# thallolang/thallo

Measured on AMD Instinct MI355X. Metric: pcg_iters_per_sec, higher is better.
Workload: dtype f32

## Files before the change

### include/thallo_hip.h

```cpp
#ifndef THALLO_HIP_H
#define THALLO_HIP_H

#ifdef __cplusplus
extern "C" {
#endif

typedef void* thallo_stream_t;

#define THALLO_HIP_MAX_PARTIALS 1024

typedef struct thallo_sum_t {
    const float* partials;
    int          count;
} thallo_sum_t;

typedef struct thallo_segs_t {
    long off[8];
    long len[8];
    int  n;
} thallo_segs_t;

#define THALLO_DIST_MAX_WORLD 8
#define THALLO_DIST_CTL_WORDS 16
typedef struct thallo_dist_t {
// ... 27 lines not shown

int thallo_hip_pcg_step2(float* r, const float* Ap, const float* pre, float* z, long n,
                         thallo_sum_t alphaN, thallo_sum_t alphaD, float* betaN_out, thallo_stream_t stream);

int thallo_hip_pcg_step2_ranges(float* r, const float* Ap, const float* pre, float* z,
                                long off0, long len0, long off1, long len1,
                                thallo_sum_t alphaN, thallo_sum_t alphaD, float* betaN_out, thallo_stream_t stream);

int thallo_hip_pcg_step2_full(float* delta, const float* p, float* r, const float* Ap, const float* pre,
                              float* z, const float* b, long n, thallo_sum_t alphaN, thallo_sum_t alphaD,
                              float* betaN_out, float* q_out, int lm, thallo_stream_t stream);

int thallo_hip_pcg_step3(float* p, const float* z, long n, thallo_sum_t betaN, thallo_sum_t alphaN,
                         int lm, thallo_stream_t stream);

int thallo_hip_pcg_pupdate(const float* z, const float* p_in, float* p_out, float* delta, long n, int first,
                           thallo_sum_t alphaN_prev, thallo_sum_t alphaD_prev, thallo_sum_t betaN_prev, thallo_stream_t stream);
int thallo_hip_pcg_pupdate_ranges(const float* z, const float* p_in, float* p_out, float* delta,
                                  long off0, long len0, long off1, long len1, int first,
                                  thallo_sum_t alphaN_prev, thallo_sum_t alphaD_prev, thallo_sum_t betaN_prev, thallo_stream_t stream);

int thallo_hip_lm_finalize_diagonal(const float* diag, float* SSq, float* CtC, float* pre, const float* r, float* b, float* z, long n,
                                    float radius, float min_lm_diagonal, float max_lm_diagonal, int save_ssq, int use_preconditioner,
                                    float* alphaN_out, thallo_stream_t stream);
int thallo_hip_lm_step1_finish(float* Ap, const float* CtC, const float* p, long n, float* alphaD_out, thallo_stream_t stream);
int thallo_hip_lm_step2_first_half(float* delta, const float* p, long n, thallo_sum_t alphaN, thallo_sum_t alphaD, thallo_stream_t stream);
int thallo_hip_lm_step2_second_half(float* r, const float* b, const float* Adelta, const float* pre, float* z, const float* delta, long n,
                                    float* betaN_out, float* q_out, thallo_stream_t stream);
int thallo_hip_pcg_init_finish(const float* r, const float* diag, float* pre, float* z, long n, int use_preconditioner,
                               float* alphaN_out, thallo_stream_t stream);
void thallo_hip_lm_set_gate(const unsigned* gate);
int thallo_hip_lm_state_reset(float* state, thallo_stream_t stream);
int thallo_hip_lm_zeta(thallo_sum_t q, int k, float q_tolerance, float* state, thallo_stream_t stream);
int thallo_hip_pcg_step2_full_zeta(float* delta, const float* p, float* r, const float* Ap, const float* pre,
                                   float* z, const float* b, long n, thallo_sum_t alphaN, thallo_sum_t alphaD,
                                   float* betaN_out, float* q_out, unsigned* tickets, int k, float q_tolerance, float* lm_state, thallo_stream_t stream);
int thallo_hip_dot(const float* a, const float* b, long n, float* out, thallo_stream_t stream);

int thallo_hip_linear_update(float* X, const float* delta, const float* p, long len,
                             thallo_sum_t alphaN, thallo_sum_t alphaD, thallo_stream_t stream);

int thallo_hip_slab_pack_iter(const float* vec, thallo_segs_t segs, const float* alphaD_partials, const double* s3_partials, int count, float* out, thallo_stream_t stream);
int thallo_hip_slab_unpack_iter(float* vec, thallo_segs_t top, const float* src_top, thallo_segs_t bot, const float* src_bot,
                                const float* gathered, long stride, int world, thallo_sum_t alphaN, float* alphaD_word, float* betaN_word, thallo_stream_t stream);
int thallo_hip_block_sums(const float* p, const float* Ap, const float* r, const float* pre, long n, float* alphaD_out, double* s3_out, thallo_stream_t stream);
int thallo_hip_shard_scalars(const float* gathered, long stride, int world, const float* alphaD_partials, const double* s3_partials, int count, thallo_sum_t alphaN,
                             float* alphaD_word, float* betaN_word, thallo_stream_t stream);
int thallo_hip_range_unpack(float* vec, thallo_segs_t first_rank_pieces, const float* gathered, long stride, long skip, int world, thallo_stream_t stream);
int thallo_hip_linear_update2(float* X, const float* delta, const float* p_older, thallo_sum_t alphaN_older, thallo_sum_t alphaD_older,
                              const float* p, thallo_sum_t alphaN, thallo_sum_t alphaD, long len, thallo_stream_t stream);
#define THALLO_HIP_MAX_UPDATE_TERMS 32
typedef struct { const float* p[THALLO_HIP_MAX_UPDATE_TERMS]; thallo_sum_t alphaN[THALLO_HIP_MAX_UPDATE_TERMS], alphaD[THALLO_HIP_MAX_UPDATE_TERMS]; int count; } thallo_update_terms_t;
int thallo_hip_linear_update_n(float* X, float* delta, thallo_update_terms_t terms, long len, int max_workgroups , thallo_stream_t stream);
int thallo_hip_wave64_selftest(unsigned long long* out_ballot, unsigned* out_peers, float* sums4);
int thallo_hip_finish_sum(thallo_sum_t s, float* out, thallo_stream_t stream);
int thallo_hip_finish_sum_gated(thallo_sum_t s, float* out, const unsigned* gate, thallo_stream_t stream);

int thallo_hip_slab_pack(const float* vec, thallo_segs_t segs, thallo_sum_t sum, float* out, thallo_stream_t stream);
int thallo_hip_slab_unpack(float* vec, thallo_segs_t top, const float* src_top, thallo_segs_t bot, const float* src_bot,
                           const float* gathered, long stride, int world, float* sum_out, thallo_stream_t stream);

int thallo_hip_alpha_beta(thallo_sum_t alphaN, thallo_sum_t alphaD, thallo_sum_t betaN, float* out2,
                          thallo_stream_t stream);

int thallo_hip_lapimg_cost(int W, int H, const float* X, const float* A, float w_fit, int xguard,
                           float* cost_out, thallo_stream_t stream);
int thallo_hip_lapimg_pcg_init(int W, int H, const float* X, const float* A, float w_fit, int xguard,
                               float* r, float* z, float* p_prev, float* delta,
                               float* diag_out, float* alphaN_out, thallo_stream_t stream);
int thallo_hip_lapimg_apply_jtj(int W, int H, float w_fit, int xguard, const float* p, float* Ap, float* alphaD_out, thallo_stream_t stream);
int thallo_hip_lapimg_pcg_step1(int W, int H, float w_fit, int xguard,
                                const float* z, const float* p_in, float* p_out, float* delta, float* Ap,
                                int first, thallo_sum_t alphaN_prev, thallo_sum_t alphaD_prev, thallo_sum_t betaN_prev,
                                float* alphaD_out, thallo_stream_t stream);

int thallo_hip_iw_cost(int W, int H, int row0, int row1, const float* offset, const float* angle, const float* urshape,
                       const float* constraints, const float* mask, float w_fit, float w_reg,
                       float* cost_out, thallo_stream_t stream);
int thallo_hip_iw_pcg_init(int W, int H, int row0, int row1, const float* offset, const float* angle, const float* urshape,
                           const float* constraints, const float* mask, float w_fit, float w_reg,
                           float* r, float* pre, float* z, float* p_prev, float* delta,
                           float* cs, unsigned char* flags, float* diag_out, int* irregular_out, float* alphaN_out, thallo_stream_t stream);
int thallo_hip_iw_pcg_step1(int W, int H, int row0, int row1, const float* cs, const float* urshape, const unsigned char* flags,
                            float w_fit, float w_reg,
                            const float* z, const float* p_in, float* p_out, float* delta, float* Ap,
                            int mode, thallo_sum_t alphaN_prev, thallo_sum_t alphaD_prev, thallo_sum_t betaN_prev,
                            thallo_sum_t alphaN_prev2, thallo_sum_t alphaD_prev2,
                            const int* irregular, const float* r, float* alphaD_out, thallo_stream_t stream);
#define THALLO_IW_STEP1_MODE(k, batched) ((k) == 0 ? 1 : !(batched) ? 0 : ((k) & 1) ? 2 : 4)
int thallo_hip_iw_pcg_iter(int W, int H, int row0, int row1, const float* cs, const float* urshape, const unsigned char* flags, const float* pre,
                           float w_fit, float w_reg, const float* r_in, float* r_out, const float* Ap_in, float* Ap_out,
                           const float* p_in, float* p_out, float* delta, int mode,
                           thallo_sum_t alphaN_prev, thallo_sum_t alphaD_prev, thallo_sum_t betaN_prev,
                           thallo_sum_t alphaN_prev2, thallo_sum_t alphaD_prev2,
                           const int* irregular, float* alphaD_out, double* s12_out,
                           unsigned* fin_tickets, float* alphaD_word, float* betaN_word, thallo_stream_t stream);
#define THALLO_HIP_FIN_TICKET_WORDS 528
int thallo_hip_iw_pcg_iter_dist(int W, int H, int row0, int row1, const float* cs, const float* urshape, const unsigned char* flags, const float* pre,
                                float w_fit, float w_reg, const float* r_in, float* r_out, const float* Ap_in, float* Ap_out,
                                const float* p_in, float* p_out, float* delta, int mode,
                                thallo_sum_t alphaN_prev, thallo_sum_t alphaD_prev, thallo_sum_t betaN_prev,
                                thallo_sum_t alphaN_prev2, thallo_sum_t alphaD_prev2,
                                const int* irregular, thallo_dist_t d, float* alphaD_out, double* s12_out,
                                unsigned* fin_tickets, int slot0, float* alphaD_word, float* betaN_word, thallo_stream_t stream);
int thallo_hip_iw_pcg_iter_march(int W, int H, int row0, int row1, const float* cs, const unsigned char* flags,
                                 float w_fit, float w_reg, const float* r_in, float* r_out, const float* Ap_in, float* Ap_out,
// ... 307 lines not shown
```

### thallo_amd/api.py

```python
import ctypes as C
import os

import numpy as np

_HERE = os.path.dirname(os.path.abspath(__file__))
LIB_PATH = os.path.join(_HERE, "libThallo.so")
ENERGY_DIR = os.path.join(_HERE, "energies")


class InitializationParameters(C.Structure):
    _fields_ = [(n, C.c_int) for n in ("doublePrecision", "verbosityLevel", "timingLevel",
                                       "threadsPerBlock", "useAutoscheduler", "cpuOnly")]


class PerformanceEntry(C.Structure):
    _fields_ = [("count", C.c_uint), ("minMS", C.c_double), ("maxMS", C.c_double),
                ("meanMS", C.c_double), ("stddevMS", C.c_double)]


class PerformanceSummary(C.Structure):
    _fields_ = [(n, PerformanceEntry) for n in ("total", "nonlinearIteration", "nonlinearSetup",
                                                "linearSolve", "nonlinearResolve")]


class SumT(C.Structure):
    _fields_ = [("partials", C.c_void_p), ("count", C.c_int)]


class DistT(C.Structure):
    _fields_ = [("mail", C.c_void_p), ("peer_mail", C.c_void_p * 8), ("peer_r", C.c_void_p * 2), ("peer_off_o", C.c_long * 2),
                ("peer_off_a", C.c_long * 2), ("ctl", C.c_void_p), ("world", C.c_int), ("rank", C.c_int)]


class SegsT(C.Structure):
    _fields_ = [("off", C.c_long * 8), ("len", C.c_long * 8), ("n", C.c_int)]


INT_PARAMS = ("nIterations", "lIterations", "residual_reset_period", "nIter")

_lib = None


AllGatherFn = C.CFUNCTYPE(C.c_int, C.c_void_p, C.c_void_p, C.c_void_p, C.c_long, C.c_void_p)
AllReduceFn = C.CFUNCTYPE(C.c_int, C.c_void_p, C.c_void_p, C.c_long, C.c_void_p)


class DistributedT(C.Structure):
    _fields_ = [("rank", C.c_int), ("world", C.c_int), ("row0", C.c_uint), ("row1", C.c_uint),
                ("allgather", AllGatherFn), ("user", C.c_void_p), ("device_exchange", C.c_int),
                ("global_row0", C.c_uint), ("global_rows", C.c_uint), ("allreduce", AllReduceFn)]


def lib():
    global _lib
    if _lib is not None:
        return _lib
    path = os.environ.get("THALLO_LIB") or LIB_PATH
    if not os.path.exists(path):
        raise RuntimeError(f"{path} not found: build it with `python -c 'import __graft_entry__ as g; g.build()'` "
                           "(make -C thallo_amd/csrc). There is no CPU fallback.")
    L = C.CDLL(path)
    vp, vpp = C.c_void_p, C.POINTER(C.c_void_p)
    L.Thallo_NewState.argtypes = [InitializationParameters]; L.Thallo_NewState.restype = vp
    L.Thallo_ProblemDefine.argtypes = [vp, C.c_char_p, C.c_char_p]; L.Thallo_ProblemDefine.restype = vp
    L.Thallo_ProblemDelete.argtypes = [vp, vp]
    L.Thallo_ProblemPlan.argtypes = [vp, vp, C.POINTER(C.c_uint)]; L.Thallo_ProblemPlan.restype = vp
    L.Thallo_PlanFree.argtypes = [vp, vp]
    L.Thallo_SetSolverParameter.argtypes = [vp, vp, C.c_char_p, vp]
    L.Thallo_GetSolverParameter.argtypes = [vp, vp, C.c_char_p, vp]
    L.Thallo_ProblemSolve.argtypes = [vp, vp, vpp]
    L.Thallo_ProblemInit.argtypes = [vp, vp, vpp]
    L.Thallo_ProblemStep.argtypes = [vp, vp, vpp]; L.Thallo_ProblemStep.restype = C.c_int
    L.Thallo_ProblemCurrentCost.argtypes = [vp, vp]; L.Thallo_ProblemCurrentCost.restype = C.c_double
    L.Thallo_GetPerformanceSummary.argtypes = [vp, vp, C.POINTER(PerformanceSummary)]
    L.ThalloX_SetStream.argtypes = [vp, vp]
    L.ThalloX_SetKernelSampling.argtypes = [vp, C.c_int]
    L.ThalloX_GetKernelStat.argtypes = [vp, C.c_int, C.POINTER(C.c_char_p), C.POINTER(C.c_long), C.POINTER(C.c_long), C.POINTER(C.c_double)]
    L.ThalloX_GetKernelStat.restype = C.c_int
    L.ThalloX_GetKernelStatOwn.argtypes = [vp, C.c_int, C.POINTER(C.c_long), C.POINTER(C.c_double)]
    L.ThalloX_GetKernelStatOwn.restype = C.c_int
    L.ThalloX_ResetKernelStats.argtypes = [vp]
    L.ThalloX_GetAlphaBetaTrace.argtypes = [vp, vp, C.c_int]; L.ThalloX_GetAlphaBetaTrace.restype = C.c_int
    L.ThalloX_EnableLM.argtypes = [vp, C.c_int]
    L.ThalloX_PlanEnergyName.argtypes = [vp]; L.ThalloX_PlanEnergyName.restype = C.c_char_p
    L.ThalloX_LastError.restype = C.c_char_p
    L.ThalloX_PlanReady.argtypes = [vp]; L.ThalloX_PlanReady.restype = C.c_int
    L.ThalloX_PlanScheduleName.argtypes = [vp]; L.ThalloX_PlanScheduleName.restype = C.c_char_p
    L.ThalloX_PlanSetDistributed.argtypes = [vp, C.POINTER(DistributedT)]; L.ThalloX_PlanSetDistributed.restype = C.c_int
    L.ThalloX_PlanDistributedInfo.argtypes = [vp]; L.ThalloX_PlanDistributedInfo.restype = C.c_char_p
    L.ThalloX_DistributedControl.argtypes = [vp, C.c_int, C.c_int]; L.ThalloX_DistributedControl.restype = C.c_int
    L.ThalloX_UnknownsChanged.argtypes = [vp, vp]
    L.ThalloX_RcclUniqueId.argtypes = [vp]; L.ThalloX_RcclUniqueId.restype = C.c_int
    L.ThalloX_PlanUseRccl.argtypes = [vp, vp, C.c_int, C.c_int]; L.ThalloX_PlanUseRccl.restype = C.c_int
    L.ThalloX_RcclSelfTest.argtypes = []; L.ThalloX_RcclSelfTest.restype = C.c_int
    L.ThalloX_RcclAvailable.argtypes = []; L.ThalloX_RcclAvailable.restype = C.c_int
    L.ThalloX_DistributedKernelOnly.argtypes = [vp, C.c_int]; L.ThalloX_DistributedKernelOnly.restype = C.c_int
    L.ThalloX_ProblemFileHash.argtypes = [C.c_char_p, C.c_char_p, C.c_int]; L.ThalloX_ProblemFileHash.restype = C.c_ulonglong
    L.ThalloX_ProblemFileSchedule.argtypes = [C.c_char_p]; L.ThalloX_ProblemFileSchedule.restype = C.c_int
    fl, ci, cl = C.c_float, C.c_int, C.c_long
    L.thallo_hip_vector_elems.argtypes = [cl]; L.thallo_hip_vector_elems.restype = cl
    L.thallo_hip_finish_sum.argtypes = [SumT, vp, vp]
    L.thallo_hip_iw_cost.argtypes = [ci, ci, ci, ci, vp, vp, vp, vp, vp, fl, fl, vp, vp]
    L.thallo_hip_iw_pcg_init.argtypes = [ci, ci, ci, ci, vp, vp, vp, vp, vp, fl, fl, vp, vp, vp, vp, vp, vp, vp, vp, vp, vp, vp]
    L.thallo_hip_iw_pcg_step1.argtypes = [ci, ci, ci, ci, vp, vp, vp, fl, fl, vp, vp, vp, vp, vp, ci, SumT, SumT, SumT, SumT, SumT, vp, vp, vp, vp]
    L.thallo_hip_linear_update2.argtypes = [vp, vp, vp, SumT, SumT, vp, SumT, SumT, cl, vp]
    L.thallo_hip_ipc_alloc.argtypes = [C.c_long, C.POINTER(vp), vp]
    L.thallo_hip_ipc_alloc2.argtypes = [C.c_long, C.POINTER(vp), vp, C.POINTER(ci)]
    L.thallo_hip_ipc_open.argtypes = [vp, C.POINTER(vp)]
    L.thallo_hip_ipc_close.argtypes = [vp]; L.thallo_hip_ipc_free.argtypes = [vp]
    L.thallo_hip_dist_begin_step.argtypes = [DistT, vp]
    L.thallo_hip_dist_collect.argtypes = [DistT, ci, ci, vp, vp]
    L.thallo_hip_dist_error.argtypes = [DistT, ci, vp]
    L.thallo_hip_slab_pack_iter.argtypes = [vp, SegsT, vp, vp, ci, vp, vp]
    L.thallo_hip_slab_unpack_iter.argtypes = [vp, SegsT, vp, SegsT, vp, vp, cl, ci, SumT, vp, vp, vp]
    L.thallo_hip_dist_exchange.argtypes = [DistT, ci, SumT, vp, vp]
    L.thallo_hip_dist_exchange_iter.argtypes = [DistT, ci, vp, vp, ci, SumT, vp, vp, vp]
    _iter = [ci, ci, ci, ci, vp, vp, vp, vp, fl, fl, vp, vp, vp, vp, vp, vp, vp, ci, SumT, SumT, SumT, SumT, SumT, vp]
    L.thallo_hip_iw_pcg_iter.argtypes = _iter + [vp, vp, vp, vp, vp, vp]
    L.thallo_hip_iw_pcg_iter_dist.argtypes = _iter + [DistT, vp, vp, vp, ci, vp, vp, vp]
    _march = [ci, ci, ci, ci, vp, vp, fl, fl, vp, vp, vp, vp, vp, vp, vp, ci, SumT, SumT, SumT, SumT, SumT, vp]
    L.thallo_hip_iw_pcg_iter_march.argtypes = _march + [vp, vp, vp, vp, vp, vp]
    L.thallo_hip_iw_pcg_iter_march_dist.argtypes = _march + [DistT, vp, vp, vp, ci, vp, vp, vp]
    L.thallo_hip_iw_urshape_irregular.argtypes = [ci, ci, vp, vp, vp]
    L.thallo_hip_march_debug_set.argtypes = [ci, ci]
    L.thallo_hip_iw_pcg_iter_finish.argtypes = [vp, vp, ci, SumT, vp, vp, vp]
    L.thallo_hip_iw_pcg_step2_dist.argtypes = [ci, ci, ci, ci, vp, fl, fl, vp, vp, SumT, SumT, DistT, vp, vp]
    L.thallo_hip_iw_pcg_step2.argtypes = [ci, ci, ci, ci, vp, fl, fl, vp, vp, vp, vp, SumT, SumT, vp, vp, vp]
    L.thallo_hip_iw_apply_jtj.argtypes = [ci, ci, ci, ci, vp, vp, vp, fl, fl, vp, vp, vp, vp, vp]
    L.thallo_hip_pcg_step2.argtypes = [vp, vp, vp, vp, cl, SumT, SumT, vp, vp]
    L.thallo_hip_pcg_step2_ranges.argtypes = [vp, vp, vp, vp, cl, cl, cl, cl, SumT, SumT, vp, vp]
    L.thallo_hip_linear_update.argtypes = [vp, vp, vp, cl, SumT, SumT, vp]
    L.thallo_hip_slab_pack.argtypes = [vp, SegsT, SumT, vp, vp]
    L.thallo_hip_slab_unpack.argtypes = [vp, SegsT, vp, SegsT, vp, vp, cl, ci, vp, vp]
    _lib = L
    return L


def energy_file(name):
    p = os.path.join(ENERGY_DIR, name if name.endswith(".t") else name + ".t")
    if not os.path.exists(p):
        raise FileNotFoundError(p)
    return p


def last_error():
    return lib().ThalloX_LastError().decode()


def slab_ghost_rows(path, dims):
    L = lib()
    L.ThalloX_FrontendSlabGhostRows.argtypes = [C.c_char_p, C.c_void_p]
    L.ThalloX_FrontendSlabGhostRows.restype = C.c_int
    d = (C.c_uint * len(dims))(*[int(x) for x in dims])
    g = L.ThalloX_FrontendSlabGhostRows(os.fsencode(path), d)
    if g < 0:
        raise ValueError(last_error())
    return g


def rccl_unique_id():
    buf = (C.c_ubyte * 128)()
    if lib().ThalloX_RcclUniqueId(C.addressof(buf)) != 0:
        raise RuntimeError("ThalloX_RcclUniqueId failed: " + last_error())
    return bytes(buf)


def _ptr_of(x):
    if hasattr(x, "data_ptr"):
        return x.data_ptr()
    if isinstance(x, (C.c_float, C.c_int, C.c_double, C.c_uint)):
        return C.addressof(x)
    if isinstance(x, int):
        return x
    raise TypeError(f"cannot turn {type(x)} into a problem parameter")

# ... 145 lines not shown
        import json
        t = self._L.ThalloX_PlanDistributedInfo(self.plan).decode()
        return json.loads(t) if t else {}

    def distributed_error(self, clear=True):
        return self._L.ThalloX_DistributedControl(self.plan, 0, 1 if clear else 0)

    def distributed_use_allgather(self):
        return self._L.ThalloX_DistributedControl(self.plan, 1, 0)

    def distributed_kernel_only(self, reps):
        return self._L.ThalloX_DistributedKernelOnly(self.plan, reps)

    def unknowns_changed(self):
        self._L.ThalloX_UnknownsChanged(self.state, self.plan)

    def enable_lm(self, on=True):
        self._L.ThalloX_EnableLM(self.plan, 1 if on else 0)

    def set_kernel_sampling(self, period):
        self._L.ThalloX_SetKernelSampling(self.plan, period)

    def reset_kernel_stats(self):
        self._L.ThalloX_ResetKernelStats(self.plan)

    def kernel_stats(self):
        out = {}
        i = 0
        while True:
            name = C.c_char_p(); launches = C.c_long(); samples = C.c_long(); total = C.c_double()
            if self._L.ThalloX_GetKernelStat(self.plan, i, C.byref(name), C.byref(launches), C.byref(samples), C.byref(total)):
                break
            ks = C.c_long(); kt = C.c_double()
            self._L.ThalloX_GetKernelStatOwn(self.plan, i, C.byref(ks), C.byref(kt))
            out[name.value.decode()] = {"launches": launches.value, "samples": samples.value, "total_ms": total.value,
                                        "mean_ms": total.value / samples.value if samples.value else None,
                                        "own_samples": ks.value, "own_mean_ms": kt.value / ks.value if ks.value else None}
            i += 1
        return out

    def alpha_beta_trace(self, cap=4096):
        buf = (C.c_float * (2 * cap))()
        n = self._L.ThalloX_GetAlphaBetaTrace(self.plan, C.addressof(buf), cap)
        n = min(n, cap)
        return [(buf[2 * i], buf[2 * i + 1]) for i in range(n)]


def iw_fused_bytes_per_iter(L, every_iteration_delta=False, ring=False):
    if os.environ.get("THALLO_MARCH", "1")[:1] in ("0", "3", "4"):
        return 99.0
    if L < 1:
        return 0.0
    if ring:
        return (69.0 + 57.0 * (L - 1)) / L
    if every_iteration_delta:
        return (69.0 + 81.0 * (L - 1)) / L
    odd, even = L // 2, (L - 1) // 2
    return (69.0 + 57.0 * odd + 93.0 * even) / L
```

### thallo_amd/csrc/energy_image_warping.hip

```cpp
#include "iw_device.hpp"

using namespace thallo;

namespace {

constexpr int TW = 64, TH = 16, BLOCK = 256;
constexpr int LW = TW + 2, LH = TH + 2, LN = LW * LH;
constexpr int PER = TH / (BLOCK / TW);
constexpr int HALO = 2 * LW + 2 * TH;

inline Geo make_geo(int W, int H, int row0, int row1)
{
    Geo g; g.W = W; g.H = H; g.row0 = row0; g.row1 = row1;
    g.tx = (W + TW - 1) / TW; g.ty = (row1 - row0 + TH - 1) / TH; g.ntiles = g.tx * g.ty;
    return g;
}
inline bool rows_ok(int H, int row0, int row1) { return row0 >= 0 && row1 <= H && row0 < row1; }
inline int grid_for(const Geo& g, int per_cu)
{
    int cap = thallo_hip_device_cu_count() * per_cu;
    if (cap > THALLO_MAX_PARTIALS) cap = THALLO_MAX_PARTIALS;
    cap -= cap % 8;
    return g.ntiles < cap ? g.ntiles : cap;
}
// ... 213 lines not shown

template <bool DIST>
__global__ __launch_bounds__(BLOCK) void k_step2_iw(float4* __restrict__ r, const float4* __restrict__ Ap, const float4* __restrict__ pre,
                                                     float4* __restrict__ z, const unsigned char* __restrict__ flags, long N, float wf2, float wr2,
                                                     long off0, long len0, long off1, long len1,
                                                     thallo_sum_t aN, thallo_sum_t aD, const int* __restrict__ irregular, float* __restrict__ bN_out,
                                                     thallo_dist_t dd, long row_o4, long row_a4)
{
    __shared__ float red[16];
    const bool grid = DIST || (irregular != nullptr && __builtin_amdgcn_readfirstlane(irregular[0]) == 0);
    const float alpha = safe_div<false>(sum_partials(aN.partials, aN.count), sum_partials(aD.partials, aD.count));
    float acc = 0.0f;
    const long n4 = len0 + len1;
    for (long j = (long)blockIdx.x * BLOCK + threadIdx.x; j < n4; j += (long)gridDim.x * BLOCK) {
        const bool in_off = j < len0;
        const long i = in_off ? off0 + j : off1 + (j - len0);
        float4 rv = ldf4(r + i, true);
        const float4 av = Ap[i];
        rv.x -= alpha * av.x; rv.y -= alpha * av.y; rv.z -= alpha * av.z; rv.w -= alpha * av.w;
        float4 m;
        if (grid) {
            if (in_off) {
                const unsigned f2 = reinterpret_cast<const unsigned short*>(flags)[i];
                float m0, m1, dummy;
                pre_from_flags((unsigned char)(f2 & 255), wf2, wr2, m0, dummy); pre_from_flags((unsigned char)(f2 >> 8), wf2, wr2, m1, dummy);
                m = make_float4(m0, m0, m1, m1);
            } else {
                const unsigned f4 = reinterpret_cast<const unsigned*>(flags)[i - N / 2];
                float d, a0, a1, a2, a3;
                pre_from_flags((unsigned char)(f4 & 255), wf2, wr2, d, a0); pre_from_flags((unsigned char)((f4 >> 8) & 255), wf2, wr2, d, a1);
                pre_from_flags((unsigned char)((f4 >> 16) & 255), wf2, wr2, d, a2); pre_from_flags((unsigned char)(f4 >> 24), wf2, wr2, d, a3);
                m = make_float4(a0, a1, a2, a3);
            }
        } else m = pre[i];
        const float4 zv = make_float4(m.x * rv.x, m.y * rv.y, m.z * rv.z, m.w * rv.w);
        stf4(r + i, rv, true);
        if (!grid) z[i] = zv;
        if (DIST) {
            const long jj = in_off ? j : j - len0, rowlen = in_off ? row_o4 : row_a4, total = in_off ? len0 : len1;
            if (jj < rowlen && dd.peer_r[0]) {
                float* dst = dd.peer_r[0] + (in_off ? dd.peer_off_o[0] : dd.peer_off_a[0]) + 4 * jj;
                st_sys(dst, rv.x); st_sys(dst + 1, rv.y); st_sys(dst + 2, rv.z); st_sys(dst + 3, rv.w);
            }
            if (jj >= total - rowlen && dd.peer_r[1]) {
                float* dst = dd.peer_r[1] + (in_off ? dd.peer_off_o[1] : dd.peer_off_a[1]) + 4 * (jj - (total - rowlen));
                st_sys(dst, rv.x); st_sys(dst + 1, rv.y); st_sys(dst + 2, rv.z); st_sys(dst + 3, rv.w);
            }
        }
        acc += zv.x * rv.x + zv.y * rv.y + zv.z * rv.z + zv.w * rv.w;
    }
    block_store_partial(acc, bN_out, red);
}

__global__ __launch_bounds__(BLOCK) void k_init(Geo g, const float2* __restrict__ off, const float* __restrict__ ang,
                                                const float2* __restrict__ ur, const float2* __restrict__ cons,
                                                const float* __restrict__ mask, float wf, float wr,
                                                float* __restrict__ r, float* __restrict__ pre, float* __restrict__ z,
                                                float* __restrict__ p_prev, float* __restrict__ delta,
                                                float2* __restrict__ cs, unsigned char* __restrict__ flags,
                                                float* __restrict__ diag_out, int* __restrict__ irregular, float* __restrict__ aN_out)
{
    __shared__ Tile T;
    __shared__ float red[16];
    const long N = (long)g.W * g.H;
    const float wr2 = wr * wr, wf2 = wf * wf;
    float acc = 0.0f;
    int bad = 0;
    for (TileSweep t(g.ntiles); t.valid(); t.next()) {
        const int x0 = (t.cur % g.tx) * TW, y0 = g.row0 + (t.cur / g.tx) * TH;
        for (int idx = threadIdx.x; idx < LN; idx += BLOCK) {
            const int ly = idx / LW, lx = idx - ly * LW;
            const int gx = x0 + lx - 1, gy = y0 + ly - 1;
            float ox = 0.f, oy = 0.f, cc = 1.f, ss = 0.f, uxx = 0.f, uyy = 0.f; unsigned char ff = 0;
            if (gx >= 0 && gx < g.W && gy >= 0 && gy < g.H) {
                const long pix = (long)gy * g.W + gx;
                const float2 o = off[pix]; const float2 u = ur[pix];
                ox = o.x; oy = o.y; uxx = u.x; uyy = u.y;
                sincosf(ang[pix], &ss, &cc);
                ff = mask[pix] == 0.0f ? 1 : 0;
                if ((gy < g.row0 || gy >= g.row1) && lx >= 1 && lx <= TW) {
                    cs[pix] = make_float2(cc, ss); flags[pix] = ff;
                    reinterpret_cast<float2*>(p_prev)[pix] = make_float2(0.f, 0.f); p_prev[2 * N + pix] = 0.f;
                }
            }
            T.px[idx] = ox; T.py[idx] = oy; T.c[idx] = cc; T.s[idx] = ss; T.ux[idx] = uxx; T.uy[idx] = uyy; T.f[idx] = ff;
        }
        __syncthreads();
        const int lx = (threadIdx.x % TW) + 1;
        const int gx = x0 + lx - 1;
        for (int k = 0; k < PER; ++k) {
            const int ly = (threadIdx.x / TW) * PER + k + 1;
            const int gy = y0 + ly - 1;
            const int i = ly * LW + lx;
            if (gx < g.W && gy < g.row1) {
                const long pix = (long)gy * g.W + gx;
                const unsigned char act = T.f[i] & 1;
                if (gx + 1 < g.W && (T.ux[i + 1] - T.ux[i] != 1.0f || T.uy[i + 1] - T.uy[i] != 0.0f)) bad = 1;
                if (gy + 1 < g.H && (T.ux[i + LW] - T.ux[i] != 0.0f || T.uy[i + LW] - T.uy[i] != 1.0f)) bad = 1;
                float rx = 0.f, ry = 0.f, ra = 0.f, mx = 0.f, my = 0.f, ma = 0.f, dgo_raw = 0.f, dga_raw = 0.f;
                unsigned char fl = act;
                if (act) {
                    const float oxi = T.px[i], oyi = T.py[i], ci = T.c[i], si = T.s[i], uxi = T.ux[i], uyi = T.uy[i];
                    float jx = 0.f, jy = 0.f, ja = 0.f, dgo = 0.f, dga = 0.f;
                    int cnt = 0; bool unit = true;
                    const int nb[4] = { i + 1, i - 1, i + LW, i - LW };
#pragma unroll
                    for (int d = 0; d < 4; ++d) {
                        const int j = nb[d];
                        if (T.f[j] & 1) {
                            const float dux = uxi - T.ux[j], duy = uyi - T.uy[j];
                            unit = unit && dux == (d == 0 ? -1.0f : d == 1 ? 1.0f : 0.0f) && duy == (d == 2 ? -1.0f : d == 3 ? 1.0f : 0.0f);
                            ++cnt;
                            const float dox = oxi - T.px[j], doy = oyi - T.py[j];
                            const float eix = dox - (ci * dux - si * duy), eiy = doy - (si * dux + ci * duy);
                            const float cj = T.c[j], sj = T.s[j];
                            const float ejx = -dox + (cj * dux - sj * duy), ejy = -doy + (sj * dux + cj * duy);
                            const float gix = -si * dux - ci * duy, giy = ci * dux - si * duy;
                            jx += eix - ejx; jy += eiy - ejy;
                            ja -= gix * eix + giy * eiy;
                            dgo += 2.0f; dga += gix * gix + giy * giy;
                        }
                    }
                    jx *= wr2; jy *= wr2; ja *= wr2; dgo *= wr2; dga *= wr2;
                    if (unit) dga = (float)cnt * wr2;
                    fl |= (unsigned char)(cnt << 2);
                    const float2 cv = cons[pix];
                    if (cv.x >= 0.0f && cv.y >= 0.0f) {
                        fl |= 2;
                        jx += wf2 * (oxi - cv.x); jy += wf2 * (oyi - cv.y); dgo += wf2;
                    }
                    rx = -jx; ry = -jy; ra = -ja;
                    mx = guarded_invert(dgo); my = mx; ma = guarded_invert(dga);
                    dgo_raw = dgo; dga_raw = dga;
                }
                if (diag_out) {
                    reinterpret_cast<float2*>(diag_out)[pix] = make_float2(dgo_raw, dgo_raw); diag_out[2 * N + pix] = dga_raw;
                }
                reinterpret_cast<float2*>(r)[pix] = make_float2(rx, ry);  r[2 * N + pix] = ra;
                reinterpret_cast<float2*>(pre)[pix] = make_float2(mx, my); pre[2 * N + pix] = ma;
                const float zx = mx * rx, zy = my * ry, zaa = ma * ra;
                reinterpret_cast<float2*>(z)[pix] = make_float2(zx, zy);  z[2 * N + pix] = zaa;
                reinterpret_cast<float2*>(p_prev)[pix] = make_float2(0.f, 0.f); p_prev[2 * N + pix] = 0.f;
                reinterpret_cast<float2*>(delta)[pix] = make_float2(0.f, 0.f);  delta[2 * N + pix] = 0.f;
                cs[pix] = make_float2(T.c[i], T.s[i]);
                flags[pix] = fl;
                acc += rx * zx + ry * zy + ra * zaa;
            }
        }
        __syncthreads();
    }
    if (irregular && __any(bad) && (threadIdx.x & 63) == 0) atomicAdd(irregular, 1);
    block_store_partial(acc, aN_out, red);
}

constexpr int CW = 64, CH = 4;
__global__ __launch_bounds__(BLOCK) void k_cost(int W, int H, int row0, int row1, int ctx, int ntiles,
                                                const float2* __restrict__ off, const float* __restrict__ ang,
                                                const float2* __restrict__ ur, const float2* __restrict__ cons,
                                                const float* __restrict__ mask, float wf, float wr, float* __restrict__ out)
{
    __shared__ float red[16];
    float acc = 0.0f;
    for (TileSweep t(ntiles); t.valid(); t.next()) {
        const int x = (t.cur % ctx) * CW + (threadIdx.x % CW), y = row0 + (t.cur / ctx) * CH + (threadIdx.x / CW);
        if (x < W && y < row1) {
            const long i = (long)y * W + x;
            if (mask[i] == 0.0f) {
                const float2 o = off[i]; const float2 u = ur[i];
                float si, ci; sincosf(ang[i], &si, &ci);
                float s2 = 0.f;
                const int dx[4] = { 1, -1, 0, 0 }, dy[4] = { 0, 0, 1, -1 };
#pragma unroll
                for (int d = 0; d < 4; ++d) {
                    const int xn = x + dx[d], yn = y + dy[d];
                    if (xn >= 0 && xn < W && yn >= 0 && yn < H) {
                        const long j = (long)yn * W + xn;
                        if (mask[j] == 0.0f) {
                            const float2 oj = off[j]; const float2 uj = ur[j];
                            const float dux = u.x - uj.x, duy = u.y - uj.y;
                            const float ex = wr * ((o.x - oj.x) - (ci * dux - si * duy));
                            const float ey = wr * ((o.y - oj.y) - (si * dux + ci * duy));
                            s2 += ex * ex + ey * ey;
                        }
                    }
                }
                const float2 cv = cons[i];
                if (cv.x >= 0.0f && cv.y >= 0.0f) {
                    const float fx = wf * (o.x - cv.x), fy = wf * (o.y - cv.y);
                    s2 += fx * fx + fy * fy;
                }
                acc += 0.5f * s2;
            }
        }
    }
    block_store_partial(acc, out, red);
}
// ... 245 lines not shown
                                                       PrevSums prev)
{
    __shared__ TileI T;
    __shared__ float red[16];
    __shared__ double redd[48];
    const bool grid = irregular != nullptr && __builtin_amdgcn_readfirstlane(irregular[0]) == 0;
    if (grid) iter_body<true, NT, DIST>(T, red, redd, g, cs, ur, flags, pre, wf2, wr2, r_in, r_out, A_in, A_out, p_in, p_out, delta, mode, aNp, aDp, bNp, aNpp, aDpp, aD_out, s12_out, ntm, &dd, fin_tickets, aD_word, bN_word, xslot, prev);
    else      iter_body<false, NT, DIST>(T, red, redd, g, cs, ur, flags, pre, wf2, wr2, r_in, r_out, A_in, A_out, p_in, p_out, delta, mode, aNp, aDp, bNp, aNpp, aDpp, aD_out, s12_out, ntm, &dd, fin_tickets, aD_word, bN_word, xslot, prev);
}

__global__ __launch_bounds__(64) void k_iter_finish(const float* __restrict__ aD_part, const double* __restrict__ s12, int nb, thallo_sum_t aN,
                                                    float* __restrict__ aD_word, float* __restrict__ bN_word)
{
    const int lane = threadIdx.x;
    const float ad = sum_partials(aD_part, nb);
    double n = 0.0, a = 0.0, b = 0.0;
    for (int i = lane; i < nb; i += THALLO_WAVE) { n += s12[3 * i]; a += s12[3 * i + 1]; b += s12[3 * i + 2]; }
    n = wave_sum_all_d(n); a = wave_sum_all_d(a); b = wave_sum_all_d(b);
    const float an = sum_partials(aN.partials, aN.count);
    const float alpha = safe_div<false>(an, ad);
    double bn = n - 2.0 * (double)alpha * a + (double)alpha * (double)alpha * b;
    if (!(bn > 0.0)) bn = 0.0;
    if (lane == 0) { aD_word[0] = ad; bN_word[0] = (float)bn; }
}

}

extern "C" {

#ifdef THALLO_MARCH_SWEEP
int thallo_hip_debug_stamps(unsigned long long* buf) { return hipMemcpyToSymbol(HIP_SYMBOL(g_stamps), &buf, sizeof buf) == hipSuccess ? 0 : -1; }
#endif
void thallo_hip_debug_set(int what, int value) { if (what == 0) g_iw_debug = value; if (what == 3) g_nt_mask = value; if (what == 4) g_no_grid = value; if (what == 5) g_step1_per_cu = value; if (what == 6) g_step1_threads = value; if (what == 7) g_iter_nt = value; if (what == 8) g_iter_per_cu = value < 1 ? 1 : value > 2 ? 2 : value; }

int thallo_hip_iw_cost(int W, int H, int row0, int row1, const float* offset, const float* angle, const float* urshape,
                       const float* constraints, const float* mask, float w_fit, float w_reg,
                       float* cost_out, thallo_stream_t stream)
{
    if (!rows_ok(H, row0, row1)) return -(int)hipErrorInvalidValue;
    const int ctx = (W + CW - 1) / CW, cty = (row1 - row0 + CH - 1) / CH, nt = ctx * cty;
    int grid = thallo_hip_device_cu_count() * 4; if (grid > THALLO_MAX_PARTIALS) grid = THALLO_MAX_PARTIALS;
    grid -= grid % 8; if (nt < grid) grid = nt;
    hipLaunchKernelGGL(k_cost, dim3(grid), dim3(BLOCK), 0, (hipStream_t)stream, W, H, row0, row1, ctx, nt,
                       (const float2*)offset, angle, (const float2*)urshape, (const float2*)constraints, mask, w_fit, w_reg, cost_out);
    int e = check_launch(); return e ? e : grid;
}

int thallo_hip_iw_pcg_init(int W, int H, int row0, int row1, const float* offset, const float* angle, const float* urshape,
                           const float* constraints, const float* mask, float w_fit, float w_reg,
                           float* r, float* pre, float* z, float* p_prev, float* delta,
                           float* cs, unsigned char* flags, float* diag_out, int* irregular_out, float* aN_out, thallo_stream_t stream)
{
    if (!rows_ok(H, row0, row1)) return -(int)hipErrorInvalidValue;
    const Geo g = make_geo(W, H, row0, row1); const int grid = grid_for(g, 4);
    if (irregular_out && hipMemsetAsync(irregular_out, 0, sizeof(int), (hipStream_t)stream) != hipSuccess) return -(int)hipErrorInvalidValue;
    hipLaunchKernelGGL(k_init, dim3(grid), dim3(BLOCK), 0, (hipStream_t)stream, g,
                       (const float2*)offset, angle, (const float2*)urshape, (const float2*)constraints, mask, w_fit, w_reg,
                       r, pre, z, p_prev, delta, (float2*)cs, flags, diag_out, irregular_out, aN_out);
    int e = check_launch(); return e ? e : grid;
}

int thallo_hip_iw_pcg_step1(int W, int H, int row0, int row1, const float* cs, const float* urshape, const unsigned char* flags,
                            float w_fit, float w_reg,
                            const float* z, const float* p_in, float* p_out, float* delta, float* Ap,
                            int mode, thallo_sum_t aNp, thallo_sum_t aDp, thallo_sum_t bNp, thallo_sum_t aNpp, thallo_sum_t aDpp,
                            const int* irregular, const float* r, float* aD_out, thallo_stream_t stream)
{
    if (!r || ((2L * W * H) & 3)) irregular = nullptr;
    if (!rows_ok(H, row0, row1)) return -(int)hipErrorInvalidValue;
    const Geo g = make_geo(W, H, row0, row1);
    int grid;
    if (g_step1_threads == 512) {
        grid = grid_for(g, g_step1_per_cu > 2 ? 2 : g_step1_per_cu);
        hipLaunchKernelGGL((k_step1<true, 4, 512>), dim3(grid), dim3(512), 0, (hipStream_t)stream, g,
                           (const float2*)cs, (const float2*)urshape, flags, w_fit * w_fit, w_reg * w_reg,
                           z, p_in, p_out, delta, Ap, mode, aNp, aDp, bNp, aNpp, aDpp, aD_out, g_iw_debug | (g_nt_mask << 8), g_no_grid ? nullptr : irregular, r);
    } else {
        grid = grid_for(g, g_step1_per_cu);
        hipLaunchKernelGGL((k_step1<true, 3, 256>), dim3(grid), dim3(BLOCK), 0, (hipStream_t)stream, g,
                           (const float2*)cs, (const float2*)urshape, flags, w_fit * w_fit, w_reg * w_reg,
                           z, p_in, p_out, delta, Ap, mode, aNp, aDp, bNp, aNpp, aDpp, aD_out, g_iw_debug | (g_nt_mask << 8), g_no_grid ? nullptr : irregular, r);
    }
    int e = check_launch(); return e ? e : grid;
}

int thallo_hip_iw_pcg_step2(int W, int H, int row0, int row1, const unsigned char* flags, float w_fit, float w_reg,
                            float* r, const float* Ap, const float* pre, float* z,
                            thallo_sum_t aN, thallo_sum_t aD, const int* irregular, float* bN_out, thallo_stream_t stream)
{
    if (!rows_ok(H, row0, row1)) return -(int)hipErrorInvalidValue;
    const long N = (long)W * H, rows = row1 - row0;
    const long off0 = 2L * W * row0, len0 = 2L * W * rows, off1 = 2 * N + (long)W * row0, len1 = (long)W * rows;
    if (g_no_grid || ((off0 | len0 | off1 | len1 | (2 * N)) & 3)) {
        if (row0 == 0 && row1 == H) return thallo_hip_pcg_step2(r, Ap, pre, z, 3 * N, aN, aD, bN_out, stream);
        return thallo_hip_pcg_step2_ranges(r, Ap, pre, z, off0, len0, off1, len1, aN, aD, bN_out, stream);
    }
    long want = ((len0 + len1) / 4 + BLOCK - 1) / BLOCK;
    int grid = thallo_hip_device_cu_count() * 4; if (grid > THALLO_MAX_PARTIALS) grid = THALLO_MAX_PARTIALS; grid -= grid % 8;
    if (want < grid) grid = (int)(want < 1 ? 1 : want);
    hipLaunchKernelGGL(k_step2_iw<false>, dim3(grid), dim3(BLOCK), 0, (hipStream_t)stream, (float4*)r, (const float4*)Ap, (const float4*)pre, (float4*)z,
                       flags, N, w_fit * w_fit, w_reg * w_reg, off0 / 4, len0 / 4, off1 / 4, len1 / 4, aN, aD, irregular, bN_out, thallo_dist_t{}, 0L, 0L);
    int e = check_launch(); return e ? e : grid;
}

static bool dist_args_ok(const thallo_dist_t& d)
{
    return d.world >= 1 && d.world <= THALLO_DIST_MAX_WORLD && d.rank >= 0 && d.rank < d.world && d.mail && d.ctl && d.peer_mail[d.rank] == d.mail;
}

int thallo_hip_iw_pcg_step2_dist(int W, int H, int row0, int row1, const unsigned char* flags, float w_fit, float w_reg,
                                 float* r, const float* Ap, thallo_sum_t aN, thallo_sum_t aD, thallo_dist_t d,
// ... 109 lines not shown
```

### thallo_amd/csrc/energy_image_warping_march_rc.hip

```cpp
#include "iw_march.hpp"
#include <hip/hip_ext.h>

using namespace thallo;

namespace {

inline int check_launch() { hipError_t e = hipGetLastError(); return e == hipSuccess ? 0 : -(int)e; }

typedef __amdgpu_buffer_rsrc_t rsrc_t;
typedef unsigned u32x4 __attribute__((ext_vector_type(4)));
typedef unsigned u32x2 __attribute__((ext_vector_type(2)));
__device__ __forceinline__ rsrc_t make_rsrc(const void* p) { return __builtin_amdgcn_make_buffer_rsrc(const_cast<void*>(p), 0, 0xffffffffu, 0x00020000); }
template <bool NT> __device__ __forceinline__ u32x4 bld4(rsrc_t r, unsigned vo, unsigned so) { return __builtin_amdgcn_raw_buffer_load_b128(r, vo, so, NT ? 2 : 0); }
template <bool NT> __device__ __forceinline__ u32x2 bld2(rsrc_t r, unsigned vo, unsigned so) { return __builtin_amdgcn_raw_buffer_load_b64(r, vo, so, NT ? 2 : 0); }
template <bool NT> __device__ __forceinline__ unsigned bld1(rsrc_t r, unsigned vo, unsigned so) { return __builtin_amdgcn_raw_buffer_load_b32(r, vo, so, NT ? 2 : 0); }
template <bool NT> __device__ __forceinline__ void bst4(rsrc_t r, unsigned vo, unsigned so, float a, float b, float c, float d)
{ u32x4 v; v.x = __float_as_uint(a); v.y = __float_as_uint(b); v.z = __float_as_uint(c); v.w = __float_as_uint(d); __builtin_amdgcn_raw_buffer_store_b128(v, r, vo, so, NT ? 2 : 0); }
template <bool NT> __device__ __forceinline__ void bst2(rsrc_t r, unsigned vo, unsigned so, float a, float b)
{ u32x2 v; v.x = __float_as_uint(a); v.y = __float_as_uint(b); __builtin_amdgcn_raw_buffer_store_b64(v, r, vo, so, NT ? 2 : 0); }
__device__ __forceinline__ float uf(unsigned u) { return __uint_as_float(u); }
__device__ __forceinline__ float to_sgpr(float v) { return __int_as_float(__builtin_amdgcn_readfirstlane(__float_as_int(v))); }

__device__ __forceinline__ float rc_sum(thallo_sum_t s)
{
// ... 24 lines not shown
    beta = safe_div<false>(bn, an);
}

__device__ __forceinline__ void rc_exchange_prev(thallo_sum_t aNp, const PrevSums& prev, const thallo_dist_t& dd)
{
    typedef unsigned long long u64_t;
    const unsigned seq = ld_agent(dd.ctl + DIST_SEQ);
    const unsigned tag = (seq << 12) | (unsigned)(prev.xslot / 7 + 1);
    const IterationSums S = load_iteration_sums(prev.aD_part, prev.s12_part, prev.count, aNp);
    float ad = 0.0f, al = 0.0f, bn = 0.0f;
    dist_exchange_iter_wave_seq(dd, seq, prev.xslot, S.ad, S.n, S.s1, S.s2, S.an, prev.aD_word, prev.bN_word, ExtraSums{ false, 0.0f, 0.0, 0.0, 0.0 }, &ad, &al, &bn);
    if ((threadIdx.x & (THALLO_WAVE - 1)) == 0) {
        __hip_atomic_store(prev.gs, ((u64_t)tag << 32) | (u64_t)__float_as_uint(ad), __ATOMIC_RELAXED, __HIP_MEMORY_SCOPE_AGENT);
        __hip_atomic_store(prev.gs + 1, ((u64_t)tag << 32) | (u64_t)__float_as_uint(bn), __ATOMIC_RELAXED, __HIP_MEMORY_SCOPE_AGENT);
    }
}
__device__ __forceinline__ void rc_iteration_scalars_x(thallo_sum_t aNp, const PrevSums& prev, const thallo_dist_t& dd, float& alpha, float& beta)
{
    typedef unsigned long long u64_t;
    const float an = rc_sum(aNp);
    const unsigned seq = ld_agent(dd.ctl + DIST_SEQ);
    const unsigned tag = (seq << 12) | (unsigned)(prev.xslot / 7 + 1);
    u64_t v0 = __hip_atomic_load(prev.gs, __ATOMIC_RELAXED, __HIP_MEMORY_SCOPE_AGENT), v1 = __hip_atomic_load(prev.gs + 1, __ATOMIC_RELAXED, __HIP_MEMORY_SCOPE_AGENT);
    int it = 0; long long t0 = 0;
    const long long bound = dist_spin_ticks(dd);
    while ((unsigned)(v0 >> 32) != tag || (unsigned)(v1 >> 32) != tag) {
        if ((it & 255) == 0) { if (ld_agent(dd.ctl + DIST_ERR) != 0) break; if (it == 0) t0 = wall_clock64(); }
        ++it;
        if ((it & 255) == 0 && wall_clock64() - t0 > bound) {
            if (__hip_atomic_exchange(dd.ctl + DIST_ERR, 1u, __ATOMIC_RELAXED, __HIP_MEMORY_SCOPE_AGENT) == 0u) {
                unsigned* pm = dd.ctl + DIST_POST_MORTEM;
                pm[0] = (unsigned)prev.xslot; pm[1] = 0xffffu; pm[2] = tag; pm[3] = (unsigned)(v0 >> 32); pm[4] = (unsigned)(v1 >> 32);
            }
            break;
        }
        __builtin_amdgcn_s_sleep(4);
        v0 = __hip_atomic_load(prev.gs, __ATOMIC_RELAXED, __HIP_MEMORY_SCOPE_AGENT); v1 = __hip_atomic_load(prev.gs + 1, __ATOMIC_RELAXED, __HIP_MEMORY_SCOPE_AGENT);
    }
    const float ad = __uint_as_float((unsigned)v0), bn = __uint_as_float((unsigned)v1);
    alpha = safe_div<false>(an, ad);
    beta = safe_div<false>(bn, an);
}
__global__ __launch_bounds__(64) void k_rc_dist_finish(thallo_sum_t aNp, PrevSums prev, thallo_dist_t dd) { rc_exchange_prev(aNp, prev, dd); }

template <int DMODE>
struct RawRc {
    u32x4 po, cs; u32x2 pa; unsigned f;
    u32x4 ro; u32x2 ra;
    u32x4 dlo, ppo; u32x2 dla, ppa;
};
typedef unsigned long long u64x2 __attribute__((ext_vector_type(2)));
__device__ __forceinline__ void take4u(u32x4& d, const u32x4& s) { const u64x2 sv = __builtin_bit_cast(u64x2, s); unsigned long long a, b; take_pair(a, sv.x); take_pair(b, sv.y); u64x2 dv; dv.x = a; dv.y = b; d = __builtin_bit_cast(u32x4, dv); }
__device__ __forceinline__ void take2u(u32x2& d, const u32x2& s) { unsigned long long a; take_pair(a, __builtin_bit_cast(unsigned long long, s)); d = __builtin_bit_cast(u32x2, a); }
template <int DMODE>
__device__ __forceinline__ void take(RawRc<DMODE>& d, const RawRc<DMODE>& s)
{
    take4u(d.po, s.po); take2u(d.pa, s.pa); take4u(d.cs, s.cs); take1(d.f, s.f); take4u(d.ro, s.ro); take2u(d.ra, s.ra);
    if (DMODE != 1) { take4u(d.dlo, s.dlo); take2u(d.dla, s.dla); }
    if (DMODE == 2) { take4u(d.ppo, s.ppo); take2u(d.ppa, s.ppa); }
}

template <int V> struct IC { static constexpr int value = V; };
enum { PH_ENTER = 0, PH_S1 = 1, PH_FULL = 2 };

struct PRow { v2f xy[2]; float pa[2]; };
struct GRow { v2f cs[2], gx[2]; float a[2]; unsigned f; };
struct RRow { v2f xy[2]; float ra[2]; };
__device__ __forceinline__ v2f uf2(unsigned a, unsigned b) { return v2f{ uf(a), uf(b) }; }

template <int DMODE, int DEPTH, int NTM, int OCC, int SLAB>
__global__ __launch_bounds__(MARCH_NT, OCC) void k_iter_march_rc(MarchGeo g, const float* __restrict__ cs, const unsigned char* __restrict__ flags, float wf2, float wr2,
                                                            const float* __restrict__ r_in, float* __restrict__ r_out, const float* __restrict__ A_in, float* __restrict__ A_out,
                                                            const float* __restrict__ p_in, float* __restrict__ p_out, float* __restrict__ delta,
                                                            thallo_sum_t aNp, thallo_sum_t aDp, thallo_sum_t bNp, thallo_sum_t aNpp, thallo_sum_t aDpp,
                                                            float* __restrict__ aD_out, double* __restrict__ s12_out, const int* __restrict__ irregular,
                                                            thallo_dist_t dd, unsigned* __restrict__ fin_tickets, float* __restrict__ aD_word, float* __restrict__ bN_word, int xslot,
                                                            PrevSums prev)
{
    static_assert(DEPTH == 1 || DEPTH == 2 || DEPTH == 4, "the prefetch slots rotate inside a trip of four rows");
    __shared__ float4 lut[32];
    __shared__ float red[16];
    __shared__ double redd[48];
    constexpr bool nt_delta = NTM & 1, nt_ra = NTM & 2, nt_out = NTM & 4, nt_pin = NTM & 8, nt_pout = NTM & 16, nt_const = NTM & 32;
    if (irregular != nullptr && __builtin_amdgcn_readfirstlane(irregular[0]) != 0) {
        if (blockIdx.x == 0 && threadIdx.x == 0 && aD_word) { aD_word[0] = __builtin_nanf(""); bN_word[0] = __builtin_nanf(""); }
        if (blockIdx.x == 0 && threadIdx.x == 0 && prev.count > 0) { prev.aD_word[0] = __builtin_nanf(""); prev.bN_word[0] = __builtin_nanf(""); }
        if (threadIdx.x == 0) { aD_out[blockIdx.x] = __builtin_nanf(""); }
        return;
    }
    if (threadIdx.x < 32) { float mo, ma; pre_from_flags((unsigned char)threadIdx.x, wf2, wr2, mo, ma); lut[threadIdx.x] = make_float4(mo, ma, (threadIdx.x & 2) ? wf2 : 0.f, 0.f); }
    __syncthreads();

    const int lane = threadIdx.x & 63, wave = __builtin_amdgcn_readfirstlane(threadIdx.x >> 6);
    const unsigned N = (unsigned)g.W * (unsigned)g.H;
    const int W2 = g.W >> 1;
    int strip, ya, yb;
    march_place(g, wave, strip, ya, yb);
    const bool work = ya < yb;
    const int x0 = strip * MARCH_USE - 2 + 2 * lane;
    const bool xin = x0 >= 0 && x0 < g.W;
    const bool xout = xin && lane >= 1 && lane <= 62;

    const rsrc_t RS_P = make_rsrc(p_in), RS_R = make_rsrc(r_in), RS_CS = make_rsrc(cs), RS_F = make_rsrc(flags);
    const rsrc_t RS_Q = make_rsrc(p_out), RS_RO = make_rsrc(r_out), RS_D = make_rsrc(delta);
    const rsrc_t RS_AI = make_rsrc(SLAB ? (const void*)A_in : (const void*)r_in), RS_AO = make_rsrc(SLAB ? (void*)A_out : (void*)r_out);
    const int xc = x0 < 0 ? 0 : x0 > g.W - 2 ? g.W - 2 : x0;
    const unsigned h = (unsigned)xc >> 1;
    const unsigned vo16 = h * 16u, vo8 = h * 8u;
    const unsigned vf0 = (h >> 1) * 4u, vf1 = ((h + 1u) >> 1) * 4u, sh0 = (h & 1u) * 16u;
    const unsigned angle0 = 8u * N;

    float alpha = 0.0f, beta = 0.0f, alpha2 = 0.0f;
    const bool scal_writer = work && strip == 0 && ya == g.row0 && lane == 0;

    typedef RawRc<DMODE> RawT;
    RawT slot[DEPTH];
    const unsigned W2u = (unsigned)W2;
    const int t_first = ya - 2, t_last = yb + 1;
    auto issue = [&](RawT& s, int tn, auto CL_) __attribute__((always_inline)) {
        constexpr bool CL = decltype(CL_)::value;
        if (CL && tn > t_last) tn = t_last;
        const unsigned tc = CL ? (unsigned)(tn < 0 ? 0 : tn > g.H - 1 ? g.H - 1 : tn) : (unsigned)tn, row = tc * W2u;
        s.po = bld4<nt_pin>(RS_P, vo16, row * 16u); s.pa = bld2<nt_pin>(RS_P, vo8, angle0 + row * 8u);
        s.cs = bld4<nt_const>(RS_CS, vo16, row * 16u);
        const unsigned par = row & 1u;
        s.f = bld1<nt_const>(RS_F, par ? vf1 : vf0, (row - par) * 2u);
        const unsigned tr = CL ? (unsigned)(tn - 1 < 0 ? 0 : tn - 1 > g.H - 1 ? g.H - 1 : tn - 1) : (unsigned)(tn - 1), rrow = tr * W2u;
        s.ro = bld4<nt_ra>(RS_R, vo16, rrow * 16u); s.ra = bld2<nt_ra>(RS_R, vo8, angle0 + rrow * 8u);
        if (DMODE != 1) {
            const unsigned td = CL ? (unsigned)(tn - 1 < ya ? ya : tn - 1 > yb - 1 ? yb - 1 : tn - 1) : (unsigned)(tn - 1), drow = td * W2u;
            s.dlo = bld4<nt_delta>(RS_D, vo16, drow * 16u); s.dla = bld2<nt_delta>(RS_D, vo8, angle0 + drow * 8u);
            if (DMODE == 2) { s.ppo = bld4<false>(RS_Q, vo16, drow * 16u); s.ppa = bld2<false>(RS_Q, vo8, angle0 + drow * 8u); }
        }
    };

    PRow pp[4], pk[4]; GRow gg[4]; RRow rr[2];
#pragma unroll
    for (int i = 0; i < 4; ++i) {
#pragma unroll
        for (int q = 0; q < 2; ++q) { pp[i].xy[q] = v2f{ 0.f, 0.f }; pp[i].pa[q] = 0.f; pk[i].xy[q] = v2f{ 0.f, 0.f }; pk[i].pa[q] = 0.f;
                                      gg[i].cs[q] = v2f{ 1.f, 0.f }; gg[i].gx[q] = v2f{ 0.f, -1.f }; gg[i].a[q] = 0.f; }
        gg[i].f = 0u;
    }
#pragma unroll
    for (int i = 0; i < 2; ++i)
#pragma unroll
        for (int q = 0; q < 2; ++q) { rr[i].xy[q] = v2f{ 0.f, 0.f }; rr[i].ra[q] = 0.f; }

    float acc = 0.0f; double s0 = 0.0, s1 = 0.0, s2 = 0.0;
    const unsigned mxin = xin ? 0xffffu : 0u;

    auto step = [&](int t, auto J_, auto PH_, auto CL_) __attribute__((always_inline)) {
        constexpr int j = decltype(J_)::value, PH = decltype(PH_)::value;
        constexpr bool CL = decltype(CL_)::value;
        PRow& p0 = pp[j % 4]; const PRow& p1 = pp[(j + 3) % 4]; const PRow& p2 = pp[(j + 2) % 4];
        GRow& g0 = gg[j % 4]; const GRow& g1 = gg[(j + 3) % 4]; const GRow& g2 = gg[(j + 2) % 4]; const GRow& g3 = gg[(j + 1) % 4];
        PRow& k1 = pk[(j + 3) % 4]; const PRow& k2 = pk[(j + 2) % 4]; const PRow& k3 = pk[(j + 1) % 4];
        RRow& r1 = rr[(j + 1) % 2]; const RRow& r2 = rr[j % 2];
        RawT cur;
        take(cur, slot[j % DEPTH]);
        fence_order();
        issue(slot[j % DEPTH], t + DEPTH, CL_);
        fence_order();
        {
            const bool rowok = !CL || (t >= 0 && t < g.H);
            const unsigned par = ((unsigned)t * W2u) & 1u;
            const unsigned fl = (cur.f >> (par ? 16u - sh0 : sh0)) & (rowok ? mxin : 0u);
            p0.xy[0] = uf2(cur.po.x, cur.po.y); p0.xy[1] = uf2(cur.po.z, cur.po.w); p0.pa[0] = uf(cur.pa.x); p0.pa[1] = uf(cur.pa.y);
            g0.cs[0] = uf2(cur.cs.x, cur.cs.y); g0.cs[1] = uf2(cur.cs.z, cur.cs.w); g0.f = fl;
            g0.gx[0] = v2f{ g0.cs[0].y, -g0.cs[0].x }; g0.gx[1] = v2f{ g0.cs[1].y, -g0.cs[1].x };
            g0.a[0] = (float)(fl & 1u); g0.a[1] = (float)((fl >> 8) & 1u);
        }
        if constexpr (PH >= PH_S1) {
            const int u = t - 1;
            const float4 m0 = lut[g1.f & 31u], m1 = lut[(g1.f >> 8) & 31u];
            const float wfit[2] = { m0.z, m1.z };
            v2f axy[2]; float av[2];
            jtjp_pair_xy(p2, p1, p0, g2, g1, g0, g2.a, g1.a, g0.a, wfit, wr2, axy, av);
            const bool ghost_row = SLAB && CL && ((u == ya - 1 && ya == g.row0 && u >= 0) || (u == yb && yb == g.row1 && u < g.H));
            if (ghost_row) {
                const unsigned row = (unsigned)u * W2u;
                const u32x4 ao = bld4<false>(RS_AI, vo16, row * 16u); const u32x2 aa = bld2<false>(RS_AI, vo8, angle0 + row * 8u);
                axy[0] = uf2(ao.x, ao.y); axy[1] = uf2(ao.z, ao.w); av[0] = uf(aa.x); av[1] = uf(aa.y);
            }
            v2f rxy[2] = { uf2(cur.ro.x, cur.ro.y), uf2(cur.ro.z, cur.ro.w) }; float rq[2] = { uf(cur.ra.x), uf(cur.ra.y) };
            rxy[0] = fma2(-alpha, axy[0], rxy[0]); rxy[1] = fma2(-alpha, axy[1], rxy[1]);
            rq[0] = __builtin_fmaf(-alpha, av[0], rq[0]); rq[1] = __builtin_fmaf(-alpha, av[1], rq[1]);
            const float mo[2] = { m0.x, m1.x }, ma[2] = { m0.y, m1.y };
#pragma unroll
            for (int q = 0; q < 2; ++q) {
                k1.xy[q] = mo[q] * rxy[q] + beta * p1.xy[q]; k1.pa[q] = ma[q] * rq[q] + beta * p1.pa[q];
                r1.xy[q] = rxy[q]; r1.ra[q] = rq[q];
            }
            const bool mine = !CL || (u >= ya && u < yb);
            if (xout && (mine || ghost_row)) {
                const unsigned row = (unsigned)u * W2u;
                bst4<nt_out>(RS_RO, vo16, row * 16u, rxy[0].x, rxy[0].y, rxy[1].x, rxy[1].y); bst2<nt_out>(RS_RO, vo8, angle0 + row * 8u, rq[0], rq[1]);
                bst4<nt_pout>(RS_Q, vo16, row * 16u, k1.xy[0].x, k1.xy[0].y, k1.xy[1].x, k1.xy[1].y); bst2<nt_pout>(RS_Q, vo8, angle0 + row * 8u, k1.pa[0], k1.pa[1]);
                if (DMODE != 1 && mine) {
                    float d[4] = { uf(cur.dlo.x), uf(cur.dlo.y), uf(cur.dlo.z), uf(cur.dlo.w) }, da[2] = { uf(cur.dla.x), uf(cur.dla.y) };
                    if (DMODE == 2) {
                        d[0] = __builtin_fmaf(alpha2, uf(cur.ppo.x), d[0]); d[1] = __builtin_fmaf(alpha2, uf(cur.ppo.y), d[1]);
                        d[2] = __builtin_fmaf(alpha2, uf(cur.ppo.z), d[2]); d[3] = __builtin_fmaf(alpha2, uf(cur.ppo.w), d[3]);
                        da[0] = __builtin_fmaf(alpha2, uf(cur.ppa.x), da[0]); da[1] = __builtin_fmaf(alpha2, uf(cur.ppa.y), da[1]);
                    }
                    d[0] = __builtin_fmaf(alpha, p1.xy[0].x, d[0]); d[1] = __builtin_fmaf(alpha, p1.xy[0].y, d[1]);
                    d[2] = __builtin_fmaf(alpha, p1.xy[1].x, d[2]); d[3] = __builtin_fmaf(alpha, p1.xy[1].y, d[3]);
                    da[0] = __builtin_fmaf(alpha, p1.pa[0], da[0]); da[1] = __builtin_fmaf(alpha, p1.pa[1], da[1]);
                    bst4<nt_delta>(RS_D, vo16, row * 16u, d[0], d[1], d[2], d[3]); bst2<nt_delta>(RS_D, vo8, angle0 + row * 8u, da[0], da[1]);
                }
            }
        }
        __builtin_amdgcn_sched_barrier(0);
        if constexpr (PH >= PH_FULL) {
            const int v = t - 2;
            const bool on = xout;
            const float4 m0 = lut[on ? g2.f & 31u : 0u], m1 = lut[on ? (g2.f >> 8) & 31u : 0u];
            const float wfit[2] = { m0.z, m1.z }, mo[2] = { m0.x, m1.x }, ma[2] = { m0.y, m1.y };
            v2f axy[2]; float av[2];
            jtjp_pair_xy(k3, k2, k1, g3, g2, g1, g3.a, g2.a, g1.a, wfit, wr2, axy, av);
            if (SLAB && xout && (v == g.row0 || v == g.row1 - 1)) {
                if (SLAB == 1) {
                    const unsigned row = (unsigned)v * W2u;
                    bst4<false>(RS_AO, vo16, row * 16u, axy[0].x, axy[0].y, axy[1].x, axy[1].y); bst2<false>(RS_AO, vo8, angle0 + row * 8u, av[0], av[1]);
                } else {
#pragma unroll
                    for (int k = 0; k < 2; ++k) {
                        if (v == (k == 0 ? g.row0 : g.row1 - 1) && dd.peer_r[k]) {
                            float* d2 = dd.peer_r[k] + dd.peer_off_o[k] + 2 * x0;
                            st_sys(d2, axy[0].x); st_sys(d2 + 1, axy[0].y); st_sys(d2 + 2, axy[1].x); st_sys(d2 + 3, axy[1].y);
                            float* d1 = dd.peer_r[k] + dd.peer_off_a[k] + x0;
                            st_sys(d1, av[0]); st_sys(d1 + 1, av[1]);
                        }
                    }
                }
            }
            const float msum = on ? 1.0f : 0.0f;
            __builtin_amdgcn_sched_barrier(0);
            iter_sums_pixel_masked(msum, k2.xy[0].x, k2.xy[0].y, k2.pa[0], axy[0].x, axy[0].y, av[0], r2.xy[0].x, r2.xy[0].y, r2.ra[0], mo[0], ma[0], acc, s0, s1, s2);
            __builtin_amdgcn_sched_barrier(0);
            iter_sums_pixel_masked(msum, k2.xy[1].x, k2.xy[1].y, k2.pa[1], axy[1].x, axy[1].y, av[1], r2.xy[1].x, r2.xy[1].y, r2.ra[1], mo[1], ma[1], acc, s0, s1, s2);
        }
        asm volatile("" : "+v"(acc), "+v"(s0), "+v"(s1), "+v"(s2));
        __builtin_amdgcn_sched_barrier(0);
    };

    if (SLAB == 2 && prev.gs != nullptr && prev.count > 0 && blockIdx.x == gridDim.x - 1 && wave == 0 && !work) rc_exchange_prev(aNp, prev, dd);

    if (work) {
#pragma unroll
        for (int i = 0; i < DEPTH; ++i) issue(slot[i], t_first + i, IC<1>{});
        step(t_first, IC<0>{}, IC<PH_ENTER>{}, IC<1>{});
        step(t_first + 1, IC<1>{}, IC<PH_ENTER>{}, IC<1>{});
        if (SLAB == 2 && prev.gs != nullptr && prev.count > 0) rc_iteration_scalars_x(aNp, prev, dd, alpha, beta);
        else rc_iteration_scalars(aNp, aDp, bNp, prev, alpha, beta, scal_writer);
        alpha = to_sgpr(alpha); beta = to_sgpr(beta);
        if (DMODE == 2) alpha2 = to_sgpr(safe_div<false>(rc_sum(aNpp), rc_sum(aDpp)));
        step(ya, IC<2>{}, IC<PH_S1>{}, IC<1>{});
        step(ya + 1, IC<3>{}, IC<PH_S1>{}, IC<1>{});
        int t_lim = t_last < g.H - 1 ? t_last : g.H - 1;
        if (DMODE != 1 && yb < t_lim) t_lim = yb;
        const int t_safe = t_lim - DEPTH;
        int t = ya + 2;
        for (; t + 3 <= t_safe; t += 4) {
            step(t, IC<0>{}, IC<PH_FULL>{}, IC<0>{});
            step(t + 1, IC<1>{}, IC<PH_FULL>{}, IC<0>{});
            step(t + 2, IC<2>{}, IC<PH_FULL>{}, IC<0>{});
            step(t + 3, IC<3>{}, IC<PH_FULL>{}, IC<0>{});
        }
        auto tail = [&](auto I_) __attribute__((always_inline)) {
            constexpr int i = decltype(I_)::value;
            if constexpr (i < DEPTH + 5) { if (t + i <= t_last) step(t + i, IC<i % 4>{}, IC<PH_FULL>{}, IC<1>{}); }
        };
        tail(IC<0>{}); tail(IC<1>{}); tail(IC<2>{}); tail(IC<3>{}); tail(IC<4>{}); tail(IC<5>{}); tail(IC<6>{}); tail(IC<7>{}); tail(IC<8>{});
    }
    iter_tail<MARCH_NT, SLAB == 2>(acc, s0, s1, s2, red, redd, aD_out, s12_out, bNp, &dd, fin_tickets, aD_word, bN_word, xslot);
}

}

[[maybe_unused]] constexpr int MARCH_RC_DEPTH = 4;
constexpr int MARCH_RC_OCC = 2;
[[maybe_unused]] constexpr int MARCH_RC_DEEP_ROWS = 24;
#ifdef THALLO_MARCH_SWEEP
namespace thallo {
int g_march_rc_depth = MARCH_RC_DEPTH;
int g_march_rc_occ = MARCH_RC_OCC;
int g_march_rc_nt = MARCH_NTM;
}
#endif

namespace {
struct LaunchEvents { hipEvent_t start = nullptr, stop = nullptr; int armed = 0, used = 0; };
thread_local LaunchEvents g_launch_ev;

template <int SLAB>
int launch_march_rc(int W, int H, int row0, int row1, const float* cs, const unsigned char* flags, float w_fit, float w_reg,
                    const float* r_in, float* r_out, const float* A_in, float* A_out, const float* p_in, float* p_out, float* delta, int mode,
                    thallo_sum_t aNp, thallo_sum_t aDp, thallo_sum_t bNp, thallo_sum_t aNpp, thallo_sum_t aDpp, const int* irregular, thallo_dist_t d,
                    float* aD_out, double* s12_out, unsigned* fin_tickets, float* aD_word, float* bN_word, int xslot, hipStream_t stream, PrevSums prev)
{
    const int R = march_pick_rows(W, row1 - row0);
    if (R <= 0) return -(int)hipErrorNotSupported;
    const MarchGeo g = make_march_geo(W, H, row0, row1, R);
    const int grid = (g.total + 7) / 8 * 8 + ((SLAB == 2 && prev.gs != nullptr) ? 8 : 0);
    if (grid > THALLO_MAX_PARTIALS) return -(int)hipErrorInvalidValue;
    const int dmode = (mode >> 1) & 3;
    const float wf2 = w_fit * w_fit, wr2 = w_reg * w_reg;
    const bool ev_on = g_launch_ev.armed != 0;
    if (ev_on) g_launch_ev.used = 1;
#define RC_LAUNCH(DM, DP, OCC, NTM) do { if (ev_on) hipExtLaunchKernelGGL((k_iter_march_rc<DM, DP, NTM, OCC, SLAB>), dim3(grid), dim3(MARCH_NT), 0, stream, g_launch_ev.start, g_launch_ev.stop, 0, g, cs, flags, wf2, wr2, \
        r_in, r_out, A_in, A_out, p_in, p_out, delta, aNp, aDp, bNp, aNpp, aDpp, aD_out, s12_out, irregular, d, fin_tickets, aD_word, bN_word, xslot, prev); \
    else hipLaunchKernelGGL((k_iter_march_rc<DM, DP, NTM, OCC, SLAB>), dim3(grid), dim3(MARCH_NT), 0, stream, g, cs, flags, wf2, wr2, \
        r_in, r_out, A_in, A_out, p_in, p_out, delta, aNp, aDp, bNp, aNpp, aDpp, aD_out, s12_out, irregular, d, fin_tickets, aD_word, bN_word, xslot, prev); } while (0)
#ifdef THALLO_MARCH_SWEEP
#define RC_BY_DEPTH(DM) do { if constexpr (SLAB != 0) RC_LAUNCH(DM, MARCH_RC_DEPTH, MARCH_RC_OCC, MARCH_NTM); else { const int dp = g_march_rc_depth, oc = g_march_rc_occ, nt = g_march_rc_nt; \
        if (nt != MARCH_NTM) { if (nt == 0) RC_LAUNCH(DM, MARCH_RC_DEPTH, 2, 0); else if (nt == 1) RC_LAUNCH(DM, MARCH_RC_DEPTH, 2, 1); else if (nt == 4) RC_LAUNCH(DM, MARCH_RC_DEPTH, 2, 4); else if (nt == 7) RC_LAUNCH(DM, MARCH_RC_DEPTH, 2, 7); \
                                 else if (nt == 13) RC_LAUNCH(DM, MARCH_RC_DEPTH, 2, 13); else if (nt == 21) RC_LAUNCH(DM, MARCH_RC_DEPTH, 2, 21); else if (nt == 37) RC_LAUNCH(DM, MARCH_RC_DEPTH, 2, 37); else if (nt == 63) RC_LAUNCH(DM, MARCH_RC_DEPTH, 2, 63); else return -(int)hipErrorInvalidValue; } \
        else if (oc == 1) { if (dp == 4) RC_LAUNCH(DM, 4, 1, MARCH_NTM); else RC_LAUNCH(DM, 2, 1, MARCH_NTM); } \
        else if (oc == 3) { if (dp == 1) RC_LAUNCH(DM, 1, 3, MARCH_NTM); else RC_LAUNCH(DM, 2, 3, MARCH_NTM); } \
        else { if (dp == 1) RC_LAUNCH(DM, 1, 2, MARCH_NTM); else if (dp == 4) RC_LAUNCH(DM, 4, 2, MARCH_NTM); else RC_LAUNCH(DM, 2, 2, MARCH_NTM); } } } while (0)
#else
#define RC_BY_DEPTH(DM) do { if (R >= MARCH_RC_DEEP_ROWS) RC_LAUNCH(DM, 4, MARCH_RC_OCC, MARCH_NTM); else RC_LAUNCH(DM, 2, MARCH_RC_OCC, MARCH_NTM); } while (0)
#endif
    if (dmode == 1) RC_BY_DEPTH(1); else if (dmode == 2) RC_BY_DEPTH(2); else RC_BY_DEPTH(0);
#undef RC_BY_DEPTH
#undef RC_LAUNCH
    int e = check_launch(); return e ? e : grid;
}

int rc_check(int W, int H, int row0, int row1, const void* cs, const void* flags, const void* r_in, const void* r_out, const void* A_in, const void* A_out,
             const void* p_in, const void* p_out, const void* delta, int mode, thallo_sum_t aNp, thallo_sum_t aNpp, thallo_sum_t aDpp, const void* aD_out, const void* s12_out)
{
    if ((W & 1) || W < 2 || H < 1 || row0 < 0 || row1 > H || row0 >= row1 || row0 > 1 || H - row1 > 1) return -(int)hipErrorInvalidValue;
    if (mode & 1) return -(int)hipErrorInvalidValue;
    if (!cs || !flags || !r_in || !r_out || !p_in || !p_out || !delta || !aD_out || !s12_out) return -(int)hipErrorInvalidValue;
    if ((row0 > 0 || row1 < H) && (!A_in || !A_out)) return -(int)hipErrorInvalidValue;
    if (aNp.count < 1 || !aNp.partials) return -(int)hipErrorInvalidValue;
    if (((mode >> 1) & 3) == 2 && (aNpp.count < 1 || aDpp.count < 1 || !aNpp.partials || !aDpp.partials)) return -(int)hipErrorInvalidValue;
    if (12.0 * (double)W * (double)H >= 4294967296.0) return -(int)hipErrorNotSupported;
    return 0;
}
}

extern "C" {

int thallo_hip_iw_pcg_iter_march_rc(int W, int H, int row0, int row1, const float* cs, const unsigned char* flags, float w_fit, float w_reg,
                                    const float* r_in, float* r_out, const float* Ap_in, float* Ap_out, const float* p_in, float* p_out, float* delta, int mode,
                                    thallo_sum_t aNp, thallo_sum_t aDp, thallo_sum_t bNp, thallo_sum_t aNpp, thallo_sum_t aDpp,
                                    const int* irregular, float* aD_out, double* s12_out,
                                    unsigned* fin_tickets, float* aD_word, float* bN_word, thallo_stream_t stream)
{
    if (int e = rc_check(W, H, row0, row1, cs, flags, r_in, r_out, Ap_in, Ap_out, p_in, p_out, delta, mode, aNp, aNpp, aDpp, aD_out, s12_out)) return e;
    if (aDp.count < 1 || bNp.count < 1 || !aDp.partials || !bNp.partials) return -(int)hipErrorInvalidValue;
    if (!fin_tickets || !aD_word || !bN_word) { fin_tickets = nullptr; aD_word = nullptr; bN_word = nullptr; }
    const PrevSums none = { nullptr, nullptr, 0, nullptr, nullptr };
    if (row0 == 0 && row1 == H)
        return launch_march_rc<0>(W, H, row0, row1, cs, flags, w_fit, w_reg, r_in, r_out, nullptr, nullptr, p_in, p_out, delta, mode, aNp, aDp, bNp, aNpp, aDpp, irregular, thallo_dist_t{},
                                  aD_out, s12_out, fin_tickets, aD_word, bN_word, 0, (hipStream_t)stream, none);
    return launch_march_rc<1>(W, H, row0, row1, cs, flags, w_fit, w_reg, r_in, r_out, Ap_in, Ap_out, p_in, p_out, delta, mode, aNp, aDp, bNp, aNpp, aDpp, irregular, thallo_dist_t{},
                              aD_out, s12_out, fin_tickets, aD_word, bN_word, 0, (hipStream_t)stream, none);
}

int thallo_hip_iw_pcg_iter_march_rc_deferred(int W, int H, int row0, int row1, const float* cs, const unsigned char* flags, float w_fit, float w_reg,
                                             const float* r_in, float* r_out, const float* Ap_in, float* Ap_out, const float* p_in, float* p_out, float* delta, int mode,
                                             thallo_sum_t aNp, thallo_sum_t aNpp, thallo_sum_t aDpp, thallo_prev_t prev,
                                             const int* irregular, float* aD_out, double* s12_out, thallo_stream_t stream)
{
    if (int e = rc_check(W, H, row0, row1, cs, flags, r_in, r_out, Ap_in, Ap_out, p_in, p_out, delta, mode, aNp, aNpp, aDpp, aD_out, s12_out)) return e;
    if (prev.count < 1 || prev.count > THALLO_MAX_PARTIALS || !prev.alphaD_partials || !prev.s12_partials || !prev.alphaD_word || !prev.betaN_word ||
        prev.s12_partials == s12_out) return -(int)hipErrorInvalidValue;
    const thallo_sum_t none = { nullptr, 0 };
    const PrevSums ps = { prev.alphaD_partials, prev.s12_partials, prev.count, prev.alphaD_word, prev.betaN_word };
    if (row0 == 0 && row1 == H)
        return launch_march_rc<0>(W, H, row0, row1, cs, flags, w_fit, w_reg, r_in, r_out, nullptr, nullptr, p_in, p_out, delta, mode, aNp, none, none, aNpp, aDpp, irregular, thallo_dist_t{},
                                  aD_out, s12_out, nullptr, nullptr, nullptr, 0, (hipStream_t)stream, ps);
    return launch_march_rc<1>(W, H, row0, row1, cs, flags, w_fit, w_reg, r_in, r_out, Ap_in, Ap_out, p_in, p_out, delta, mode, aNp, none, none, aNpp, aDpp, irregular, thallo_dist_t{},
                              aD_out, s12_out, nullptr, nullptr, nullptr, 0, (hipStream_t)stream, ps);
}

int thallo_hip_iw_pcg_iter_march_rc_dist(int W, int H, int row0, int row1, const float* cs, const unsigned char* flags, float w_fit, float w_reg,
                                         const float* r_in, float* r_out, const float* Ap_in, float* Ap_out, const float* p_in, float* p_out, float* delta, int mode,
                                         thallo_sum_t aNp, thallo_sum_t aDp, thallo_sum_t bNp, thallo_sum_t aNpp, thallo_sum_t aDpp,
                                         const int* irregular, thallo_dist_t d, float* aD_out, double* s12_out,
                                         unsigned* fin_tickets, int slot0, float* aD_word, float* bN_word, thallo_stream_t stream)
{
    if (int e = rc_check(W, H, row0, row1, cs, flags, r_in, r_out, Ap_in, Ap_out, p_in, p_out, delta, mode, aNp, aNpp, aDpp, aD_out, s12_out)) return e;
    if (!Ap_in || !Ap_out || aDp.count < 1 || bNp.count < 1 || !aDp.partials || !bNp.partials || d.world < 1 || d.world > THALLO_DIST_MAX_WORLD) return -(int)hipErrorInvalidValue;
    if (!fin_tickets || !aD_word || !bN_word) { fin_tickets = nullptr; aD_word = nullptr; bN_word = nullptr; }
    if (fin_tickets && (slot0 < 0 || !d.mail || !d.ctl || 7 * d.world > 64 || bNp.count != 1)) return -(int)hipErrorInvalidValue;
    for (int k = 0; k < 2; ++k) if (d.peer_r[k] && ((d.peer_off_o[k] | d.peer_off_a[k]) & 1)) return -(int)hipErrorInvalidValue;
    return launch_march_rc<2>(W, H, row0, row1, cs, flags, w_fit, w_reg, r_in, r_out, Ap_in, Ap_out, p_in, p_out, delta, mode, aNp, aDp, bNp, aNpp, aDpp, irregular, d,
                              aD_out, s12_out, fin_tickets, aD_word, bN_word, slot0, (hipStream_t)stream, PrevSums{ nullptr, nullptr, 0, nullptr, nullptr });
}

int thallo_hip_iw_march_rc_deferred_fits(int W, int rows)
{
    if (W < 2 || (W & 1) || rows < 1) return 0;
    const int R = march_pick_rows(W, rows);
    if (R <= 0) return 0;
    const MarchGeo g = make_march_geo(W, rows, 0, rows, R);
    const long grid = (g.total + 7) / 8 * 8 + 8;
    return grid <= march_cap(MARCH_RC_OCC) && grid <= THALLO_MAX_PARTIALS ? 1 : 0;
}

int thallo_hip_iw_pcg_iter_march_rc_dist_deferred(int W, int H, int row0, int row1, const float* cs, const unsigned char* flags, float w_fit, float w_reg,
                                                  const float* r_in, float* r_out, const float* Ap_in, float* Ap_out, const float* p_in, float* p_out, float* delta, int mode,
                                                  thallo_sum_t aNp, thallo_sum_t aNpp, thallo_sum_t aDpp, thallo_prev_t prev, int prev_slot0, unsigned long long* gs,
                                                  const int* irregular, thallo_dist_t d, float* aD_out, double* s12_out, thallo_stream_t stream)
{
    if (int e = rc_check(W, H, row0, row1, cs, flags, r_in, r_out, Ap_in, Ap_out, p_in, p_out, delta, mode, aNp, aNpp, aDpp, aD_out, s12_out)) return e;
    if (!Ap_in || !Ap_out || d.world < 1 || d.world > THALLO_DIST_MAX_WORLD || !d.mail || !d.ctl || 7 * d.world > 64 || prev_slot0 < 0 || !gs || aNp.count != 1) return -(int)hipErrorInvalidValue;
    if (!thallo_hip_iw_march_rc_deferred_fits(W, row1 - row0)) return -(int)hipErrorNotSupported;
    if (prev.count < 1 || prev.count > THALLO_MAX_PARTIALS || !prev.alphaD_partials || !prev.s12_partials || !prev.alphaD_word || !prev.betaN_word ||
        prev.s12_partials == s12_out) return -(int)hipErrorInvalidValue;
    for (int k = 0; k < 2; ++k) if (d.peer_r[k] && ((d.peer_off_o[k] | d.peer_off_a[k]) & 1)) return -(int)hipErrorInvalidValue;
    const thallo_sum_t none = { nullptr, 0 };
    const PrevSums ps = { prev.alphaD_partials, prev.s12_partials, prev.count, prev.alphaD_word, prev.betaN_word, gs, prev_slot0 };
    return launch_march_rc<2>(W, H, row0, row1, cs, flags, w_fit, w_reg, r_in, r_out, Ap_in, Ap_out, p_in, p_out, delta, mode, aNp, none, none, aNpp, aDpp, irregular, d,
                              aD_out, s12_out, nullptr, nullptr, nullptr, 0, (hipStream_t)stream, ps);
}
int thallo_hip_iw_dist_finish_deferred(thallo_prev_t prev, int prev_slot0, thallo_sum_t aNp, thallo_dist_t d, unsigned long long* gs, thallo_stream_t stream)
{
    if (prev.count < 1 || prev.count > THALLO_MAX_PARTIALS || !prev.alphaD_partials || !prev.s12_partials || !prev.alphaD_word || !prev.betaN_word || prev_slot0 < 0 || !gs ||
        aNp.count != 1 || !aNp.partials || d.world < 1 || d.world > THALLO_DIST_MAX_WORLD || !d.mail || !d.ctl || 7 * d.world > 64) return -(int)hipErrorInvalidValue;
    const PrevSums ps = { prev.alphaD_partials, prev.s12_partials, prev.count, prev.alphaD_word, prev.betaN_word, gs, prev_slot0 };
// ... 20 lines not shown
```

### thallo_amd/csrc/pcg_kernels.hip

```cpp
#include "device_common.hpp"
#include "../../include/thallo_hip.h"

using namespace thallo;

namespace {

constexpr int BLOCK = 256;

inline int flat_grid(long n4, int cus)
{
    long want = (n4 + BLOCK - 1) / BLOCK;
    long cap = (long)cus * 4;
    if (cap > THALLO_MAX_PARTIALS) cap = THALLO_MAX_PARTIALS;
    if (cap >= 8) cap -= cap % 8;
    if (want > cap) want = cap;
    if (want < 1) want = 1;
    return (int)want;
}

int g_cus = 0;
int g_nt2 = 3;
int cu_count()
{
    if (!g_cus) {
// ... 388 lines not shown
{
    __shared__ float red[16];
    float acc = 0.0f;
    for (long i = (long)blockIdx.x * BLOCK + threadIdx.x; i < n4; i += (long)gridDim.x * BLOCK) {
        const float4 rv = r[i];
        float4 m = make_float4(1.f, 1.f, 1.f, 1.f);
        if (use_precond) { const float4 d = diag[i]; m = make_float4(guarded_invert(d.x), guarded_invert(d.y), guarded_invert(d.z), guarded_invert(d.w)); }
        const float4 zv = make_float4(m.x * rv.x, m.y * rv.y, m.z * rv.z, m.w * rv.w);
        pre[i] = m; z[i] = zv;
        acc += rv.x * zv.x + rv.y * zv.y + rv.z * zv.z + rv.w * zv.w;
    }
    block_store_partial(acc, aN_out, red);
}

__global__ __launch_bounds__(BLOCK) void k_dot(const float4* __restrict__ a, const float4* __restrict__ b, long n4, float* __restrict__ out)
{
    __shared__ float red[16];
    float acc = 0.0f;
    for (long i = (long)blockIdx.x * BLOCK + threadIdx.x; i < n4; i += (long)gridDim.x * BLOCK) {
        const float4 x = a[i], y = b[i];
        acc += x.x * y.x + x.y * y.y + x.z * y.z + x.w * y.w;
    }
    block_store_partial(acc, out, red);
}

template <bool HAS_P>
__global__ __launch_bounds__(BLOCK) void k_linear_update(float* __restrict__ X, const float* __restrict__ delta,
                                                          const float* __restrict__ p, long len,
                                                          thallo_sum_t aN, thallo_sum_t aD)
{
    float alpha = 0.0f;
    if (HAS_P) alpha = safe_div<false>(sum_partials(aN.partials, aN.count), sum_partials(aD.partials, aD.count));
    for (long i = (long)blockIdx.x * BLOCK + threadIdx.x; i < len; i += (long)gridDim.x * BLOCK) {
        float d = delta[i];
        if (HAS_P) d = __builtin_fmaf(alpha, p[i], d);
        X[i] = X[i] + d;
    }
}

__global__ __launch_bounds__(BLOCK) void k_linear_update2(float* __restrict__ X, const float* __restrict__ delta,
                                                           const float* __restrict__ p0, thallo_sum_t aN0, thallo_sum_t aD0,
                                                           const float* __restrict__ p1, thallo_sum_t aN1, thallo_sum_t aD1, long len)
{
    const float a0 = safe_div<false>(sum_partials(aN0.partials, aN0.count), sum_partials(aD0.partials, aD0.count));
    const float a1 = safe_div<false>(sum_partials(aN1.partials, aN1.count), sum_partials(aD1.partials, aD1.count));
    for (long i = (long)blockIdx.x * BLOCK + threadIdx.x; i < len; i += (long)gridDim.x * BLOCK) {
        float d = delta[i];
        d = __builtin_fmaf(a0, p0[i], d);
        d = __builtin_fmaf(a1, p1[i], d);
        X[i] = X[i] + d;
    }
}

template <bool V4>
__global__ __launch_bounds__(BLOCK) void k_linear_update_n(float* __restrict__ X, float* __restrict__ delta, thallo_update_terms_t T, long len)
{
    __shared__ float al[THALLO_HIP_MAX_UPDATE_TERMS];
    for (int j = 0; j < T.count; ++j) {
        const float a = safe_div<false>(sum_partials(T.alphaN[j].partials, T.alphaN[j].count), sum_partials(T.alphaD[j].partials, T.alphaD[j].count));
        if (threadIdx.x == 0) al[j] = a;
    }
    __syncthreads();
    if (V4) {
        const long n4 = len >> 2;
        for (long i = (long)blockIdx.x * BLOCK + threadIdx.x; i < n4; i += (long)gridDim.x * BLOCK) {
            float4 d = reinterpret_cast<const float4*>(delta)[i];
            int j = 0;
            for (; j + 8 <= T.count; j += 8) {
                float4 q[8];
#pragma unroll
                for (int u = 0; u < 8; ++u) q[u] = ldf4(reinterpret_cast<const float4*>(T.p[j + u]) + i, true);
#pragma unroll
                for (int u = 0; u < 8; ++u) {
                    const float a = al[j + u];
                    d.x = __builtin_fmaf(a, q[u].x, d.x); d.y = __builtin_fmaf(a, q[u].y, d.y); d.z = __builtin_fmaf(a, q[u].z, d.z); d.w = __builtin_fmaf(a, q[u].w, d.w);
                }
            }
            for (; j + 4 <= T.count; j += 4) {
                float4 q[4];
#pragma unroll
                for (int u = 0; u < 4; ++u) q[u] = ldf4(reinterpret_cast<const float4*>(T.p[j + u]) + i, true);
#pragma unroll
                for (int u = 0; u < 4; ++u) {
                    const float a = al[j + u];
                    d.x = __builtin_fmaf(a, q[u].x, d.x); d.y = __builtin_fmaf(a, q[u].y, d.y); d.z = __builtin_fmaf(a, q[u].z, d.z); d.w = __builtin_fmaf(a, q[u].w, d.w);
                }
            }
            for (; j < T.count; ++j) {
                const float4 q = ldf4(reinterpret_cast<const float4*>(T.p[j]) + i, true);
                const float a = al[j];
                d.x = __builtin_fmaf(a, q.x, d.x); d.y = __builtin_fmaf(a, q.y, d.y); d.z = __builtin_fmaf(a, q.z, d.z); d.w = __builtin_fmaf(a, q.w, d.w);
            }
            if (X) { float4 x = reinterpret_cast<const float4*>(X)[i]; x.x = x.x + d.x; x.y = x.y + d.y; x.z = x.z + d.z; x.w = x.w + d.w; reinterpret_cast<float4*>(X)[i] = x; }
            else reinterpret_cast<float4*>(delta)[i] = d;
        }
    } else {
        for (long i = (long)blockIdx.x * BLOCK + threadIdx.x; i < len; i += (long)gridDim.x * BLOCK) {
            float d = delta[i];
            for (int j = 0; j < T.count; ++j) d = __builtin_fmaf(al[j], T.p[j][i], d);
            if (X) X[i] = X[i] + d; else delta[i] = d;
        }
    }
}

__global__ __launch_bounds__(BLOCK) void k_slab_pack(const float* __restrict__ vec, thallo_segs_t segs, thallo_sum_t s, float* __restrict__ out)
{
    if (blockIdx.x == 0 && s.count > 0) {
        const float v = sum_partials(s.partials, s.count);
        if (threadIdx.x == 0) out[0] = v;
    }
    long base = 1;
    for (int k = 0; k < segs.n; ++k) {
        for (long i = (long)blockIdx.x * BLOCK + threadIdx.x; i < segs.len[k]; i += (long)gridDim.x * BLOCK) out[base + i] = vec[segs.off[k] + i];
        base += segs.len[k];
    }
}

__global__ __launch_bounds__(BLOCK) void k_slab_unpack(float* __restrict__ vec, thallo_segs_t top, const float* __restrict__ src_top,
                                                        thallo_segs_t bot, const float* __restrict__ src_bot,
                                                        const float* __restrict__ gathered, long stride, int world, float* __restrict__ sum_out)
{
    if (blockIdx.x == 0 && threadIdx.x == 0 && sum_out) {
        float v = 0.0f;
        for (int r = 0; r < world; ++r) v += gathered[(long)r * stride];
        sum_out[0] = v;
    }
    if (src_top) {
        long base = 0;
        for (int k = 0; k < top.n; ++k) {
            for (long i = (long)blockIdx.x * BLOCK + threadIdx.x; i < top.len[k]; i += (long)gridDim.x * BLOCK) vec[top.off[k] + i] = src_top[base + i];
            base += top.len[k];
        }
    }
    if (src_bot) {
        long base = 0;
        for (int k = 0; k < bot.n; ++k) {
            for (long i = (long)blockIdx.x * BLOCK + threadIdx.x; i < bot.len[k]; i += (long)gridDim.x * BLOCK) vec[bot.off[k] + i] = src_bot[base + i];
            base += bot.len[k];
        }
    }
}

template <bool HAS_PRE>
__global__ __launch_bounds__(BLOCK) void k_block_sums(const float4* __restrict__ p, const float4* __restrict__ Ap, const float4* __restrict__ r, const float4* __restrict__ pre,
                                                       long n4, float* __restrict__ aD_out, double* __restrict__ s3_out)
{
    __shared__ float red[16];
    __shared__ double redd[3 * BLOCK / 64];
    float acc = 0.0f; Sums3 sm;
    for (long i = (long)blockIdx.x * BLOCK + threadIdx.x; i < n4; i += (long)gridDim.x * BLOCK) {
        const float4 pv = p[i], av = Ap[i], rv = r[i];
// ... 388 lines not shown
    hipLaunchKernelGGL(k_lm_step1_finish, dim3(grid), dim3(BLOCK), 0, (hipStream_t)stream, (float4*)Ap, (const float4*)CtC, (const float4*)p, n4, aD_out, g_gate);
    int e = check_launch(); return e ? e : grid;
}
int thallo_hip_lm_step2_first_half(float* delta, const float* p, long n, thallo_sum_t aN, thallo_sum_t aD, thallo_stream_t stream)
{
    const long n4 = (n + 3) / 4; const int grid = flat_grid(n4, cu_count());
    hipLaunchKernelGGL(k_lm_step2_first, dim3(grid), dim3(BLOCK), 0, (hipStream_t)stream, (float4*)delta, (const float4*)p, n4, aN, aD, g_gate);
    int e = check_launch(); return e ? e : grid;
}
int thallo_hip_lm_step2_second_half(float* r, const float* b, const float* Adelta, const float* pre, float* z, const float* delta, long n,
                                    float* bN_out, float* q_out, thallo_stream_t stream)
{
    const long n4 = (n + 3) / 4; const int grid = flat_grid(n4, cu_count());
    hipLaunchKernelGGL(k_lm_step2_second, dim3(grid), dim3(BLOCK), 0, (hipStream_t)stream, (float4*)r, (const float4*)b, (const float4*)Adelta,
                       (const float4*)pre, (float4*)z, (const float4*)delta, n4, bN_out, q_out, g_gate);
    int e = check_launch(); return e ? e : grid;
}
int thallo_hip_pcg_init_finish(const float* r, const float* diag, float* pre, float* z, long n, int use_preconditioner,
                               float* aN_out, thallo_stream_t stream)
{
    const long n4 = (n + 3) / 4; const int grid = flat_grid(n4, cu_count());
    hipLaunchKernelGGL(k_init_finish, dim3(grid), dim3(BLOCK), 0, (hipStream_t)stream, (const float4*)r, (const float4*)diag, (float4*)pre, (float4*)z, n4,
                       use_preconditioner, aN_out);
    int e = check_launch(); return e ? e : grid;
}
int thallo_hip_dot(const float* a, const float* b, long n, float* out, thallo_stream_t stream)
{
    const long n4 = (n + 3) / 4; const int grid = flat_grid(n4, cu_count());
    hipLaunchKernelGGL(k_dot, dim3(grid), dim3(BLOCK), 0, (hipStream_t)stream, (const float4*)a, (const float4*)b, n4, out);
    int e = check_launch(); return e ? e : grid;
}

int thallo_hip_linear_update(float* X, const float* delta, const float* p, long len,
                             thallo_sum_t aN, thallo_sum_t aD, thallo_stream_t stream)
{
    const int grid = flat_grid(len, cu_count());
    hipStream_t s = (hipStream_t)stream;
    if (p) hipLaunchKernelGGL(k_linear_update<true>, dim3(grid), dim3(BLOCK), 0, s, X, delta, p, len, aN, aD);
    else   hipLaunchKernelGGL(k_linear_update<false>, dim3(grid), dim3(BLOCK), 0, s, X, delta, p, len, aN, aD);
    int e = check_launch();
    return e ? e : grid;
}

int thallo_hip_linear_update2(float* X, const float* delta, const float* p_older, thallo_sum_t aN0, thallo_sum_t aD0,
                              const float* p, thallo_sum_t aN1, thallo_sum_t aD1, long len, thallo_stream_t stream)
{
    if (!p_older || !p) return -(int)hipErrorInvalidValue;
    const int grid = flat_grid(len, cu_count());
    hipLaunchKernelGGL(k_linear_update2, dim3(grid), dim3(BLOCK), 0, (hipStream_t)stream, X, delta, p_older, aN0, aD0, p, aN1, aD1, len);
    int e = check_launch();
    return e ? e : grid;
}

int thallo_hip_linear_update_n(float* X, float* delta, thallo_update_terms_t terms, long len, int max_workgroups, thallo_stream_t stream)
{
    if (!delta || len < 0 || terms.count < 0 || terms.count > THALLO_HIP_MAX_UPDATE_TERMS) return -(int)hipErrorInvalidValue;
    bool v4 = !(len & 3) && !(((uintptr_t)X | (uintptr_t)delta) & 15);
    for (int j = 0; j < terms.count; ++j) {
        if (!terms.p[j] || !terms.alphaN[j].partials || !terms.alphaD[j].partials || terms.alphaN[j].count < 1 || terms.alphaD[j].count < 1) return -(int)hipErrorInvalidValue;
        if ((uintptr_t)terms.p[j] & 15) v4 = false;
    }
    if (len == 0 || (terms.count == 0 && !X)) return 0;
    int grid = flat_grid(v4 ? len >> 2 : len, 2 * cu_count());
    if (max_workgroups > 0 && grid > max_workgroups) grid = max_workgroups;
    if (v4) hipLaunchKernelGGL(k_linear_update_n<true>, dim3(grid), dim3(BLOCK), 0, (hipStream_t)stream, X, delta, terms, len);
    else    hipLaunchKernelGGL(k_linear_update_n<false>, dim3(grid), dim3(BLOCK), 0, (hipStream_t)stream, X, delta, terms, len);
    int e = check_launch();
    return e ? e : grid;
}

int thallo_hip_finish_sum(thallo_sum_t sum, float* out, thallo_stream_t stream)
{
    hipLaunchKernelGGL(k_finish_sum, dim3(1), dim3(64), 0, (hipStream_t)stream, sum, out);
    return check_launch();
}

int thallo_hip_finish_sum_gated(thallo_sum_t sum, float* out, const unsigned* gate, thallo_stream_t stream)
{
    if (!gate || !out || !sum.partials) return -(int)hipErrorInvalidValue;
    hipLaunchKernelGGL(k_finish_sum_gated, dim3(1), dim3(64), 0, (hipStream_t)stream, sum, out, gate);
    return check_launch();
}

int thallo_hip_slab_pack(const float* vec, thallo_segs_t segs, thallo_sum_t sum, float* out, thallo_stream_t stream)
{
    if (segs.n < 0 || segs.n > 8) return -(int)hipErrorInvalidValue;
    hipLaunchKernelGGL(k_slab_pack, dim3(8), dim3(BLOCK), 0, (hipStream_t)stream, vec, segs, sum, out);
    return check_launch();
}

int thallo_hip_slab_unpack(float* vec, thallo_segs_t top, const float* src_top, thallo_segs_t bot, const float* src_bot,
                           const float* gathered, long stride, int world, float* sum_out, thallo_stream_t stream)
{
    if (top.n < 0 || top.n > 8 || bot.n < 0 || bot.n > 8) return -(int)hipErrorInvalidValue;
    hipLaunchKernelGGL(k_slab_unpack, dim3(8), dim3(BLOCK), 0, (hipStream_t)stream, vec, top, src_top, bot, src_bot, gathered, stride, world, sum_out);
    return check_launch();
}

int thallo_hip_block_sums(const float* p, const float* Ap, const float* r, const float* pre, long n, float* aD_out, double* s3_out, thallo_stream_t stream)
{
    if (!p || !Ap || !r || !aD_out || !s3_out || n < 0 || (n & 3)) return -(int)hipErrorInvalidValue;
    const long n4 = n / 4; const int grid = flat_grid(n4 ? n4 : 1, cu_count());
    if (pre) hipLaunchKernelGGL(k_block_sums<true>, dim3(grid), dim3(BLOCK), 0, (hipStream_t)stream, (const float4*)p, (const float4*)Ap, (const float4*)r, (const float4*)pre, n4, aD_out, s3_out);
    else     hipLaunchKernelGGL(k_block_sums<false>, dim3(grid), dim3(BLOCK), 0, (hipStream_t)stream, (const float4*)p, (const float4*)Ap, (const float4*)r, (const float4*)pre, n4, aD_out, s3_out);
    int e = check_launch(); return e ? e : grid;
}
int thallo_hip_shard_scalars(const float* gathered, long stride, int world, const float* aD_partials, const double* s3_partials, int count, thallo_sum_t alphaN,
                             float* alphaD_word, float* betaN_word, thallo_stream_t stream)
{
    if (!gathered || world < 1 || stride < 1 || !aD_partials || count < 0 || count > THALLO_MAX_PARTIALS || !alphaD_word) return -(int)hipErrorInvalidValue;
    const int only_first = betaN_word == nullptr;
    if (!only_first && (!s3_partials || alphaN.count < 1)) return -(int)hipErrorInvalidValue;
    hipLaunchKernelGGL(k_shard_scalars, dim3(1), dim3(64), 0, (hipStream_t)stream, gathered, stride, world, aD_partials, s3_partials, count, alphaN, only_first, alphaD_word, betaN_word);
    return check_launch();
}

int thallo_hip_range_unpack(float* vec, thallo_segs_t first_rank_pieces, const float* gathered, long stride, long skip, int world, thallo_stream_t stream)
{
    if (!vec || !gathered || first_rank_pieces.n < 1 || first_rank_pieces.n > 8 || world < 1 || stride < 1 || skip < 0) return -(int)hipErrorInvalidValue;
    long len = 0; for (int j = 0; j < first_rank_pieces.n; ++j) len += first_rank_pieces.len[j];
    int grid = (int)((len + BLOCK - 1) / BLOCK); if (grid > 64) grid = 64; if (grid < 1) grid = 1;
    hipLaunchKernelGGL(k_range_unpack, dim3(grid), dim3(BLOCK), 0, (hipStream_t)stream, vec, first_rank_pieces, gathered, stride, skip, world);
// ... 59 lines not shown
```

### thallo_amd/csrc/plugin.hpp

```cpp
#pragma once
#include <hip/hip_runtime.h>
#include <string>
#include <vector>
#include <map>
#include "../../include/thallo_hip.h"

namespace thallo {

void set_error(const char* fmt, ...);
const char* last_error();
const char* env_switch(const char* name);

class KernelTimer {
public:
    struct Stat { std::string name; long launches = 0; long samples = 0; double total_ms = 0; double sq_ms = 0;
                  std::vector<std::pair<hipEvent_t, hipEvent_t>> pending;
                  long ksamples = 0; double ktotal_ms = 0; std::vector<std::pair<hipEvent_t, hipEvent_t>> kpending; };
    int period = 0;
    bool invasive = false;
    ~KernelTimer();
    int  begin(const char* name, hipStream_t s);
    void end(int slot, hipStream_t s);
    void collect();
    void reset();
// ... 32 lines not shown
    double* s12b = nullptr;
    double* s12buf(int i) { return i ? s12b : s12; }
    unsigned* fin_tickets = nullptr;
    float* rbuf(int i) { return i ? r2 : r; }
    float* Abuf(int i) { return i ? Ap2 : Ap; }
};

struct UnknownImage { int param_index; long n_floats; };

struct Vectors64 { long n = 0, n_alloc = 0; double *delta = nullptr, *r = nullptr, *z = nullptr, *Ap = nullptr, *pre = nullptr, *p = nullptr;
                   double* diag = nullptr; };
class EnergyPlugin64 {
public:
    virtual ~EnergyPlugin64() {}
    virtual int cost64(struct LaunchCtx&, double* partials_out) = 0;
    virtual int pcg_init64(struct LaunchCtx&, Vectors64&, double* alphaN_partials) = 0;
    virtual int apply_jtj64(struct LaunchCtx&, Vectors64&, const double* p, double* Ap, double* alphaD_partials) = 0;
    virtual double* unknown_ptr64(int k) = 0;
};

class EnergyPlugin {
public:
    virtual ~EnergyPlugin() {}
    virtual const char* name() const = 0;
    virtual EnergyPlugin64* f64() { return nullptr; }
    virtual const char* schedule_name() const { return "matrix-free"; }
    virtual long n_unknowns() const = 0;
    virtual const std::vector<UnknownImage>& unknown_images() const = 0;
    virtual bool use_preconditioner() const = 0;
    virtual int bind(void** params) = 0;
    virtual int prepare(LaunchCtx&) { return 0; }
    virtual int cost(LaunchCtx&, float* cost_out) = 0;
    virtual int pcg_init(LaunchCtx&, SolverVectors&, int cur, float* alphaN_out) = 0;
    virtual int apply_jtj(LaunchCtx&, const float* p, float* Ap, float* alphaD_out) = 0;
    virtual bool apply_adds_ctc() const { return false; }
    virtual bool lm_one_kernel() const { return false; }
    virtual bool lm_iter_defers_finish() const { return false; }
    virtual bool lm_iter_after_reset() const { return false; }
    virtual int lm_reset_residual(LaunchCtx&, SolverVectors&, float* ) { return -1; }
    virtual bool lm_one_kernel_slab() const { return false; }
    virtual int pcg_iter_lm(LaunchCtx&, SolverVectors&, int , bool , thallo_sum_t , thallo_sum_t , thallo_sum_t , float* ,
                            const thallo_fin_t&, float* , int , float ) { return -1; }
    virtual bool init_folds_lm_diagonal() const { return false; }
    virtual int pcg_init_lm(LaunchCtx&, SolverVectors&, int , float , float , float , int , float* ) { return -1; }
    virtual bool lm_model_cost_one_launch() const { return false; }
    virtual int lm_model_cost(LaunchCtx&, SolverVectors&, const float* , const float* , int , const float* , int ,
                              float* , float* , bool ) { return -1; }
    virtual bool apply_folds_pupdate() const { return false; }
    virtual int apply_jtj_pupdate(LaunchCtx&, const float* , const float* , float* , float* , float* , bool ,
                                  thallo_sum_t , thallo_sum_t ) { return -1; }
    virtual int pcg_step1(LaunchCtx&, SolverVectors&, int cur, bool first,
                          thallo_sum_t aN_prev, thallo_sum_t aD_prev, thallo_sum_t bN_prev, float* alphaD_out) = 0;
    virtual bool batches_delta() const { return false; }
    virtual bool takes_any_p_plane() const { return false; }
    virtual bool persist_ok() const { return false; }
    virtual int pcg_persist(struct LaunchCtx&, SolverVectors&, float* const* planes, int n_planes, int k0, int k1, float* parts, int slots, int B, int nb_prev, thallo_sum_t alphaN_prev) { return -1; }
    virtual int pcg_step1_mode(LaunchCtx& c, SolverVectors& v, int cur, int mode, thallo_sum_t aN_prev, thallo_sum_t aD_prev, thallo_sum_t bN_prev,
                               thallo_sum_t, thallo_sum_t, float* alphaD_out)
    { return pcg_step1(c, v, cur, (mode & 1) != 0, aN_prev, aD_prev, bN_prev, alphaD_out); }
    virtual bool apply_returns_sums() const { return false; }
    virtual int apply_jtj_sums(LaunchCtx&, SolverVectors&, const float* , float* , float* , const thallo_fin_t& ) { return -1; }
    virtual bool one_kernel_iteration() const { return false; }
    virtual bool dist_flat_form() const { return !one_kernel_iteration(); }
    virtual bool one_kernel_slab() const { return false; }
    virtual int pcg_iter(LaunchCtx&, SolverVectors&, int , int , thallo_sum_t, thallo_sum_t, thallo_sum_t, thallo_sum_t, thallo_sum_t, float* ,
                         float* , float* ) { return -1; }
    virtual int pcg_iter_finish(LaunchCtx&, SolverVectors&, const float* , int , thallo_sum_t , float* , float* ) { return -1; }
    virtual bool iter_defers_finish() const { return false; }
    virtual int pcg_iter_deferred(LaunchCtx&, SolverVectors&, int , int , thallo_sum_t , thallo_sum_t , thallo_sum_t ,
                                  const thallo_prev_t& , float* , double* ) { return -1; }
    virtual int pcg_iter_finish_from(LaunchCtx&, const float* , const double* , int , thallo_sum_t ,
                                     float* , float* ) { return -1; }
    virtual bool resident_ok() const { return false; }
    virtual int  pcg_resident(LaunchCtx&, SolverVectors&, int , thallo_sum_t , float* ) { return -1; }
    virtual bool resident_updates_unknowns() const { return false; }
    virtual bool resident_lm_ok() const { return false; }
    virtual int  pcg_resident_lm(LaunchCtx&, SolverVectors&, int , thallo_sum_t , float* , float* , float , float* , float* ) { return -1; }
    virtual int  resident_status(LaunchCtx&, int , unsigned* ) { return 0; }
    virtual void resident_disable() {}
    virtual bool dist_defers_finish() const { return false; }
    virtual int  pcg_iter_dist_deferred(LaunchCtx&, SolverVectors&, int , int , thallo_sum_t , thallo_sum_t , thallo_sum_t , thallo_sum_t , thallo_sum_t ,
                                        const thallo_prev_t& , int , unsigned long long* , const thallo_dist_t&, float* , double* ) { return -1; }
    virtual int  pcg_iter_dist_finish(LaunchCtx&, const thallo_prev_t& , int , thallo_sum_t , const thallo_dist_t&, unsigned long long* ) { return -1; }
    virtual bool dist_batches_delta() const { return false; }
    virtual bool resident_slab_ok() const { return false; }
    virtual long resident_ghost_bytes() const { return 0; }
    virtual int  pcg_resident_dist(LaunchCtx&, SolverVectors&, int , thallo_sum_t , float* , const thallo_dist_t&, long , int ) { return -1; }
    virtual int pcg_step2(LaunchCtx& c, SolverVectors& v, thallo_sum_t aN, thallo_sum_t aD, float* betaN_out)
    {
        TimedLaunch t(c, "PCGStep2");
        return thallo_hip_pcg_step2(v.r, v.Ap, use_preconditioner() ? v.pre : nullptr, v.z, v.n, aN, aD, betaN_out, c.stream);
    }
    virtual float* unknown_ptr(int k) = 0;
    virtual void unknowns_changed() {}
    virtual void unknowns_written() { unknowns_changed(); }
    virtual void forbid_renumbering() {}
    virtual bool direct_solve() const { return false; }
    virtual int  solve_direct(LaunchCtx&, SolverVectors&) { return -1; }
    virtual bool supports_row_slabs() const { return false; }
    virtual int  set_row_slab(int , int ) { return -1; }
    virtual int  slab_ghost_rows() const { return 1; }
    virtual bool slab_returns_sums() const { return apply_returns_sums(); }
    virtual bool slab_setup_ok() const { return true; }
    virtual const char* slab_setup_error() const { return ""; }
    virtual int  set_slab_global(int , int ) { return 0; }
    virtual int  slab_width() const { return 0; }
// ... 35 lines not shown
```

### thallo_amd/csrc/plugins.cpp

```cpp
#include "plugin.hpp"
#ifdef THALLO_RESEARCH
#include "probe/thallo_hip_research.h"
#endif
#include <algorithm>
#include <cstdio>
#include <cstring>
#include <cstdlib>

namespace thallo {

int DeviceBuffer::alloc(size_t n)
{
    release();
    if (n == 0) return 0;
    hipError_t e = hipMalloc(&ptr, n);
    if (e != hipSuccess) { ptr = nullptr; set_error("hipMalloc(%zu) failed: %s", n, hipGetErrorString(e)); return -(int)e; }
    bytes = n;
    e = hipMemset(ptr, 0, n);
    return e == hipSuccess ? 0 : -(int)e;
}
void DeviceBuffer::release() { if (ptr) { hipFree(ptr); ptr = nullptr; bytes = 0; } }

struct HostCsr {
    int rows = 0, cols = 0;
// ... 83 lines not shown
        if (!mat_mode || mat.mode) return 0;
        HostCsr j; j.begin(W * H);
        for (int y = 0; y < H; ++y) for (int x = 0; x < W; ++x) { j.add(y * W + x, w_fit); j.end_row(); }
        for (int y = 0; y < H; ++y) for (int x = 0; x < W; ++x) {
            const int i = y * W + x;
            if (x + 1 < W && (xguard || y + 1 < H)) { j.add(i, 1.0f); j.add(i + 1, -1.0f); }
            j.end_row();
            if (y + 1 < H) { j.add(i, 1.0f); j.add(i + W, -1.0f); }
            j.end_row();
        }
        return mat.build(j, mat_mode);
    }
    const char* name() const override { return "laplacian_image"; }
    long n_unknowns() const override { return (long)W * H; }
    const std::vector<UnknownImage>& unknown_images() const override { return imgs; }
    bool use_preconditioner() const override { return false; }
    int bind(void** p) override { X = (float*)p[0]; A = (const float*)p[1]; return (X && A) ? 0 : -1; }
    float* unknown_ptr(int) override { return X; }
    int cost(LaunchCtx& c, float* out) override
    { TimedLaunch t(c, "computeCost"); return thallo_hip_lapimg_cost(W, H, X, A, w_fit, xguard, out, c.stream); }
    int pcg_init(LaunchCtx& c, SolverVectors& v, int cur, float* aN) override
    { TimedLaunch t(c, "PCGInit1"); return thallo_hip_lapimg_pcg_init(W, H, X, A, w_fit, xguard, v.r, v.z, v.p[cur], v.delta, v.diag, aN, c.stream); }
    int apply_jtj(LaunchCtx& c, const float* p, float* Ap, float* out) override
    {
        if (mat.mode) return mat.apply(c, p, Ap, out);
        TimedLaunch t(c, "PCGStep1"); return thallo_hip_lapimg_apply_jtj(W, H, w_fit, xguard, p, Ap, out, c.stream);
    }
    int pcg_step1(LaunchCtx& c, SolverVectors& v, int cur, bool first, thallo_sum_t aN, thallo_sum_t aD, thallo_sum_t bN, float* out) override
    {
        if (mat.mode) {
            { TimedLaunch t(c, "PCGStep3"); int rc = thallo_hip_pcg_pupdate(v.z, v.p[cur], v.p[cur ^ 1], v.delta, v.n, first ? 1 : 0, aN, aD, bN, c.stream); if (rc < 0) return rc; }
            return mat.apply(c, v.p[cur ^ 1], v.Ap, out);
        }
        TimedLaunch t(c, "PCGStep1"); return thallo_hip_lapimg_pcg_step1(W, H, w_fit, xguard, v.z, v.p[cur], v.p[cur ^ 1], v.delta, v.Ap, first ? 1 : 0, aN, aD, bN, out, c.stream);
    }
};

class ImageWarpingPlugin : public EnergyPlugin {
    int W, H;
    std::vector<UnknownImage> imgs;
    float *offset = nullptr, *angle = nullptr;
    const float *urshape = nullptr, *constraints = nullptr, *mask = nullptr;
    float w_fit = 0, w_reg = 0;
    DeviceBuffer cs, flags, irregular;
    DeviceBuffer xres;
    bool resident_ = false;
    bool resident_slab_ = false;
    bool resident_broken_ = false;
    bool march_ = false;
    DeviceBuffer xpst;
    bool persist_ = false;
    bool march_rc_ = false;
    bool grid_ = false;
    int row0_ = 0, row1_ = 0;
public:
    ImageWarpingPlugin(const unsigned* dims) : W((int)dims[0]), H((int)dims[1]), row1_((int)dims[1])
    {
        const long N = (long)W * H;
        imgs.push_back({ 0, 2 * N }); imgs.push_back({ 1, N });
    }
    const char* name() const override { return "image_warping"; }
    long n_unknowns() const override { return 3L * W * H; }
    const std::vector<UnknownImage>& unknown_images() const override { return imgs; }
    bool use_preconditioner() const override { return true; }
    int bind(void** p) override
    {
        offset = (float*)p[0]; angle = (float*)p[1]; urshape = (const float*)p[2];
        constraints = (const float*)p[3]; mask = (const float*)p[4];
        if (!offset || !angle || !urshape || !constraints || !mask || !p[5] || !p[6]) { set_error("image_warping: null problem parameter"); return -1; }
        w_fit = *(const float*)p[5]; w_reg = *(const float*)p[6];
        const long N = (long)W * H;
        if (!cs.ptr) { if (cs.alloc(N * 8)) return -1; if (flags.alloc((N + 255) / 256 * 256)) return -1; if (irregular.alloc(64)) return -1; }
        return 0;
    }
    int prepare(LaunchCtx& c) override
    {
        march_ = grid_ = march_rc_ = false;
        const char* e = env_switch("THALLO_MARCH");
        int* word = (int*)irregular.ptr + 8;
        int rc = thallo_hip_iw_urshape_irregular(W, H, urshape, word, c.stream);
        if (rc < 0) { set_error("image_warping: UrShape check failed (%d)", rc); return -1; }
        int bad = 1;
        if (hipMemcpyAsync(&bad, word, sizeof(int), hipMemcpyDeviceToHost, c.stream) != hipSuccess || hipStreamSynchronize(c.stream) != hipSuccess) return -1;
        grid_ = bad == 0;
        if ((e && e[0] == '0') || (W & 1)) return 0;
        march_ = grid_ && ((long)W * H >= 400000 || (e && (e[0] == '2' || e[0] == '4')));
        if (march_ && thallo_hip_iw_march_rows(W, H) <= 0) march_ = false;
        march_rc_ = march_ && !(e && (e[0] == '3' || e[0] == '4')) && 12.0 * (double)W * (double)H < 4294967296.0;
        resident_ = resident_slab_ = false;
        const char* er = env_switch("THALLO_RESIDENT");
        const bool whole = row0_ == 0 && row1_ == H;
        const int rr = whole ? thallo_hip_iw_resident_rows(W, H) : thallo_hip_iw_resident_rows_slab(W, row1_ - row0_, row1_ < H ? 1 : 0);
        if (grid_ && !(er && er[0] == '0') && rr > 0 && !resident_broken_) {
            const long need = thallo_hip_iw_resident_bytes(W, row1_ - row0_);
            if (need > 0 && (long)xres.bytes < need) {
                if (xres.alloc((size_t)need) || hipMemsetAsync(xres.ptr, 0, (size_t)need, c.stream) != hipSuccess) { set_error("image_warping: out of device memory for the resident kernel's exchange buffers"); return -1; }
            }
            if (need > 0) { resident_ = whole; resident_slab_ = true; }
        }
        persist_ = false;
#ifdef THALLO_RESEARCH
        const char* ep = env_switch("THALLO_PERSIST");
        if (march_rc_ && whole && !resident_broken_ && ep && ep[0] == '1' && thallo_hip_iw_march_persist_rows(W, H) > 0) {
            const long need = thallo_hip_iw_march_persist_bytes();
            if ((long)xpst.bytes < need && xpst.alloc((size_t)need)) { set_error("image_warping: out of device memory for the persistent loop's exchange buffer"); return -1; }
            persist_ = true;
        }
#endif
        return 0;
    }
    bool supports_row_slabs() const override { return true; }
    int set_row_slab(int row0, int row1) override
    {
        if (row0 < 0 || row1 > H || row0 >= row1 || (W & 3)) { set_error("image_warping: row slab [%d,%d) of %d rows, W = %d (W %% 4 must be 0)", row0, row1, H, W); return -1; }
        row0_ = row0; row1_ = row1; return 0;
    }
    int slab_width() const override { return W; }
    bool slab_grid_ok() const override { return grid_; }
    unsigned char* slab_flags() override { return (unsigned char*)flags.ptr; }
    int pcg_iter_dist(LaunchCtx& c, SolverVectors& v, int cur, int mode, thallo_sum_t aN, thallo_sum_t aD, thallo_sum_t bN, thallo_sum_t aN2, thallo_sum_t aD2,
                      const thallo_dist_t& d, float* out, int slot0, float* aD_word, float* bN_word) override
    {
        TimedLaunch t(c, "PCGIteration");
        if (march_rc_ && !(mode & 1))
            return thallo_hip_iw_pcg_iter_march_rc_dist(W, H, row0_, row1_, (const float*)cs.ptr, (const unsigned char*)flags.ptr, w_fit, w_reg,
                                                        v.rbuf(cur), v.rbuf(cur ^ 1), v.Abuf(cur), v.Abuf(cur ^ 1), v.p[cur], v.p[cur ^ 1], v.delta, mode,
                                                        aN, aD, bN, aN2, aD2, (const int*)irregular.ptr, d, out, v.s12, v.fin_tickets, slot0, aD_word, bN_word, c.stream);
        if (march_)
            return thallo_hip_iw_pcg_iter_march_dist(W, H, row0_, row1_, (const float*)cs.ptr, (const unsigned char*)flags.ptr, w_fit, w_reg,
                                                     v.rbuf(cur), v.rbuf(cur ^ 1), v.Abuf(cur), v.Abuf(cur ^ 1), v.p[cur], v.p[cur ^ 1], v.delta, mode,
                                                     aN, aD, bN, aN2, aD2, (const int*)irregular.ptr, d, out, v.s12, v.fin_tickets, slot0, aD_word, bN_word, c.stream);
        return thallo_hip_iw_pcg_iter_dist(W, H, row0_, row1_, (const float*)cs.ptr, urshape, (const unsigned char*)flags.ptr, v.pre, w_fit, w_reg,
                                           v.rbuf(cur), v.rbuf(cur ^ 1), v.Abuf(cur), v.Abuf(cur ^ 1), v.p[cur], v.p[cur ^ 1], v.delta, mode,
                                           aN, aD, bN, aN2, aD2, (const int*)irregular.ptr, d, out, v.s12, v.fin_tickets, slot0, aD_word, bN_word, c.stream);
    }
    bool dist_defers_finish() const override { return march_rc_ && march_ && thallo_hip_iw_march_rc_deferred_fits(W, row1_ - row0_) != 0; }
    int pcg_iter_dist_deferred(LaunchCtx& c, SolverVectors& v, int cur, int mode, thallo_sum_t aN, thallo_sum_t aD, thallo_sum_t bN, thallo_sum_t aN2, thallo_sum_t aD2,
                               const thallo_prev_t& prev, int prev_slot0, unsigned long long* gs, const thallo_dist_t& d, float* out, double* s12_out) override
    {
        TimedLaunch t(c, "PCGIteration");
        if (mode & 1)
            return thallo_hip_iw_pcg_iter_march_dist(W, H, row0_, row1_, (const float*)cs.ptr, (const unsigned char*)flags.ptr, w_fit, w_reg,
                                                     v.rbuf(cur), v.rbuf(cur ^ 1), v.Abuf(cur), v.Abuf(cur ^ 1), v.p[cur], v.p[cur ^ 1], v.delta, mode,
                                                     aN, aD, bN, aN2, aD2, (const int*)irregular.ptr, d, out, s12_out, nullptr, 0, nullptr, nullptr, c.stream);
        return thallo_hip_iw_pcg_iter_march_rc_dist_deferred(W, H, row0_, row1_, (const float*)cs.ptr, (const unsigned char*)flags.ptr, w_fit, w_reg,
                                                             v.rbuf(cur), v.rbuf(cur ^ 1), v.Abuf(cur), v.Abuf(cur ^ 1), v.p[cur], v.p[cur ^ 1], v.delta, mode,
                                                             aN, aN2, aD2, prev, prev_slot0, gs, (const int*)irregular.ptr, d, out, s12_out, c.stream);
    }
    int pcg_iter_dist_finish(LaunchCtx& c, const thallo_prev_t& prev, int prev_slot0, thallo_sum_t aN, const thallo_dist_t& d, unsigned long long* gs) override
    { TimedLaunch t(c, "PCGScalars"); return thallo_hip_iw_dist_finish_deferred(prev, prev_slot0, aN, d, gs, c.stream); }
    float* unknown_ptr(int k) override { return k == 0 ? offset : angle; }
    int cost(LaunchCtx& c, float* out) override
    { TimedLaunch t(c, "computeCost"); return thallo_hip_iw_cost(W, H, row0_, row1_, offset, angle, urshape, constraints, mask, w_fit, w_reg, out, c.stream); }
    int pcg_init(LaunchCtx& c, SolverVectors& v, int cur, float* aN) override
    {
        TimedLaunch t(c, "PCGInit1");
        return thallo_hip_iw_pcg_init(W, H, row0_, row1_, offset, angle, urshape, constraints, mask, w_fit, w_reg,
                                      v.r, v.pre, v.z, v.p[cur], v.delta, (float*)cs.ptr, (unsigned char*)flags.ptr, v.diag, (int*)irregular.ptr, aN, c.stream);
    }
    int apply_jtj(LaunchCtx& c, const float* p, float* Ap, float* out) override
    {
        TimedLaunch t(c, "PCGStep1");
        return thallo_hip_iw_apply_jtj(W, H, row0_, row1_, (const float*)cs.ptr, urshape, (const unsigned char*)flags.ptr, w_fit, w_reg, p, Ap, (const int*)irregular.ptr, out, c.stream);
    }
    int pcg_step1(LaunchCtx& c, SolverVectors& v, int cur, bool first, thallo_sum_t aN, thallo_sum_t aD, thallo_sum_t bN, float* out) override
    {
        TimedLaunch t(c, "PCGStep1");
        const thallo_sum_t none = { nullptr, 0 };
        return thallo_hip_iw_pcg_step1(W, H, row0_, row1_, (const float*)cs.ptr, urshape, (const unsigned char*)flags.ptr, w_fit, w_reg,
                                       v.z, v.p[cur], v.p[cur ^ 1], v.delta, v.Ap, first ? 1 : 0, aN, aD, bN, none, none, (const int*)irregular.ptr, v.r, out, c.stream);
    }
    bool batches_delta() const override { return true; }
    bool takes_any_p_plane() const override { return march_; }
    bool persist_ok() const override { return persist_; }
#ifdef THALLO_RESEARCH
    int pcg_persist(LaunchCtx& c, SolverVectors& v, float* const* planes, int n_planes, int k0, int k1, float* parts, int slots, int B, int nb_prev, thallo_sum_t alphaN_prev) override
    {
        TimedLaunch t(c, "PCGLoopPersistent");
        return thallo_hip_iw_pcg_march_persist(W, H, (const float*)cs.ptr, (const unsigned char*)flags.ptr, w_fit, w_reg, v.rbuf(0), v.rbuf(1), planes, n_planes, k0, k1,
                                               parts, slots, B, v.s12, v.s12b, nb_prev, alphaN_prev, (const int*)irregular.ptr, xpst.ptr, c.stream);
    }
#endif
    bool dist_batches_delta() const override { return march_rc_; }
    bool one_kernel_iteration() const override { return true; }
    int pcg_iter(LaunchCtx& c, SolverVectors& v, int cur, int mode, thallo_sum_t aN, thallo_sum_t aD, thallo_sum_t bN, thallo_sum_t aN2, thallo_sum_t aD2, float* out,
                 float* aD_word, float* bN_word) override
    {
        TimedLaunch t(c, "PCGIteration");
        if (march_rc_ && !(mode & 1))
            return thallo_hip_iw_pcg_iter_march_rc(W, H, row0_, row1_, (const float*)cs.ptr, (const unsigned char*)flags.ptr, w_fit, w_reg,
                                                   v.rbuf(cur), v.rbuf(cur ^ 1), v.Abuf(cur), v.Abuf(cur ^ 1), v.p[cur], v.p[cur ^ 1], v.delta, mode,
                                                   aN, aD, bN, aN2, aD2, (const int*)irregular.ptr, out, v.s12,
                                                   aD_word ? v.fin_tickets : nullptr, aD_word, bN_word, c.stream);
        if (march_)
            return thallo_hip_iw_pcg_iter_march(W, H, row0_, row1_, (const float*)cs.ptr, (const unsigned char*)flags.ptr, w_fit, w_reg,
                                                v.rbuf(cur), v.rbuf(cur ^ 1), v.Abuf(cur), v.Abuf(cur ^ 1), v.p[cur], v.p[cur ^ 1], v.delta, mode,
                                                aN, aD, bN, aN2, aD2, (const int*)irregular.ptr, out, v.s12,
                                                aD_word ? v.fin_tickets : nullptr, aD_word, bN_word, c.stream);
        return thallo_hip_iw_pcg_iter(W, H, row0_, row1_, (const float*)cs.ptr, urshape, (const unsigned char*)flags.ptr, v.pre, w_fit, w_reg,
                                      v.rbuf(cur), v.rbuf(cur ^ 1), v.Abuf(cur), v.Abuf(cur ^ 1), v.p[cur], v.p[cur ^ 1], v.delta, mode,
                                      aN, aD, bN, aN2, aD2, (const int*)irregular.ptr, out, v.s12,
                                      aD_word ? v.fin_tickets : nullptr, aD_word, bN_word, c.stream);
    }
    int pcg_iter_finish(LaunchCtx& c, SolverVectors& v, const float* part, int count, thallo_sum_t aN, float* aD_word, float* bN_word) override
    {
        TimedLaunch t(c, "PCGScalars");
        return thallo_hip_iw_pcg_iter_finish(part, v.s12, count, aN, aD_word, bN_word, c.stream);
    }
    bool resident_ok() const override { return resident_; }
    int pcg_resident(LaunchCtx& c, SolverVectors& v, int L, thallo_sum_t aN0, float* words) override
    {
        TimedLaunch t(c, "PCGLoopResident");
        return thallo_hip_iw_pcg_resident(W, H, row0_, row1_, (const float*)cs.ptr, (const unsigned char*)flags.ptr, w_fit, w_reg, v.rbuf(0), v.p[0],
                                          v.rbuf(L & 1), v.Abuf(L & 1), v.p[L & 1], v.delta, aN0, words, (const int*)irregular.ptr,
                                          resident_updates_unknowns() ? offset : nullptr, resident_updates_unknowns() ? angle : nullptr, xres.ptr, L, c.stream);
    }
    bool resident_updates_unknowns() const override { const char* e = env_switch("THALLO_IW_RESIDENT_FOLD"); return resident_ && !(e && e[0] == '0'); }
    bool resident_slab_ok() const override { return resident_slab_; }
    long resident_ghost_bytes() const override { return (W & 1) ? 0 : thallo_hip_iw_resident_ghost_bytes(W); }
    int pcg_resident_dist(LaunchCtx& c, SolverVectors& v, int L, thallo_sum_t aN0, float* words, const thallo_dist_t& d, long ghost_off, int slot0) override
    {
        if (!resident_slab_) return -(int)hipErrorNotSupported;
        TimedLaunch t(c, "PCGLoopResident");
        return thallo_hip_iw_pcg_resident_dist(W, H, row0_, row1_, (const float*)cs.ptr, (const unsigned char*)flags.ptr, w_fit, w_reg, v.rbuf(0), v.p[0],
                                               v.rbuf(L & 1), v.Abuf(L & 1), v.p[L & 1], v.delta, aN0, words, (const int*)irregular.ptr, xres.ptr, d, ghost_off, slot0, L, c.stream);
    }
    int resident_status(LaunchCtx& c, int clear, unsigned* pm) override
    {
        const int a = xres.ptr ? thallo_hip_iw_resident_status(xres.ptr, clear, -1, pm, c.stream) : 0;
#ifdef THALLO_RESEARCH
        if (a == 0 && xpst.ptr) return thallo_hip_iw_march_persist_status(xpst.ptr, clear, -1, pm, c.stream);
#endif
        return a;
    }
    void resident_disable() override { resident_ = resident_slab_ = persist_ = false; resident_broken_ = true; }
    bool iter_defers_finish() const override { return true; }
    int pcg_iter_deferred(LaunchCtx& c, SolverVectors& v, int cur, int mode, thallo_sum_t aN, thallo_sum_t aN2, thallo_sum_t aD2, const thallo_prev_t& prev,
                          float* out, double* s12_out) override
    {
        TimedLaunch t(c, "PCGIteration");
        if (march_rc_ && !(mode & 1))
            return thallo_hip_iw_pcg_iter_march_rc_deferred(W, H, row0_, row1_, (const float*)cs.ptr, (const unsigned char*)flags.ptr, w_fit, w_reg,
                                                            v.rbuf(cur), v.rbuf(cur ^ 1), v.Abuf(cur), v.Abuf(cur ^ 1), v.p[cur], v.p[cur ^ 1], v.delta, mode,
                                                            aN, aN2, aD2, prev, (const int*)irregular.ptr, out, s12_out, c.stream);
        if (march_)
            return thallo_hip_iw_pcg_iter_march_deferred(W, H, row0_, row1_, (const float*)cs.ptr, (const unsigned char*)flags.ptr, w_fit, w_reg,
                                                         v.rbuf(cur), v.rbuf(cur ^ 1), v.Abuf(cur), v.Abuf(cur ^ 1), v.p[cur], v.p[cur ^ 1], v.delta, mode,
                                                         aN, aN2, aD2, prev, (const int*)irregular.ptr, out, s12_out, c.stream);
        return thallo_hip_iw_pcg_iter_deferred(W, H, row0_, row1_, (const float*)cs.ptr, urshape, (const unsigned char*)flags.ptr, v.pre, w_fit, w_reg,
                                               v.rbuf(cur), v.rbuf(cur ^ 1), v.Abuf(cur), v.Abuf(cur ^ 1), v.p[cur], v.p[cur ^ 1], v.delta, mode,
                                               aN, aN2, aD2, prev, (const int*)irregular.ptr, out, s12_out, c.stream);
    }
    int pcg_iter_finish_from(LaunchCtx& c, const float* part, const double* s12p, int count, thallo_sum_t aN, float* aD_word, float* bN_word) override
    {
        TimedLaunch t(c, "PCGScalars");
        return thallo_hip_iw_pcg_iter_finish(part, s12p, count, aN, aD_word, bN_word, c.stream);
    }
    int pcg_step1_mode(LaunchCtx& c, SolverVectors& v, int cur, int mode, thallo_sum_t aN, thallo_sum_t aD, thallo_sum_t bN,
                       thallo_sum_t aN2, thallo_sum_t aD2, float* out) override
    {
        TimedLaunch t(c, "PCGStep1");
        return thallo_hip_iw_pcg_step1(W, H, row0_, row1_, (const float*)cs.ptr, urshape, (const unsigned char*)flags.ptr, w_fit, w_reg,
                                       v.z, v.p[cur], v.p[cur ^ 1], v.delta, v.Ap, mode, aN, aD, bN, aN2, aD2, (const int*)irregular.ptr, v.r, out, c.stream);
    }
    int pcg_step2(LaunchCtx& c, SolverVectors& v, thallo_sum_t aN, thallo_sum_t aD, float* out) override
    {
        TimedLaunch t(c, "PCGStep2");
        return thallo_hip_iw_pcg_step2(W, H, row0_, row1_, (const unsigned char*)flags.ptr, w_fit, w_reg, v.r, v.Ap, v.pre, v.z, aN, aD, (const int*)irregular.ptr, out, c.stream);
    }
};

struct GraphIncidence {
    int N = 0, E = 0;
    DeviceBuffer out_ptr, out_v1, in_ptr, in_edge, in_src;
    long ell_stride = 0;
    int in_slots = 1;
    const int* bound_v0 = nullptr; const int* bound_v1 = nullptr;
    std::vector<int> wg_list; int wg_ghosts = 0;
    void build_wg_ghost_lists(const std::vector<int>& v0, const std::vector<int>& v1, int cap)
    {
        const int nwg = (N + 255) / 256, W = 4 + cap;
        std::vector<std::vector<int>> need(nwg);
        for (int e = 0; e < E; ++e) { const int a = v0[e] / 256, b = v1[e] / 256; if (a != b) { need[a].push_back(v1[e]); need[b].push_back(v0[e]); } }
        wg_list.assign((size_t)W * nwg, 0); wg_ghosts = 0;
        for (int w = 0; w < nwg; ++w) {
            std::vector<int>& s = need[w];
            std::sort(s.begin(), s.end()); s.erase(std::unique(s.begin(), s.end()), s.end());
            wg_ghosts = std::max(wg_ghosts, (int)s.size());
            const int n = std::min((int)s.size(), cap);
            wg_list[(size_t)W * w] = n;
            std::copy(s.begin(), s.begin() + n, wg_list.begin() + (size_t)W * w + 4);
        }
    }
    static int read_edges(int N, int E, const int* d_v0, const int* d_v1, std::vector<int>& v0, std::vector<int>& v1)
// ... 723 lines not shown
```

### thallo_amd/csrc/solver.cpp

```cpp
#include "solver.hpp"
#include <stdlib.h>
#include <cmath>
#include <cstdarg>
#include <cstdio>
#include <cstring>

namespace thallo {

static thread_local char g_err[512] = "";
void set_error(const char* fmt, ...)
{
    va_list ap; va_start(ap, fmt); vsnprintf(g_err, sizeof(g_err), fmt, ap); va_end(ap);
    fprintf(stderr, "[thallo] error: %s\n", g_err);
}
const char* last_error() { return g_err; }

#define HIP_OK(call) do { hipError_t e__ = (call); if (e__ != hipSuccess) set_error("%s failed: %s", #call, hipGetErrorString(e__)); } while (0)

hipEvent_t KernelTimer::get_event()
{
    if (!pool_.empty()) { hipEvent_t e = pool_.back(); pool_.pop_back(); return e; }
    hipEvent_t e = nullptr; HIP_OK(hipEventCreate(&e)); return e;
}
int KernelTimer::begin(const char* name, hipStream_t s)
// ... 143 lines not shown
    if (ensure_slots(sp.lIterations)) return;
    ok_ = true;
}

Plan::~Plan()
{
    hipDeviceSynchronize();
    if (host_words_) { hipHostFree(host_words_); host_words_ = nullptr; }
    for (hipEvent_t e : aux_events_) hipEventDestroy(e);
    if (aux_) hipStreamDestroy(aux_);
    dist_release();
    if (rccl_) { rccl_comm_destroy(rccl_); rccl_ = nullptr; }
    for (auto b : bufs_) delete b;
    delete plugin;
}

int Plan::ensure_slots(int L)
{
    const int need = 2 * L + 6;
    if (need <= parts_slots_) return 0;
    hipDeviceSynchronize();
    if (parts_.alloc(((size_t)need * THALLO_HIP_MAX_PARTIALS + (size_t)need + 64) * sizeof(float))) { set_error("out of device memory for %d reduction slots (lIterations too large?)", need); return -1; }
    parts_slots_ = need; nb_.assign(need, 1); fin_.assign(need, 0);
    read_ab_switches();
    return 0;
}

const char* env_switch(const char* name)
{
    static const char* const known[] = {
        "THALLO_RESIDENT",
        "THALLO_MARCH",
        "THALLO_DELTA_PLANES",
        "THALLO_DIST_P2P",
        "THALLO_FRONTEND",
        "THALLO_DENSE_JTJ_MAX",
        "THALLO_ENABLE_DIRECT_SOLVE",
    };
    static const char* const ab[][2] = {
        { "THALLO_ONE_KERNEL", "one_kernel" },
        { "THALLO_FIN_IN_KERNEL", "fin_in_kernel" },
        { "THALLO_LM_FOLD_P", "lm_fold_p" },
        { "THALLO_SFS_FUSED", "sfs_fused" },
        { "THALLO_SFS_MARCH", "sfs_march" },
        { "THALLO_BA_RENUMBER", "ba_renumber" },
        { "THALLO_LM_FOLD_STEP", "lm_fold_step" },
        { "THALLO_IW_RESIDENT_FOLD", "iw_resident_fold" },
        { "THALLO_SFS_RESIDENT_FOLD", "sfs_resident_fold" },
        { "THALLO_SFS_PAIR", "sfs_pair" },
        { "THALLO_FRONTEND_AGGREGATE", "frontend_aggregate" },
        { "THALLO_FRONTEND_COMPUTED", "frontend_computed" },
        { "THALLO_FRONTEND_PRELOAD", "frontend_preload" },
        { "THALLO_INC_LANES", "inc_lanes" },
        { "THALLO_PERSIST", "persist" },
    };
    for (const char* k : known) if (!strcmp(k, name)) return getenv(name);
    for (size_t i = 0; i < sizeof(ab) / sizeof(ab[0]); ++i) {
        if (strcmp(ab[i][0], name)) continue;
        static std::string slot[sizeof(ab) / sizeof(ab[0])];
        const char* e = getenv("THALLO_AB");
        if (!e) return nullptr;
        const size_t kl = strlen(ab[i][1]);
        for (const char* t = e; *t; ) {
            while (*t == ',' || *t == ' ') ++t;
            const char* end = t; while (*end && *end != ',' && *end != ' ') ++end;
            if ((size_t)(end - t) > kl && !strncmp(t, ab[i][1], kl) && t[kl] == '=') { slot[i].assign(t + kl + 1, end); return slot[i].c_str(); }
            t = end;
        }
        return nullptr;
    }
    set_error("internal: unknown environment switch %s", name);
    return nullptr;
}

void Plan::read_ab_switches()
{
    auto off = [](const char* name) { const char* e = env_switch(name); return e && e[0] == '0'; };
    one_kernel_    = !off("THALLO_ONE_KERNEL");
    fin_in_kernel_ = !off("THALLO_FIN_IN_KERNEL");
    { const char* e = env_switch("THALLO_FIN_IN_KERNEL"); fin_deferred_ = !(e && e[0]); }
    { const char* e = env_switch("THALLO_DELTA_PLANES"); delta_planes_ = e && e[0] ? atoi(e) : -1; if (delta_planes_ > THALLO_HIP_MAX_UPDATE_TERMS + 1) delta_planes_ = THALLO_HIP_MAX_UPDATE_TERMS + 1;
      if (delta_planes_ < -(THALLO_HIP_MAX_UPDATE_TERMS + 1)) delta_planes_ = -(THALLO_HIP_MAX_UPDATE_TERMS + 1);
      const char* c = e ? strchr(e, ':') : nullptr; aux_async_ = c != nullptr; aux_workgroups_ = c && atoi(c + 1) > 0 ? atoi(c + 1) : 0; }
    batch_delta_   = delta_planes_ != 0;
    lm_fold_p_     = !off("THALLO_LM_FOLD_P");
    lm_fold_step_  = !off("THALLO_LM_FOLD_STEP");
}

void Plan::set_param(const char* name, const void* value)
{
#define SETF(f) if (!strcmp(name, #f)) { sp.f = *(const float*)value; return; }
#define SETI(f) if (!strcmp(name, #f)) { sp.f = *(const int*)value; return; }
    SETF(min_relative_decrease) SETF(min_trust_region_radius) SETF(max_trust_region_radius) SETF(q_tolerance)
    SETF(function_tolerance) SETF(trust_region_radius) SETF(radius_decrease_factor) SETF(min_lm_diagonal)
    SETF(max_lm_diagonal) SETF(max_solver_time_in_seconds)
    SETI(residual_reset_period) SETI(nIter) SETI(nIterations) SETI(lIterations)
#undef SETF
#undef SETI
    if (ip.verbosityLevel > 0) printf("Warning: tried to set nonexistent solver parameter %s\n", name);
}
void Plan::get_param(const char* name, void* value)
{
#define GETF(f) if (!strcmp(name, #f)) { *(float*)value = sp.f; return; }
#define GETI(f) if (!strcmp(name, #f)) { *(int*)value = sp.f; return; }
    GETF(min_relative_decrease) GETF(min_trust_region_radius) GETF(max_trust_region_radius) GETF(q_tolerance)
    GETF(function_tolerance) GETF(trust_region_radius) GETF(radius_decrease_factor) GETF(min_lm_diagonal)
// ... 96 lines not shown
{
    if (!ok_ || !ready_) return 0;
    if (plugin->bind(params)) {
        if (dist_) dist_fail("%s: parameter binding failed", plugin->name());
        else { set_error("%s: parameter binding failed", plugin->name()); return 0; }
    }
    if (!lm_) plugin->unknowns_changed();
    if (sp.nIter >= sp.nIterations) { if (!finalized_) finalize(); return 0; }
    if (sp.lIterations < 0) { set_error("lIterations = %d is negative", sp.lIterations); if (!finalized_) finalize(); return 0; }
    if (ensure_slots(sp.lIterations)) {
        if (dist_) dist_fail("out of device memory for the reduction slots");
        else { if (!finalized_) finalize(); return 0; }
    }
    const int ev_iter = timer_.start("Nonlinear Iteration", ctx.stream);
    if (dist_ && lm_ && !dist_->runs_lm()) { set_error("distributed: %s runs Gauss-Newton only across ranks", plugin->name()); if (!finalized_) finalize(); return 0; }
    const int rc = lm_ && dist_ && dist_->form == DistForm::Shard ? step_lm_shard(ev_iter) : lm_ ? step_lm(ev_iter) : dist_ ? step_gn_slab(ev_iter) : step_gn(ev_iter);
    if (rc == 1 && sp.max_solver_time_in_seconds > 0.0f && ev_total_ >= 0) {
        hipStream_t s = ctx.stream;
        hipEvent_t q = nullptr; hipEventCreate(&q); hipEventRecord(q, s); hipEventSynchronize(q);
        float ms = 0.0f; hipEventElapsedTime(&ms, timer_.events[ev_total_].start, q); hipEventDestroy(q);
        if (ms / 1000.0f > sp.max_solver_time_in_seconds) { finalize(); return 0; }
    }
    return rc;
}

void Plan::linear_update_tail(int L, bool batched)
{
    const int B = 2;
    hipStream_t s = ctx.stream;
    const auto& imgs = plugin->unknown_images();
    const int jN = B + 2 * (L - 1), jD = jN + 1;
    long off = 0;
    for (size_t k = 0; k < imgs.size(); ++k) {
        TimedLaunch t(ctx, "PCGLinearUpdate");
        const long lo = owned_range(k).lo, len = owned_range(k).len;
        float* X = plugin->unknown_ptr((int)k) + lo;
        const float* dl = v_.delta + off + lo;
        if (L > 1 && batched && ((L - 1) & 1))
            thallo_hip_linear_update2(X, dl, v_.p[cur_ ^ 1] + off + lo, sum(jN - 2), sum(jD - 2), v_.p[cur_] + off + lo, sum(jN), sum(jD), len, s);
        else if (L > 0) thallo_hip_linear_update(X, dl, v_.p[cur_] + off + lo, len, sum(jN), sum(jD), s);
        else            thallo_hip_linear_update(X, dl, nullptr, len, sum(B), sum(B), s);
        off += imgs[k].n_floats;
    }
    plugin->unknowns_written();
}
Plan::Owned Plan::owned_range(size_t u) const
{
    const long n = plugin->unknown_images()[u].n_floats;
    if (!dist_ || dist_->full_vectors()) return { 0, n };
    const long rowlen = n / dist_->Hl;
    return { rowlen * dist_->row0, rowlen * (dist_->row1 - dist_->row0) };
}

bool Plan::gn_begin(int& ev_lin)
{
    hipStream_t s = ctx.stream;
    const int ev_setup = timer_.start("Nonlinear Setup", s);
    cur_ = 0;
    const int nb = plugin->pcg_init(ctx, v_, cur_, slot(2));
    if (nb < 0) { set_error("PCGInit1 launch failed (%d)", nb); return false; }
    set_nb(2, nb); finish(2);
    timer_.stop(ev_setup, s);
    ev_lin = timer_.start("Linear Solve", s);
    return true;
}
int Plan::gn_finish(int L, int ev_lin)
{
    last_l_iters = L;
    timer_.stop(ev_lin, ctx.stream);
    return timer_.start("Nonlinear Finish", ctx.stream);
}
int Plan::gn_end(int ev_fin, int ev_iter)
{
    sp.nIter++;
    timer_.stop(ev_fin, ctx.stream);
    timer_.stop(ev_iter, ctx.stream);
    return 1;
}

int Plan::step_gn(int ev_iter)
{
    if (plugin->direct_solve()) {
        hipStream_t s = ctx.stream;
        cur_ = 0;
        const int nb = plugin->pcg_init(ctx, v_, cur_, slot(2));
        if (nb < 0) { set_error("PCGInit1 launch failed (%d)", nb); return 0; }
        set_nb(2, nb);
        const int ev_lin = timer_.start("Linear Solve", s);
        if (plugin->solve_direct(ctx, v_) < 0) { const std::string why = last_error(); set_error("direct solve failed: %s", why.c_str()); return 0; }
        timer_.stop(ev_lin, s);
        last_l_iters = 0;
        linear_update_tail(0, false);
        sp.nIter++;
        timer_.stop(ev_iter, s);
        return 1;
    }
    if (one_kernel_ && sp.lIterations >= 1 && plugin->resident_ok()) return step_gn_resident(ev_iter);
    if (one_kernel_ && plugin->one_kernel_iteration()) return step_gn_one_kernel(ev_iter);
    if (plugin->apply_returns_sums()) return step_gn_expanded(ev_iter);
    const int L = sp.lIterations, B = 2;
    int ev_lin, nb;
    if (!gn_begin(ev_lin)) return 0;
    const bool batched = plugin->batches_delta() && batch_delta_;
    for (int k = 0; k < L; ++k) {
        const int jN = B + 2 * k, jD = jN + 1, jB = jN + 2;
        const PrevAlpha a = prev_alpha(k);
        if (batched) nb = plugin->pcg_step1_mode(ctx, v_, cur_, THALLO_IW_STEP1_MODE(k, 1), a.aN, a.aD, sum(jN), a.aN2, a.aD2, slot(jD));
        else         nb = plugin->pcg_step1(ctx, v_, cur_, k == 0, a.aN, a.aD, sum(jN), slot(jD));
        if (nb < 0) { set_error("PCGStep1 launch failed (%d)", nb); return 0; }
        set_nb(jD, nb); finish(jD); cur_ ^= 1;
        nb = plugin->pcg_step2(ctx, v_, sum(jN), sum(jD), slot(jB));
        if (nb < 0) { set_error("PCGStep2 launch failed (%d)", nb); return 0; }
        set_nb(jB, nb); finish(jB);
    }
    const int ev_fin = gn_finish(L, ev_lin);
    linear_update_tail(L, batched);
    return gn_end(ev_fin, ev_iter);
}

void Plan::enable_lm(bool on) { lm_ = on; }
void Plan::unknowns_changed()
{
    if (!ok_ || !ready_) return;
    plugin->unknowns_changed();
    if (lm_ && !finalized_) prev_cost_ = compute_cost();
}

int Plan::ensure_lm_vectors()
{
    if (v_.b) return 0;
    float** vecs[] = { &v_.b, &v_.Adelta, &v_.CtC, &v_.SSq, &v_.prevX, &v_.diag };
    for (float** vp : vecs) {
        DeviceBuffer* b = new DeviceBuffer(); bufs_.push_back(b);
        if (b->alloc((size_t)v_.n_alloc * sizeof(float))) return -1;
        *vp = (float*)b->ptr;
    }
    return 0;
}

Plan::GnSchedule Plan::gn_schedule(int L, int n_ring)
{
    const bool defer = plugin->iter_defers_finish();
    if (n_ring >= 2 && defer && L >= 2 && plugin->persist_ok()) return GnSchedule::Persist;
    return defer ? GnSchedule::Deferred : GnSchedule::FinishInLaunch;
}

int Plan::step_gn_one_kernel(int ev_iter)
{
    if (ensure_iter_buffers()) { set_error("out of device memory for the one-kernel schedule"); return 0; }
    const int L = sp.lIterations;
    int ev_lin;
    if (!gn_begin(ev_lin)) return 0;
    const int n_ring = ring_planes(L);
    const GnSchedule sched = gn_schedule(L, n_ring);
    const bool async = n_ring >= 2 && aux_async_ && sched != GnSchedule::Persist && aux_stream();
    GnStep st{ L, n_ring < 2 && batch_delta_ && delta_planes_ != 0 && plugin->batches_delta(), PRing(*this, n_ring, async) };
    bool done = false;
    switch (sched) {
    case GnSchedule::Persist:        done = gn_loop_persist(st); break;
    case GnSchedule::Deferred:       done = gn_loop_deferred(st, L); break;
    case GnSchedule::FinishInLaunch: done = gn_loop_finish_in_launch(st); break;
    }
    if (!done) return 0;
    const int ev_fin = gn_finish(L, ev_lin);
    if (st.ring.on() && L > 0) {
        if (ring_flush(st.ring, L - 1 - THALLO_HIP_MAX_UPDATE_TERMS) || st.ring.wait_for(L)) { set_error("PCGDeltaUpdate launch failed"); return 0; }
        if (!ring_linear_update(st.ring, L, [](int rc) { return rc >= 0; })) { set_error("PCGLinearUpdate launch failed"); return 0; }
        plugin->unknowns_written();
    } else linear_update_tail(L, st.batched);
    return gn_end(ev_fin, ev_iter);
}

int Plan::gn_launch_mode(GnStep& st, int k)
{
    PRing& R = st.ring;
    if (!R.on()) return THALLO_IW_STEP1_MODE(k, st.batched ? 1 : 0);
    if (ring_flush(R, R.flush_due(k))) { set_error("PCGDeltaUpdate launch failed"); return -1; }
    if (R.wait_to_overwrite(k)) { set_error("PCGDeltaUpdate: stream wait failed"); return -1; }
    return R.launch(k, cur_);
}

bool Plan::gn_loop_deferred(GnStep& st, int k_end)
{
    for (int k = 0; k < k_end; ++k) {
        const int jN = 2 + 2 * k, jD = jN + 1, jB = jN + 2;
        const int mode = gn_launch_mode(st, k);
        if (mode < 0) return false;
        const PrevAlpha a = prev_alpha(k);
        const thallo_prev_t prev = { k ? slot(jD - 2) : nullptr, v_.s12buf((k - 1) & 1), st.nb_prev, k ? scal(jD - 2) : nullptr, k ? scal(jB - 2) : nullptr };
        const int nb = plugin->pcg_iter_deferred(ctx, st.ring.vectors(), cur_, mode, a.aN, a.aN2, a.aD2, prev, slot(jD), v_.s12buf(k & 1));
        if (nb < 0) { set_error("PCGIteration launch failed (%d)", nb); return false; }
        if (k) words_done(k - 1);
        set_nb(jD, nb); st.nb_prev = nb; cur_ ^= 1;
        if (k == st.L - 1 && !gn_finish_last(st, k, nb)) return false;
    }
    return true;
}
bool Plan::gn_finish_last(GnStep& st, int k, int nb)
{
    const int jN = 2 + 2 * k, jD = jN + 1, jB = jN + 2;
    if (plugin->pcg_iter_finish_from(ctx, slot(jD), v_.s12buf(k & 1), nb, sum(jN), scal(jD), scal(jB)) < 0) { set_error("PCGScalars launch failed"); return false; }
    words_done(k);
    return true;
}

bool Plan::gn_loop_persist(GnStep& st)
{
    PRing& R = st.ring;
    const int L = st.L, B = 2, n = R.n;
    if (!gn_loop_deferred(st, 1)) return false;
    for (int k = 1; k < L; ) {
        const int m = L - k < n - 1 ? L - k : n - 1, k1 = k + m;
        if (k1 - 1 >= n && R.flushed < k1 - n) { if (ring_flush(R, k - 2) || R.wait_for(k - 2)) { set_error("PCGDeltaUpdate launch failed"); return false; } }
        const int nb = plugin->pcg_persist(ctx, v_, ring_.data(), n, k, k1, slot(0), parts_slots_, B, st.nb_prev, sum(B + 2 * (k - 1)));
        if (nb < 0) { set_error("PCGLoopPersistent launch failed (%d)", nb); return false; }
        resident_used_ = true;
        for (int i = k; i < k1; ++i) words_done(i - 1);
        set_nb(B + 2 * (k1 - 1) + 1, nb); st.nb_prev = nb;
        if (m & 1) cur_ ^= 1;
        k = k1;
        if (k == L && !gn_finish_last(st, L - 1, nb)) return false;
    }
    return true;
}

bool Plan::gn_loop_finish_in_launch(GnStep& st)
{
    for (int k = 0; k < st.L; ++k) {
        const int jN = 2 + 2 * k, jD = jN + 1, jB = jN + 2;
        const int mode = gn_launch_mode(st, k);
        if (mode < 0) return false;
        const PrevAlpha a = prev_alpha(k);
        const int nb = plugin->pcg_iter(ctx, st.ring.vectors(), cur_, mode, a.aN, a.aD, sum(jN), a.aN2, a.aD2, slot(jD),
                                        fin_in_kernel_ ? scal(jD) : nullptr, fin_in_kernel_ ? scal(jB) : nullptr);
        if (nb < 0) { set_error("PCGIteration launch failed (%d)", nb); return false; }
        set_nb(jD, nb); cur_ ^= 1;
        if (!fin_in_kernel_ && plugin->pcg_iter_finish(ctx, v_, slot(jD), nb, sum(jN), scal(jD), scal(jB)) < 0) { set_error("PCGScalars launch failed"); return false; }
        words_done(k);
    }
    return true;
}

bool Plan::PRing::next_batch(int upto, thallo_update_terms_t& T)
{
    T.count = 0;
    for (; flushed <= upto && T.count < THALLO_HIP_MAX_UPDATE_TERMS; ++flushed) {
        T.p[T.count] = plane(flushed); T.alphaN[T.count] = P.sum(2 + 2 * flushed); T.alphaD[T.count] = P.sum(2 + 2 * flushed + 1); ++T.count;
    }
    return T.count > 0;
}
bool Plan::PRing::events(hipEvent_t& words, hipEvent_t& done)
{
    std::vector<hipEvent_t>& ev = P.aux_events_;
    while (n_ev + 2 > ev.size()) { hipEvent_t e = nullptr; if (hipEventCreateWithFlags(&e, hipEventDisableTiming) != hipSuccess) return false; ev.push_back(e); }
    words = ev[n_ev++]; done = ev[n_ev++];
    return true;
}
int Plan::PRing::wait_for(int term)
{
    for (const Sent& q : sent) {
        if (q.upto < synced) continue;
        if (hipStreamWaitEvent(P.ctx.stream, q.done, 0) != hipSuccess) return -1;
        synced = q.upto + 1;
        if (q.upto >= term) break;
    }
    return 0;
}
int Plan::ring_flush(PRing& R, int upto)
{
    hipStream_t s = ctx.stream;
    thallo_update_terms_t T;
    while (R.next_batch(upto, T)) {
        if (!R.async) {
            TimedLaunch t(ctx, "PCGDeltaUpdate");
            if (thallo_hip_linear_update_n(nullptr, v_.delta, T, v_.n_alloc, 0, s) < 0) return -1;
            R.synced = R.flushed;
            continue;
        }
        hipEvent_t words, done;
        if (!R.events(words, done)) return -1;
        if (hipEventRecord(words, s) != hipSuccess || hipStreamWaitEvent(aux_, words, 0) != hipSuccess) return -1;
        LaunchCtx cx = ctx; cx.stream = aux_;
        {   TimedLaunch t(cx, "PCGDeltaUpdate");
            if (thallo_hip_linear_update_n(nullptr, v_.delta, T, v_.n_alloc, aux_workgroups_ > 0 ? aux_workgroups_ : thallo_hip_device_cu_count(), aux_) < 0) return -1; }
        if (hipEventRecord(done, aux_) != hipSuccess) return -1;
        R.sent.push_back(PRing::Sent{ R.flushed - 1, done });
    }
    return 0;
}

bool Plan::aux_stream()
{
    if (aux_) return true;
    if (aux_failed_) return false;
    int lo = 0, hi = 0;
    if (hipDeviceGetStreamPriorityRange(&lo, &hi) != hipSuccess) lo = 0;
    if (hipStreamCreateWithPriority(&aux_, hipStreamNonBlocking, lo) != hipSuccess) { aux_ = nullptr; aux_failed_ = true; (void)hipGetLastError(); return false; }
    return true;
}

bool Plan::ring_possible() const
{
    return plugin->takes_any_p_plane() && (!dist_ || dist_->form == DistForm::Slab);
}
int Plan::ring_wanted(int L) const
{
    if (!ring_possible() || delta_planes_ == 0 || delta_planes_ == 1 || L < 3) return 0;
    const int want = delta_planes_ >= 2 ? delta_planes_ : delta_planes_ <= -2 ? -delta_planes_ : THALLO_HIP_MAX_UPDATE_TERMS + 1;
    return want > L ? L : want;
}
void Plan::ring_prepare(int L)
{
    const int want = ring_wanted(L);
    if (!want) return;
    if (ring_.size() < 2) { ring_.clear(); ring_.push_back(v_.p[1]); ring_.push_back(v_.p[0]); }
    if (want <= (int)ring_.size() || want <= ring_tried_) return;
    ring_tried_ = want;
    const size_t bytes = (size_t)v_.n_alloc * sizeof(float);
    while ((int)ring_.size() < want) {
        size_t free_b = 0, total_b = 0;
        if (delta_planes_ == -1 && (hipMemGetInfo(&free_b, &total_b) != hipSuccess || bytes > free_b / 4 / (size_t)(want - (int)ring_.size()) ||
                                  bytes * (ring_.size() - 1) > ((size_t)32 << 30))) break;
        void* ptr = nullptr;
        if (hipMalloc(&ptr, bytes) != hipSuccess) { (void)hipGetLastError(); break; }
        if (hipMemsetAsync(ptr, 0, bytes, ctx.stream) != hipSuccess) { (void)hipGetLastError(); hipFree(ptr); break; }
        DeviceBuffer* b = new DeviceBuffer(); b->ptr = ptr; b->bytes = bytes;
        bufs_.push_back(b); ring_.push_back((float*)ptr);
    }
}
int Plan::ring_planes(int L)
{
    const int want = ring_wanted(L);
    if (!want) return 0;
    if (L != ring_L_) { ring_prepare(L); ring_L_ = L; }
    if (ring_.size() < 2) return 0;
    const int n = (int)ring_.size() < want ? (int)ring_.size() : want;
    return n >= 3 || want == 2 ? n : 0;
// ... 473 lines not shown
```

### thallo_amd/csrc/solver.hpp

```cpp
#pragma once
#include "plugin.hpp"
#include "rccl_transport.hpp"
#include "../../include/Thallo.h"

namespace thallo {

struct SolverParameters {
    float min_relative_decrease = 1e-3f;
    float min_trust_region_radius = 1e-32f;
    float max_trust_region_radius = 1e16f;
    float q_tolerance = 0.0001f;
    float function_tolerance = 0.000001f;
    float trust_region_radius = 1e4f;
    float radius_decrease_factor = 2.0f;
    float min_lm_diagonal = 1e-6f;
    float max_lm_diagonal = 1e32f;
    float max_solver_time_in_seconds = 0.0f;
    int residual_reset_period = 10;
    int nIter = 0;
    int nIterations = 10;
    int lIterations = 10;
};

class CoarseTimer {
// ... 93 lines not shown
    const char* distributed_info() const { return dist_ ? dist_->info.c_str() : ""; }
    void rccl_info(int out[3]);
    int  dist_control(int what, int value);
    int  dist_kernel_only(int reps);

    EnergyPlugin* plugin;
    SolverParameters sp;
    Thallo_InitializationParameters ip;
    Thallo_PerformanceSummary summary;
    LaunchCtx ctx;
    KernelTimer ktimer;
    std::vector<float> ab_trace;
    int last_l_iters = 0;
    unsigned* dims;

private:
    bool ok_ = false;
    bool ready_ = false;
    bool lm_ = false;
    bool finalized_ = true;
    float prev_cost_ = 0.0f;
    SolverVectors v_;
    std::vector<DeviceBuffer*> bufs_;
    DeviceBuffer parts_;
    int parts_slots_ = 0;
    DeviceBuffer scratch_;
    DeviceBuffer trace_;
    std::vector<int> nb_;
    CoarseTimer timer_;
    float* host_words_ = nullptr;
    int ev_total_ = -1;
    int cur_ = 0;

    float* slot(int j) { return (float*)parts_.ptr + (size_t)j * THALLO_HIP_MAX_PARTIALS; }
    std::vector<char> fin_;
    bool fin_in_kernel_ = true, one_kernel_ = true, batch_delta_ = true, lm_fold_p_ = true, lm_fold_step_ = true;
    int delta_planes_ = -1;
    std::vector<float*> ring_;
    bool ring_possible() const;
    int  ring_wanted(int L) const;
    int  ring_planes(int L);
    void ring_prepare(int L);
    int  ring_tried_ = 0, ring_L_ = -1;
    struct PRing {
        Plan& P;
        const int n;
        const bool async;
        int flushed = 0;
        int synced = 0;
        struct Sent { int upto; hipEvent_t done; };
        std::vector<Sent> sent;
        size_t n_ev = 0;
        SolverVectors v;
        PRing(Plan& plan, int planes, bool on_second_stream) : P(plan), n(planes), async(on_second_stream), v(plan.v_) {}
        PRing(const PRing&) = delete;
        ~PRing() { if (!sent.empty()) (void)hipStreamWaitEvent(P.ctx.stream, sent.back().done, 0); }
        bool on() const { return n >= 2; }
        SolverVectors& vectors() { return on() ? v : P.v_; }
        float* plane(int k) const { return k < 0 ? P.v_.p[0] : P.ring_[(size_t)(k % n)]; }
        int  launch(int k, int cur) { v.p[cur] = plane(k - 1); v.p[cur ^ 1] = plane(k); return k == 0 ? 1 : 2; }
        int  flush_due(int k) const { const int chunk = (n - 1) / 2 > 0 ? (n - 1) / 2 : 1; return (async ? k - 1 - flushed >= chunk : (k >= n && flushed < k - n + 1)) ? k - 2 : -1; }
        bool next_batch(int upto, thallo_update_terms_t& T);
        bool events(hipEvent_t& words, hipEvent_t& done);
        int  wait_for(int term);
        int  wait_to_overwrite(int k) { return k >= n && synced < k - n + 1 ? wait_for(k - n) : 0; }
    };
    int  ring_flush(PRing& R, int upto);
    struct Owned { long lo, len; };
    Owned owned_range(size_t u) const;
    template <class Launched> bool ring_linear_update(PRing& R, int L, Launched launched);
    hipStream_t aux_ = nullptr; bool aux_failed_ = false;
    std::vector<hipEvent_t> aux_events_;
    bool aux_async_ = false;
    int aux_workgroups_ = 0;
    bool aux_stream();
    bool fin_deferred_ = true;
    void read_ab_switches();
    float* scal(int j) { return (float*)parts_.ptr + (size_t)parts_slots_ * THALLO_HIP_MAX_PARTIALS + j; }
    thallo_sum_t partial_sum(int j) { thallo_sum_t s; s.partials = slot(j); s.count = nb_[j]; return s; }
    thallo_sum_t sum(int j) { if (fin_[j]) { thallo_sum_t s; s.partials = scal(j); s.count = 1; return s; } return partial_sum(j); }
    void set_nb(int j, int nb) { nb_[j] = nb; fin_[j] = 0; }
    void finish(int j) { if (nb_[j] <= 256) return; thallo_hip_finish_sum(partial_sum(j), scal(j), ctx.stream); fin_[j] = 1; }
    void words_done(int k) { const int jD = 2 + 2 * k + 1, jB = jD + 1; fin_[jD] = 1; set_nb(jB, 1); fin_[jB] = 1; }
    struct PrevAlpha { thallo_sum_t aN, aD, aN2, aD2; };
    PrevAlpha prev_alpha(int k) { const int jN = 2 + 2 * k, jD = jN + 1; return { sum(k ? jN - 2 : jN), sum(k ? jD - 2 : jD), sum(k > 1 ? jN - 4 : jN), sum(k > 1 ? jD - 4 : jD) }; }
    int  ensure_slots(int L);
    int  ensure_iter_buffers();
    int  ensure_sums_buffer();
    int  step_gn_expanded(int ev_iter);
    enum class GnSchedule { Persist, Deferred, FinishInLaunch };
    struct GnStep {
        const int L;
        const bool batched;
        PRing ring;
        int nb_prev = 0;
    };
    int  step_gn_one_kernel(int ev_iter);
    GnSchedule gn_schedule(int L, int n_ring);
    int  gn_launch_mode(GnStep& st, int k);
    bool gn_finish_last(GnStep& st, int k, int nb);
    bool gn_loop_persist(GnStep& st);
    bool gn_loop_deferred(GnStep& st, int k_end);
    bool gn_loop_finish_in_launch(GnStep& st);
    int  step_gn_resident(int ev_iter);
    bool gn_begin(int& ev_lin);
    int  gn_finish(int L, int ev_lin);
    int  gn_end(int ev_fin, int ev_iter);
    bool resident_used_ = false;
    float compute_cost();
    float* host_words();
    int   step_gn(int ev_iter);
    enum class LmSchedule { Reference, OneKernel, OneKernelSlab, Resident };
    struct GateOff {
        LaunchCtx& c;
        GateOff(LaunchCtx& ctx, const unsigned* gate) : c(ctx) { thallo_hip_lm_set_gate(gate); c.gate = gate; }
        void off() { thallo_hip_lm_set_gate(nullptr); c.gate = nullptr; }
        ~GateOff() { off(); }
    };
    struct LmStep {
        Plan& P;
        hipStream_t s;
        int L, T0, T1, period;
        static constexpr int B = 2, QS = 1;
        bool slab;
        long o, n, oe, ne;
        bool pc, fold_ctc, fold_init;
        float* lmst;
        const unsigned* gate;
        int ev_iter, ev_lin = -1;
        int k_done = 0;
        bool model_cost_done = false;
        bool failed = false;
        bool coll_failed = false;
        LmStep(Plan& plan, int ev_iter);
        bool skip() const { return failed || (slab && P.dist_->failed); }
        void check(int rc, const char* what);
        int  global(int j) { return slab ? P.dist_sum_slot(j) : 0; }
        int  global_rows(int j, float* vec) { return slab ? P.dist_sum_and_rows(j, vec) : 0; }
    };
    int   step_lm(int ev_iter);
    bool  lm_setup(LmStep& st);
    LmSchedule lm_schedule(const LmStep& st);
    void  lm_loop_reference(LmStep& st);
    void  lm_loop_one_kernel(LmStep& st);
    void  lm_loop_one_kernel_slab(LmStep& st);
    void  lm_loop_resident(LmStep& st);
    int   lm_finish(LmStep& st);
    bool  lm_agree_all();
    int   lm_accept_or_revert(float dJJd, float db, float newCost, int k_done, int ev_fin, int ev_iter);
    int   step_lm_shard(int ev_iter);
    void  lm_trust_region_at_start() { if (sp.nIter == 0) { radius_ = sp.trust_region_radius; decrease_factor_ = sp.radius_decrease_factor; } }
    hipError_t copy_unknowns(bool restore);
    static int lm_iterations_done(const float* rep, int enqueued);
    int   ensure_lm_vectors();
    float read_sum(int j);
    float radius_ = 1e4f, decrease_factor_ = 2.0f;
    void finalize();
    void linear_update_tail(int L, bool batched);
// ... 15 lines not shown
    void dist_partition_upload(const int* counts, const thallo_units_t& planes, long per_unit, bool& lists_ok, bool& mem_ok);
    void dist_render_info();
    int  dist_exchange_mail(long bytes, bool same_bytes, DistPeerInfo& mine, DistPeerInfo* infos, bool& ok);
    int  dist_agree_mapped(bool ok);
    int  dist_map_peers();
    int  dist_map_mail(long bytes);
    int  dist_self_check(), dist_check_units(), dist_check_allreduce(), dist_check_rows(), dist_check_slab();
    void dist_check_begin(), dist_check_read_error();
    int  dist_check_finish(bool pass, float* scratch, size_t scratch_floats, bool xrows);
    template <class Fill, class Exchange, class Verify> int dist_check_pattern(float* vec, size_t n, bool with_sum, bool xrows, Fill fill, Exchange exchange, Verify verify);
    int  dist_allgather(const void* send, void* recv, long bytes);
    int  dist_agree(bool flag, bool& all);
    void dist_fail(const char* fmt, ...);
    bool dist_skip() const { return dist_ && dist_->failed; }
    int  dist_xrows_lm(float* vec, int jN, int jD, int jB, int nb, float* lm_state, int k);
    int  dist_two_sums_and_rows(int j1, int j2, float* vec, float* zeta_state = nullptr, int zeta_k = 0, bool* zeta_done = nullptr);
    int  dist_xrows(float* vec, bool rows, int mode, thallo_sum_t s, const float* aD_part, const double* s3, int nb, float* out0, float* out1, float* zeta_state = nullptr, int zeta_k = 0);
    int  dist_sum_slot(int j);
    int  dist_sum_and_rows(int j, float* vec);
    int  dist_exchange_unknown_rows();
    int  dist_replicate(float* vec, int sum_slot);
    int  dist_ghosts(float* vec, int sum_slot);
    int  dist_allreduce(float* buf, long count);
    int  step_gn_slab(int ev_iter);
    int  dist_gn(int L, bool p2p);
    int  dist_gn_begin(bool p2p);
    int  dist_agree_defer();
    void dist_ring_flush(PRing& R, int upto);
    int  dist_launch_mode(PRing& R, int k, bool batch);
    void dist_gn_loop_resident(int L);
    void dist_gn_loop_deferred(int L, PRing& R, bool batch);
    void dist_gn_loop_p2p(int L, PRing& R, bool batch);
    int  dist_gn_loop_allgather(int L, PRing& R, bool batch);
    int  dist_allgather_iter(float* Ap, int k, int nb);
    int  dist_gn_flat(int L);
    int  dist_gn_flat_loop_one_launch(int L), dist_gn_flat_loop_three_launch(int L);
    int  dist_flat_exchange_iter(float* Ap, int k, int nb);
    int  dist_gn_range(int L);
    int  dist_gn_shard(int L);
    float dist_cost();
    void dist_release();
};

template <class Launched> bool Plan::ring_linear_update(PRing& R, int L, Launched launched)
{
    thallo_update_terms_t T; T.count = 0;
    for (int j = R.flushed; j < L; ++j) { T.p[T.count] = R.plane(j); T.alphaN[T.count] = sum(2 + 2 * j); T.alphaD[T.count] = sum(2 + 2 * j + 1); ++T.count; }
    long off = 0;
    for (size_t u = 0; u < plugin->unknown_images().size(); ++u) {
        TimedLaunch t(ctx, "PCGLinearUpdate");
        const Owned o = owned_range(u);
        thallo_update_terms_t Tu = T;
        for (int j = 0; j < Tu.count; ++j) Tu.p[j] += off + o.lo;
        if (!launched(thallo_hip_linear_update_n(plugin->unknown_ptr((int)u) + o.lo, v_.delta + off + o.lo, Tu, o.len, 0, ctx.stream))) return false;
        off += plugin->unknown_images()[u].n_floats;
    }
    return true;
}

}
```

Baseline: 17790.

## Add lean first PCG iteration path skipping zero-state writes and reads

Adds a lean init kernel variant that skips writing pre, z, p_prev and delta when the ring schedule is used. The first march_rc iteration is specialized (FIRST template) to skip loading p, the JtJ product, alpha/beta scalars and the beta term, since p_prev is zero. The delta update uses a 'first' variant that starts from zero instead of reading delta. This cuts memory traffic in the first iteration of each linear solve, at the cost of more template instantiations and more fragile invariants about zero-initialised state.

```diff
diff --git a/include/thallo_hip.h b/include/thallo_hip.h
--- a/include/thallo_hip.h
+++ b/include/thallo_hip.h
@@ -103,6 +103,7 @@
 #define THALLO_HIP_MAX_UPDATE_TERMS 32
 typedef struct { const float* p[THALLO_HIP_MAX_UPDATE_TERMS]; thallo_sum_t alphaN[THALLO_HIP_MAX_UPDATE_TERMS], alphaD[THALLO_HIP_MAX_UPDATE_TERMS]; int count; } thallo_update_terms_t;
 int thallo_hip_linear_update_n(float* X, float* delta, thallo_update_terms_t terms, long len, int max_workgroups , thallo_stream_t stream);
+int thallo_hip_linear_update_n_first(float* X, float* delta, thallo_update_terms_t terms, long len, int max_workgroups, thallo_stream_t stream);
 int thallo_hip_wave64_selftest(unsigned long long* out_ballot, unsigned* out_peers, float* sums4);
 int thallo_hip_finish_sum(thallo_sum_t s, float* out, thallo_stream_t stream);
 int thallo_hip_finish_sum_gated(thallo_sum_t s, float* out, const unsigned* gate, thallo_stream_t stream);
diff --git a/thallo_amd/api.py b/thallo_amd/api.py
--- a/thallo_amd/api.py
+++ b/thallo_amd/api.py
@@ -25,6 +25,10 @@
 
 class SumT(C.Structure):
     _fields_ = [("partials", C.c_void_p), ("count", C.c_int)]
+
+
+class UpdateTermsT(C.Structure):
+    _fields_ = [("p", C.c_void_p * 32), ("alphaN", SumT * 32), ("alphaD", SumT * 32), ("count", C.c_int)]
 
 
 class DistT(C.Structure):
@@ -121,6 +125,9 @@
     _march = [ci, ci, ci, ci, vp, vp, fl, fl, vp, vp, vp, vp, vp, vp, vp, ci, SumT, SumT, SumT, SumT, SumT, vp]
     L.thallo_hip_iw_pcg_iter_march.argtypes = _march + [vp, vp, vp, vp, vp, vp]
     L.thallo_hip_iw_pcg_iter_march_dist.argtypes = _march + [DistT, vp, vp, vp, ci, vp, vp, vp]
+    L.thallo_hip_iw_pcg_iter_march_rc.argtypes = _march + [vp, vp, vp, vp, vp, vp]
+    L.thallo_hip_linear_update_n.argtypes = [vp, vp, UpdateTermsT, cl, ci, vp]
+    L.thallo_hip_linear_update_n_first.argtypes = [vp, vp, UpdateTermsT, cl, ci, vp]
     L.thallo_hip_iw_urshape_irregular.argtypes = [ci, ci, vp, vp, vp]
     L.thallo_hip_march_debug_set.argtypes = [ci, ci]
     L.thallo_hip_iw_pcg_iter_finish.argtypes = [vp, vp, ci, SumT, vp, vp, vp]
@@ -372,7 +379,8 @@
     if L < 1:
         return 0.0
     if ring:
-        return (69.0 + 57.0 * (L - 1)) / L
+        first_rc = dict(t.split("=", 1) for t in os.environ.get("THALLO_AB", "").replace(" ", ",").split(",") if "=" in t).get("iw_first_rc", "1")[:1] != "0"
+        return ((45.0 if first_rc else 69.0) + 57.0 * (L - 1)) / L
     if every_iteration_delta:
         return (69.0 + 81.0 * (L - 1)) / L
     odd, even = L // 2, (L - 1) // 2
diff --git a/thallo_amd/csrc/energy_image_warping.hip b/thallo_amd/csrc/energy_image_warping.hip
--- a/thallo_amd/csrc/energy_image_warping.hip
+++ b/thallo_amd/csrc/energy_image_warping.hip
@@ -289,6 +289,7 @@
     block_store_partial(acc, bN_out, red);
 }
 
+template <bool LEAN>
 __global__ __launch_bounds__(BLOCK) void k_init(Geo g, const float2* __restrict__ off, const float* __restrict__ ang,
                                                 const float2* __restrict__ ur, const float2* __restrict__ cons,
                                                 const float* __restrict__ mask, float wf, float wr,
@@ -317,7 +318,7 @@
                 ff = mask[pix] == 0.0f ? 1 : 0;
                 if ((gy < g.row0 || gy >= g.row1) && lx >= 1 && lx <= TW) {
                     cs[pix] = make_float2(cc, ss); flags[pix] = ff;
-                    reinterpret_cast<float2*>(p_prev)[pix] = make_float2(0.f, 0.f); p_prev[2 * N + pix] = 0.f;
+                    if (!LEAN) { reinterpret_cast<float2*>(p_prev)[pix] = make_float2(0.f, 0.f); p_prev[2 * N + pix] = 0.f; }
                 }
             }
             T.px[idx] = ox; T.py[idx] = oy; T.c[idx] = cc; T.s[idx] = ss; T.ux[idx] = uxx; T.uy[idx] = uyy; T.f[idx] = ff;
@@ -374,11 +375,13 @@
                     reinterpret_cast<float2*>(diag_out)[pix] = make_float2(dgo_raw, dgo_raw); diag_out[2 * N + pix] = dga_raw;
                 }
                 reinterpret_cast<float2*>(r)[pix] = make_float2(rx, ry);  r[2 * N + pix] = ra;
-                reinterpret_cast<float2*>(pre)[pix] = make_float2(mx, my); pre[2 * N + pix] = ma;
                 const float zx = mx * rx, zy = my * ry, zaa = ma * ra;
-                reinterpret_cast<float2*>(z)[pix] = make_float2(zx, zy);  z[2 * N + pix] = zaa;
-                reinterpret_cast<float2*>(p_prev)[pix] = make_float2(0.f, 0.f); p_prev[2 * N + pix] = 0.f;
-                reinterpret_cast<float2*>(delta)[pix] = make_float2(0.f, 0.f);  delta[2 * N + pix] = 0.f;
+                if (!LEAN) {
+                    reinterpret_cast<float2*>(pre)[pix] = make_float2(mx, my); pre[2 * N + pix] = ma;
+                    reinterpret_cast<float2*>(z)[pix] = make_float2(zx, zy);  z[2 * N + pix] = zaa;
+                    reinterpret_cast<float2*>(p_prev)[pix] = make_float2(0.f, 0.f); p_prev[2 * N + pix] = 0.f;
+                    reinterpret_cast<float2*>(delta)[pix] = make_float2(0.f, 0.f);  delta[2 * N + pix] = 0.f;
+                }
                 cs[pix] = make_float2(T.c[i], T.s[i]);
                 flags[pix] = fl;
                 acc += rx * zx + ry * zy + ra * zaa;
@@ -730,11 +733,16 @@
                            float* cs, unsigned char* flags, float* diag_out, int* irregular_out, float* aN_out, thallo_stream_t stream)
 {
     if (!rows_ok(H, row0, row1)) return -(int)hipErrorInvalidValue;
+    const bool lean = !pre && !z && !p_prev && !delta;
+    if (!r || !cs || !flags || !aN_out || (lean ? (row0 != 0 || row1 != H) : (!pre || !z || !p_prev || !delta))) return -(int)hipErrorInvalidValue;
     const Geo g = make_geo(W, H, row0, row1); const int grid = grid_for(g, 4);
     if (irregular_out && hipMemsetAsync(irregular_out, 0, sizeof(int), (hipStream_t)stream) != hipSuccess) return -(int)hipErrorInvalidValue;
-    hipLaunchKernelGGL(k_init, dim3(grid), dim3(BLOCK), 0, (hipStream_t)stream, g,
-                       (const float2*)offset, angle, (const float2*)urshape, (const float2*)constraints, mask, w_fit, w_reg,
-                       r, pre, z, p_prev, delta, (float2*)cs, flags, diag_out, irregular_out, aN_out);
+    if (lean) hipLaunchKernelGGL(k_init<true>, dim3(grid), dim3(BLOCK), 0, (hipStream_t)stream, g,
+                                 (const float2*)offset, angle, (const float2*)urshape, (const float2*)constraints, mask, w_fit, w_reg,
+                                 r, pre, z, p_prev, delta, (float2*)cs, flags, diag_out, irregular_out, aN_out);
+    else hipLaunchKernelGGL(k_init<false>, dim3(grid), dim3(BLOCK), 0, (hipStream_t)stream, g,
+                            (const float2*)offset, angle, (const float2*)urshape, (const float2*)constraints, mask, w_fit, w_reg,
+                            r, pre, z, p_prev, delta, (float2*)cs, flags, diag_out, irregular_out, aN_out);
     int e = check_launch(); return e ? e : grid;
 }
 
diff --git a/thallo_amd/csrc/energy_image_warping_march_rc.hip b/thallo_amd/csrc/energy_image_warping_march_rc.hip
--- a/thallo_amd/csrc/energy_image_warping_march_rc.hip
+++ b/thallo_amd/csrc/energy_image_warping_march_rc.hip
@@ -100,10 +100,11 @@
 typedef unsigned long long u64x2 __attribute__((ext_vector_type(2)));
 __device__ __forceinline__ void take4u(u32x4& d, const u32x4& s) { const u64x2 sv = __builtin_bit_cast(u64x2, s); unsigned long long a, b; take_pair(a, sv.x); take_pair(b, sv.y); u64x2 dv; dv.x = a; dv.y = b; d = __builtin_bit_cast(u32x4, dv); }
 __device__ __forceinline__ void take2u(u32x2& d, const u32x2& s) { unsigned long long a; take_pair(a, __builtin_bit_cast(unsigned long long, s)); d = __builtin_bit_cast(u32x2, a); }
-template <int DMODE>
+template <bool FIRST, int DMODE>
 __device__ __forceinline__ void take(RawRc<DMODE>& d, const RawRc<DMODE>& s)
 {
-    take4u(d.po, s.po); take2u(d.pa, s.pa); take4u(d.cs, s.cs); take1(d.f, s.f); take4u(d.ro, s.ro); take2u(d.ra, s.ra);
+    if (!FIRST) { take4u(d.po, s.po); take2u(d.pa, s.pa); }
+    take4u(d.cs, s.cs); take1(d.f, s.f); take4u(d.ro, s.ro); take2u(d.ra, s.ra);
     if (DMODE != 1) { take4u(d.dlo, s.dlo); take2u(d.dla, s.dla); }
     if (DMODE == 2) { take4u(d.ppo, s.ppo); take2u(d.ppa, s.ppa); }
 }
@@ -116,7 +117,7 @@
 struct RRow { v2f xy[2]; float ra[2]; };
 __device__ __forceinline__ v2f uf2(unsigned a, unsigned b) { return v2f{ uf(a), uf(b) }; }
 
-template <int DMODE, int DEPTH, int NTM, int OCC, int SLAB>
+template <int DMODE, int DEPTH, int NTM, int OCC, int SLAB, bool FIRST = false>
 __global__ __launch_bounds__(MARCH_NT, OCC) void k_iter_march_rc(MarchGeo g, const float* __restrict__ cs, const unsigned char* __restrict__ flags, float wf2, float wr2,
                                                             const float* __restrict__ r_in, float* __restrict__ r_out, const float* __restrict__ A_in, float* __restrict__ A_out,
                                                             const float* __restrict__ p_in, float* __restrict__ p_out, float* __restrict__ delta,
@@ -126,6 +127,7 @@
                                                             PrevSums prev)
 {
     static_assert(DEPTH == 1 || DEPTH == 2 || DEPTH == 4, "the prefetch slots rotate inside a trip of four rows");
+    static_assert(!FIRST || (SLAB == 0 && DMODE == 1), "the first iteration: whole images, no delta update");
     __shared__ float4 lut[32];
     __shared__ float red[16];
     __shared__ double redd[48];
@@ -169,7 +171,7 @@
         constexpr bool CL = decltype(CL_)::value;
         if (CL && tn > t_last) tn = t_last;
         const unsigned tc = CL ? (unsigned)(tn < 0 ? 0 : tn > g.H - 1 ? g.H - 1 : tn) : (unsigned)tn, row = tc * W2u;
-        s.po = bld4<nt_pin>(RS_P, vo16, row * 16u); s.pa = bld2<nt_pin>(RS_P, vo8, angle0 + row * 8u);
+        if (!FIRST) { s.po = bld4<nt_pin>(RS_P, vo16, row * 16u); s.pa = bld2<nt_pin>(RS_P, vo8, angle0 + row * 8u); }
         s.cs = bld4<nt_const>(RS_CS, vo16, row * 16u);
         const unsigned par = row & 1u;
         s.f = bld1<nt_const>(RS_F, par ? vf1 : vf0, (row - par) * 2u);
@@ -206,7 +208,7 @@
         PRow& k1 = pk[(j + 3) % 4]; const PRow& k2 = pk[(j + 2) % 4]; const PRow& k3 = pk[(j + 1) % 4];
         RRow& r1 = rr[(j + 1) % 2]; const RRow& r2 = rr[j % 2];
         RawT cur;
-        take(cur, slot[j % DEPTH]);
+        take<FIRST>(cur, slot[j % DEPTH]);
         fence_order();
         issue(slot[j % DEPTH], t + DEPTH, CL_);
         fence_order();
@@ -214,7 +216,7 @@
             const bool rowok = !CL || (t >= 0 && t < g.H);
             const unsigned par = ((unsigned)t * W2u) & 1u;
             const unsigned fl = (cur.f >> (par ? 16u - sh0 : sh0)) & (rowok ? mxin : 0u);
-            p0.xy[0] = uf2(cur.po.x, cur.po.y); p0.xy[1] = uf2(cur.po.z, cur.po.w); p0.pa[0] = uf(cur.pa.x); p0.pa[1] = uf(cur.pa.y);
+            if constexpr (!FIRST) { p0.xy[0] = uf2(cur.po.x, cur.po.y); p0.xy[1] = uf2(cur.po.z, cur.po.w); p0.pa[0] = uf(cur.pa.x); p0.pa[1] = uf(cur.pa.y); }
             g0.cs[0] = uf2(cur.cs.x, cur.cs.y); g0.cs[1] = uf2(cur.cs.z, cur.cs.w); g0.f = fl;
             g0.gx[0] = v2f{ g0.cs[0].y, -g0.cs[0].x }; g0.gx[1] = v2f{ g0.cs[1].y, -g0.cs[1].x };
             g0.a[0] = (float)(fl & 1u); g0.a[1] = (float)((fl >> 8) & 1u);
@@ -222,22 +224,28 @@
         if constexpr (PH >= PH_S1) {
             const int u = t - 1;
             const float4 m0 = lut[g1.f & 31u], m1 = lut[(g1.f >> 8) & 31u];
-            const float wfit[2] = { m0.z, m1.z };
-            v2f axy[2]; float av[2];
-            jtjp_pair_xy(p2, p1, p0, g2, g1, g0, g2.a, g1.a, g0.a, wfit, wr2, axy, av);
-            const bool ghost_row = SLAB && CL && ((u == ya - 1 && ya == g.row0 && u >= 0) || (u == yb && yb == g.row1 && u < g.H));
-            if (ghost_row) {
-                const unsigned row = (unsigned)u * W2u;
-                const u32x4 ao = bld4<false>(RS_AI, vo16, row * 16u); const u32x2 aa = bld2<false>(RS_AI, vo8, angle0 + row * 8u);
-                axy[0] = uf2(ao.x, ao.y); axy[1] = uf2(ao.z, ao.w); av[0] = uf(aa.x); av[1] = uf(aa.y);
+            [[maybe_unused]] v2f axy[2]; [[maybe_unused]] float av[2];
+            bool ghost_row = false;
+            if constexpr (!FIRST) {
+                const float wfit[2] = { m0.z, m1.z };
+                jtjp_pair_xy(p2, p1, p0, g2, g1, g0, g2.a, g1.a, g0.a, wfit, wr2, axy, av);
+                ghost_row = SLAB && CL && ((u == ya - 1 && ya == g.row0 && u >= 0) || (u == yb && yb == g.row1 && u < g.H));
+                if (ghost_row) {
+                    const unsigned row = (unsigned)u * W2u;
+                    const u32x4 ao = bld4<false>(RS_AI, vo16, row * 16u); const u32x2 aa = bld2<false>(RS_AI, vo8, angle0 + row * 8u);
+                    axy[0] = uf2(ao.x, ao.y); axy[1] = uf2(ao.z, ao.w); av[0] = uf(aa.x); av[1] = uf(aa.y);
+                }
             }
             v2f rxy[2] = { uf2(cur.ro.x, cur.ro.y), uf2(cur.ro.z, cur.ro.w) }; float rq[2] = { uf(cur.ra.x), uf(cur.ra.y) };
-            rxy[0] = fma2(-alpha, axy[0], rxy[0]); rxy[1] = fma2(-alpha, axy[1], rxy[1]);
-            rq[0] = __builtin_fmaf(-alpha, av[0], rq[0]); rq[1] = __builtin_fmaf(-alpha, av[1], rq[1]);
+            if constexpr (!FIRST) {
+                rxy[0] = fma2(-alpha, axy[0], rxy[0]); rxy[1] = fma2(-alpha, axy[1], rxy[1]);
+                rq[0] = __builtin_fmaf(-alpha, av[0], rq[0]); rq[1] = __builtin_fmaf(-alpha, av[1], rq[1]);
+            }
             const float mo[2] = { m0.x, m1.x }, ma[2] = { m0.y, m1.y };
 #pragma unroll
             for (int q = 0; q < 2; ++q) {
-                k1.xy[q] = mo[q] * rxy[q] + beta * p1.xy[q]; k1.pa[q] = ma[q] * rq[q] + beta * p1.pa[q];
+                if constexpr (FIRST) { k1.xy[q] = mo[q] * rxy[q] + 0.0f; k1.pa[q] = ma[q] * rq[q] + 0.0f; }
+                else { k1.xy[q] = mo[q] * rxy[q] + beta * p1.xy[q]; k1.pa[q] = ma[q] * rq[q] + beta * p1.pa[q]; }
                 r1.xy[q] = rxy[q]; r1.ra[q] = rq[q];
             }
             const bool mine = !CL || (u >= ya && u < yb);
@@ -300,9 +308,11 @@
         for (int i = 0; i < DEPTH; ++i) issue(slot[i], t_first + i, IC<1>{});
         step(t_first, IC<0>{}, IC<PH_ENTER>{}, IC<1>{});
         step(t_first + 1, IC<1>{}, IC<PH_ENTER>{}, IC<1>{});
-        if (SLAB == 2 && prev.gs != nullptr && prev.count > 0) rc_iteration_scalars_x(aNp, prev, dd, alpha, beta);
-        else rc_iteration_scalars(aNp, aDp, bNp, prev, alpha, beta, scal_writer);
-        alpha = to_sgpr(alpha); beta = to_sgpr(beta);
+        if constexpr (!FIRST) {
+            if (SLAB == 2 && prev.gs != nullptr && prev.count > 0) rc_iteration_scalars_x(aNp, prev, dd, alpha, beta);
+            else rc_iteration_scalars(aNp, aDp, bNp, prev, alpha, beta, scal_writer);
+            alpha = to_sgpr(alpha); beta = to_sgpr(beta);
+        }
         if (DMODE == 2) alpha2 = to_sgpr(safe_div<false>(rc_sum(aNpp), rc_sum(aDpp)));
         step(ya, IC<2>{}, IC<PH_S1>{}, IC<1>{});
         step(ya + 1, IC<3>{}, IC<PH_S1>{}, IC<1>{});
@@ -357,9 +367,10 @@
     const float wf2 = w_fit * w_fit, wr2 = w_reg * w_reg;
     const bool ev_on = g_launch_ev.armed != 0;
     if (ev_on) g_launch_ev.used = 1;
-#define RC_LAUNCH(DM, DP, OCC, NTM) do { if (ev_on) hipExtLaunchKernelGGL((k_iter_march_rc<DM, DP, NTM, OCC, SLAB>), dim3(grid), dim3(MARCH_NT), 0, stream, g_launch_ev.start, g_launch_ev.stop, 0, g, cs, flags, wf2, wr2, \
+#define RC_LAUNCH(DM, DP, OCC, NTM) RC_LAUNCH_F(DM, DP, OCC, NTM, false)
+#define RC_LAUNCH_F(DM, DP, OCC, NTM, FIRST) do { if (ev_on) hipExtLaunchKernelGGL((k_iter_march_rc<DM, DP, NTM, OCC, SLAB, FIRST>), dim3(grid), dim3(MARCH_NT), 0, stream, g_launch_ev.start, g_launch_ev.stop, 0, g, cs, flags, wf2, wr2, \
         r_in, r_out, A_in, A_out, p_in, p_out, delta, aNp, aDp, bNp, aNpp, aDpp, aD_out, s12_out, irregular, d, fin_tickets, aD_word, bN_word, xslot, prev); \
-    else hipLaunchKernelGGL((k_iter_march_rc<DM, DP, NTM, OCC, SLAB>), dim3(grid), dim3(MARCH_NT), 0, stream, g, cs, flags, wf2, wr2, \
+    else hipLaunchKernelGGL((k_iter_march_rc<DM, DP, NTM, OCC, SLAB, FIRST>), dim3(grid), dim3(MARCH_NT), 0, stream, g, cs, flags, wf2, wr2, \
         r_in, r_out, A_in, A_out, p_in, p_out, delta, aNp, aDp, bNp, aNpp, aDpp, aD_out, s12_out, irregular, d, fin_tickets, aD_word, bN_word, xslot, prev); } while (0)
 #ifdef THALLO_MARCH_SWEEP
 #define RC_BY_DEPTH(DM) do { if constexpr (SLAB != 0) RC_LAUNCH(DM, MARCH_RC_DEPTH, MARCH_RC_OCC, MARCH_NTM); else { const int dp = g_march_rc_depth, oc = g_march_rc_occ, nt = g_march_rc_nt; \
@@ -371,9 +382,13 @@
 #else
 #define RC_BY_DEPTH(DM) do { if (R >= MARCH_RC_DEEP_ROWS) RC_LAUNCH(DM, 4, MARCH_RC_OCC, MARCH_NTM); else RC_LAUNCH(DM, 2, MARCH_RC_OCC, MARCH_NTM); } while (0)
 #endif
-    if (dmode == 1) RC_BY_DEPTH(1); else if (dmode == 2) RC_BY_DEPTH(2); else RC_BY_DEPTH(0);
+    if (mode & 1) {
+        if constexpr (SLAB == 0) { if (R >= MARCH_RC_DEEP_ROWS) RC_LAUNCH_F(1, 4, MARCH_RC_OCC, MARCH_NTM, true); else RC_LAUNCH_F(1, 2, MARCH_RC_OCC, MARCH_NTM, true); }
+    }
+    else if (dmode == 1) RC_BY_DEPTH(1); else if (dmode == 2) RC_BY_DEPTH(2); else RC_BY_DEPTH(0);
 #undef RC_BY_DEPTH
 #undef RC_LAUNCH
+#undef RC_LAUNCH_F
     int e = check_launch(); return e ? e : grid;
 }
 
@@ -381,11 +396,11 @@
              const void* p_in, const void* p_out, const void* delta, int mode, thallo_sum_t aNp, thallo_sum_t aNpp, thallo_sum_t aDpp, const void* aD_out, const void* s12_out)
 {
     if ((W & 1) || W < 2 || H < 1 || row0 < 0 || row1 > H || row0 >= row1 || row0 > 1 || H - row1 > 1) return -(int)hipErrorInvalidValue;
-    if (mode & 1) return -(int)hipErrorInvalidValue;
-    if (!cs || !flags || !r_in || !r_out || !p_in || !p_out || !delta || !aD_out || !s12_out) return -(int)hipErrorInvalidValue;
+    if ((mode & 1) && (row0 > 0 || row1 < H)) return -(int)hipErrorInvalidValue;
+    if (!cs || !flags || !r_in || !r_out || !p_out || !aD_out || !s12_out || (!(mode & 1) && (!p_in || !delta))) return -(int)hipErrorInvalidValue;
     if ((row0 > 0 || row1 < H) && (!A_in || !A_out)) return -(int)hipErrorInvalidValue;
     if (aNp.count < 1 || !aNp.partials) return -(int)hipErrorInvalidValue;
-    if (((mode >> 1) & 3) == 2 && (aNpp.count < 1 || aDpp.count < 1 || !aNpp.partials || !aDpp.partials)) return -(int)hipErrorInvalidValue;
+    if (!(mode & 1) && ((mode >> 1) & 3) == 2 && (aNpp.count < 1 || aDpp.count < 1 || !aNpp.partials || !aDpp.partials)) return -(int)hipErrorInvalidValue;
     if (12.0 * (double)W * (double)H >= 4294967296.0) return -(int)hipErrorNotSupported;
     return 0;
 }
@@ -416,10 +431,11 @@
                                              const int* irregular, float* aD_out, double* s12_out, thallo_stream_t stream)
 {
     if (int e = rc_check(W, H, row0, row1, cs, flags, r_in, r_out, Ap_in, Ap_out, p_in, p_out, delta, mode, aNp, aNpp, aDpp, aD_out, s12_out)) return e;
-    if (prev.count < 1 || prev.count > THALLO_MAX_PARTIALS || !prev.alphaD_partials || !prev.s12_partials || !prev.alphaD_word || !prev.betaN_word ||
-        prev.s12_partials == s12_out) return -(int)hipErrorInvalidValue;
+    const bool first = mode & 1;
+    if (!first && (prev.count < 1 || prev.count > THALLO_MAX_PARTIALS || !prev.alphaD_partials || !prev.s12_partials || !prev.alphaD_word || !prev.betaN_word ||
+                   prev.s12_partials == s12_out)) return -(int)hipErrorInvalidValue;
     const thallo_sum_t none = { nullptr, 0 };
-    const PrevSums ps = { prev.alphaD_partials, prev.s12_partials, prev.count, prev.alphaD_word, prev.betaN_word };
+    const PrevSums ps = first ? PrevSums{ nullptr, nullptr, 0, nullptr, nullptr } : PrevSums{ prev.alphaD_partials, prev.s12_partials, prev.count, prev.alphaD_word, prev.betaN_word };
     if (row0 == 0 && row1 == H)
         return launch_march_rc<0>(W, H, row0, row1, cs, flags, w_fit, w_reg, r_in, r_out, nullptr, nullptr, p_in, p_out, delta, mode, aNp, none, none, aNpp, aDpp, irregular, thallo_dist_t{},
                                   aD_out, s12_out, nullptr, nullptr, nullptr, 0, (hipStream_t)stream, ps);
diff --git a/thallo_amd/csrc/pcg_kernels.hip b/thallo_amd/csrc/pcg_kernels.hip
--- a/thallo_amd/csrc/pcg_kernels.hip
+++ b/thallo_amd/csrc/pcg_kernels.hip
@@ -464,7 +464,7 @@
     }
 }
 
-template <bool V4>
+template <bool V4, bool FIRST>
 __global__ __launch_bounds__(BLOCK) void k_linear_update_n(float* __restrict__ X, float* __restrict__ delta, thallo_update_terms_t T, long len)
 {
     __shared__ float al[THALLO_HIP_MAX_UPDATE_TERMS];
@@ -476,7 +476,7 @@
     if (V4) {
         const long n4 = len >> 2;
         for (long i = (long)blockIdx.x * BLOCK + threadIdx.x; i < n4; i += (long)gridDim.x * BLOCK) {
-            float4 d = reinterpret_cast<const float4*>(delta)[i];
+            float4 d = FIRST ? make_float4(0.0f, 0.0f, 0.0f, 0.0f) : reinterpret_cast<const float4*>(delta)[i];
             int j = 0;
             for (; j + 8 <= T.count; j += 8) {
                 float4 q[8];
@@ -508,7 +508,7 @@
         }
     } else {
         for (long i = (long)blockIdx.x * BLOCK + threadIdx.x; i < len; i += (long)gridDim.x * BLOCK) {
-            float d = delta[i];
+            float d = FIRST ? 0.0f : delta[i];
             for (int j = 0; j < T.count; ++j) d = __builtin_fmaf(al[j], T.p[j][i], d);
             if (X) X[i] = X[i] + d; else delta[i] = d;
         }
@@ -1003,9 +1003,10 @@
     return e ? e : grid;
 }
 
-int thallo_hip_linear_update_n(float* X, float* delta, thallo_update_terms_t terms, long len, int max_workgroups, thallo_stream_t stream)
-{
-    if (!delta || len < 0 || terms.count < 0 || terms.count > THALLO_HIP_MAX_UPDATE_TERMS) return -(int)hipErrorInvalidValue;
+namespace {
+int linear_update_n(float* X, float* delta, thallo_update_terms_t terms, long len, int max_workgroups, thallo_stream_t stream, bool first)
+{
+    if ((!delta && !(first && X)) || len < 0 || terms.count < 0 || terms.count > THALLO_HIP_MAX_UPDATE_TERMS) return -(int)hipErrorInvalidValue;
     bool v4 = !(len & 3) && !(((uintptr_t)X | (uintptr_t)delta) & 15);
     for (int j = 0; j < terms.count; ++j) {
         if (!terms.p[j] || !terms.alphaN[j].partials || !terms.alphaD[j].partials || terms.alphaN[j].count < 1 || terms.alphaD[j].count < 1) return -(int)hipErrorInvalidValue;
@@ -1014,11 +1015,21 @@
     if (len == 0 || (terms.count == 0 && !X)) return 0;
     int grid = flat_grid(v4 ? len >> 2 : len, 2 * cu_count());
     if (max_workgroups > 0 && grid > max_workgroups) grid = max_workgroups;
-    if (v4) hipLaunchKernelGGL(k_linear_update_n<true>, dim3(grid), dim3(BLOCK), 0, (hipStream_t)stream, X, delta, terms, len);
-    else    hipLaunchKernelGGL(k_linear_update_n<false>, dim3(grid), dim3(BLOCK), 0, (hipStream_t)stream, X, delta, terms, len);
+    if (first) {
+        if (v4) hipLaunchKernelGGL((k_linear_update_n<true, true>), dim3(grid), dim3(BLOCK), 0, (hipStream_t)stream, X, delta, terms, len);
+        else    hipLaunchKernelGGL((k_linear_update_n<false, true>), dim3(grid), dim3(BLOCK), 0, (hipStream_t)stream, X, delta, terms, len);
+    } else {
+        if (v4) hipLaunchKernelGGL((k_linear_update_n<true, false>), dim3(grid), dim3(BLOCK), 0, (hipStream_t)stream, X, delta, terms, len);
+        else    hipLaunchKernelGGL((k_linear_update_n<false, false>), dim3(grid), dim3(BLOCK), 0, (hipStream_t)stream, X, delta, terms, len);
+    }
     int e = check_launch();
     return e ? e : grid;
 }
+}
+int thallo_hip_linear_update_n(float* X, float* delta, thallo_update_terms_t terms, long len, int max_workgroups, thallo_stream_t stream)
+{ return linear_update_n(X, delta, terms, len, max_workgroups, stream, false); }
+int thallo_hip_linear_update_n_first(float* X, float* delta, thallo_update_terms_t terms, long len, int max_workgroups, thallo_stream_t stream)
+{ return linear_update_n(X, delta, terms, len, max_workgroups, stream, true); }
 
 int thallo_hip_finish_sum(thallo_sum_t sum, float* out, thallo_stream_t stream)
 {
diff --git a/thallo_amd/csrc/plugin.hpp b/thallo_amd/csrc/plugin.hpp
--- a/thallo_amd/csrc/plugin.hpp
+++ b/thallo_amd/csrc/plugin.hpp
@@ -108,6 +108,8 @@
     virtual int pcg_step1(LaunchCtx&, SolverVectors&, int cur, bool first,
                           thallo_sum_t aN_prev, thallo_sum_t aD_prev, thallo_sum_t bN_prev, float* alphaD_out) = 0;
     virtual bool batches_delta() const { return false; }
+    virtual bool first_rc_ok() const { return false; }
+    virtual void first_rc_request() {}
     virtual bool takes_any_p_plane() const { return false; }
     virtual bool persist_ok() const { return false; }
     virtual int pcg_persist(struct LaunchCtx&, SolverVectors&, float* const* planes, int n_planes, int k0, int k1, float* parts, int slots, int B, int nb_prev, thallo_sum_t alphaN_prev) { return -1; }
diff --git a/thallo_amd/csrc/plugins.cpp b/thallo_amd/csrc/plugins.cpp
--- a/thallo_amd/csrc/plugins.cpp
+++ b/thallo_amd/csrc/plugins.cpp
@@ -159,6 +159,8 @@
     bool persist_ = false;
     bool march_rc_ = false;
     bool grid_ = false;
+    bool first_rc_req_ = false;
+    bool first_rc_ = false;
     int row0_ = 0, row1_ = 0;
 public:
     ImageWarpingPlugin(const unsigned* dims) : W((int)dims[0]), H((int)dims[1]), row1_((int)dims[1])
@@ -262,9 +264,15 @@
     int pcg_init(LaunchCtx& c, SolverVectors& v, int cur, float* aN) override
     {
         TimedLaunch t(c, "PCGInit1");
+        first_rc_ = first_rc_req_; first_rc_req_ = false;
+        if (first_rc_)
+            return thallo_hip_iw_pcg_init(W, H, row0_, row1_, offset, angle, urshape, constraints, mask, w_fit, w_reg,
+                                          v.r, nullptr, nullptr, nullptr, nullptr, (float*)cs.ptr, (unsigned char*)flags.ptr, v.diag, (int*)irregular.ptr, aN, c.stream);
         return thallo_hip_iw_pcg_init(W, H, row0_, row1_, offset, angle, urshape, constraints, mask, w_fit, w_reg,
                                       v.r, v.pre, v.z, v.p[cur], v.delta, (float*)cs.ptr, (unsigned char*)flags.ptr, v.diag, (int*)irregular.ptr, aN, c.stream);
     }
+    bool first_rc_ok() const override { const char* e = env_switch("THALLO_IW_FIRST_RC"); return march_rc_ && row0_ == 0 && row1_ == H && !(e && e[0] == '0'); }
+    void first_rc_request() override { first_rc_req_ = first_rc_ok(); }
     int apply_jtj(LaunchCtx& c, const float* p, float* Ap, float* out) override
     {
         TimedLaunch t(c, "PCGStep1");
@@ -294,7 +302,7 @@
                  float* aD_word, float* bN_word) override
     {
         TimedLaunch t(c, "PCGIteration");
-        if (march_rc_ && !(mode & 1))
+        if (march_rc_ && (!(mode & 1) || first_rc_))
             return thallo_hip_iw_pcg_iter_march_rc(W, H, row0_, row1_, (const float*)cs.ptr, (const unsigned char*)flags.ptr, w_fit, w_reg,
                                                    v.rbuf(cur), v.rbuf(cur ^ 1), v.Abuf(cur), v.Abuf(cur ^ 1), v.p[cur], v.p[cur ^ 1], v.delta, mode,
                                                    aN, aD, bN, aN2, aD2, (const int*)irregular.ptr, out, v.s12,
@@ -346,7 +354,7 @@
                           float* out, double* s12_out) override
     {
         TimedLaunch t(c, "PCGIteration");
-        if (march_rc_ && !(mode & 1))
+        if (march_rc_ && (!(mode & 1) || first_rc_))
             return thallo_hip_iw_pcg_iter_march_rc_deferred(W, H, row0_, row1_, (const float*)cs.ptr, (const unsigned char*)flags.ptr, w_fit, w_reg,
                                                             v.rbuf(cur), v.rbuf(cur ^ 1), v.Abuf(cur), v.Abuf(cur ^ 1), v.p[cur], v.p[cur ^ 1], v.delta, mode,
                                                             aN, aN2, aD2, prev, (const int*)irregular.ptr, out, s12_out, c.stream);
diff --git a/thallo_amd/csrc/solver.cpp b/thallo_amd/csrc/solver.cpp
--- a/thallo_amd/csrc/solver.cpp
+++ b/thallo_amd/csrc/solver.cpp
@@ -219,6 +219,7 @@
         { "THALLO_FRONTEND_COMPUTED", "frontend_computed" },
         { "THALLO_FRONTEND_PRELOAD", "frontend_preload" },
         { "THALLO_INC_LANES", "inc_lanes" },
+        { "THALLO_IW_FIRST_RC", "iw_first_rc" },
         { "THALLO_PERSIST", "persist" },
     };
     for (const char* k : known) if (!strcmp(k, name)) return getenv(name);
@@ -421,11 +422,12 @@
     return { rowlen * dist_->row0, rowlen * (dist_->row1 - dist_->row0) };
 }
 
-bool Plan::gn_begin(int& ev_lin)
+bool Plan::gn_begin(int& ev_lin, bool lean)
 {
     hipStream_t s = ctx.stream;
     const int ev_setup = timer_.start("Nonlinear Setup", s);
     cur_ = 0;
+    if (lean) plugin->first_rc_request();
     const int nb = plugin->pcg_init(ctx, v_, cur_, slot(2));
     if (nb < 0) { set_error("PCGInit1 launch failed (%d)", nb); return false; }
     set_nb(2, nb); finish(2);
@@ -519,11 +521,13 @@
     if (ensure_iter_buffers()) { set_error("out of device memory for the one-kernel schedule"); return 0; }
     const int L = sp.lIterations;
     int ev_lin;
-    if (!gn_begin(ev_lin)) return 0;
     const int n_ring = ring_planes(L);
     const GnSchedule sched = gn_schedule(L, n_ring);
+    const bool lean = n_ring >= 2 && sched != GnSchedule::Persist && !dist_ && plugin->batches_delta() && plugin->first_rc_ok();
+    if (!gn_begin(ev_lin, lean)) return 0;
     const bool async = n_ring >= 2 && aux_async_ && sched != GnSchedule::Persist && aux_stream();
     GnStep st{ L, n_ring < 2 && batch_delta_ && delta_planes_ != 0 && plugin->batches_delta(), PRing(*this, n_ring, async) };
+    st.ring.from_zero = lean;
     bool done = false;
     switch (sched) {
     case GnSchedule::Persist:        done = gn_loop_persist(st); break;
@@ -535,6 +539,7 @@
     if (st.ring.on() && L > 0) {
         if (ring_flush(st.ring, L - 1 - THALLO_HIP_MAX_UPDATE_TERMS) || st.ring.wait_for(L)) { set_error("PCGDeltaUpdate launch failed"); return 0; }
         if (!ring_linear_update(st.ring, L, [](int rc) { return rc >= 0; })) { set_error("PCGLinearUpdate launch failed"); return 0; }
+        st.ring.from_zero = false;
         plugin->unknowns_written();
     } else linear_update_tail(L, st.batched);
     return gn_end(ev_fin, ev_iter);
@@ -640,9 +645,11 @@
     hipStream_t s = ctx.stream;
     thallo_update_terms_t T;
     while (R.next_batch(upto, T)) {
+        const auto update = R.from_zero ? thallo_hip_linear_update_n_first : thallo_hip_linear_update_n;
+        R.from_zero = false;
         if (!R.async) {
             TimedLaunch t(ctx, "PCGDeltaUpdate");
-            if (thallo_hip_linear_update_n(nullptr, v_.delta, T, v_.n_alloc, 0, s) < 0) return -1;
+            if (update(nullptr, v_.delta, T, v_.n_alloc, 0, s) < 0) return -1;
             R.synced = R.flushed;
             continue;
         }
@@ -651,7 +658,7 @@
         if (hipEventRecord(words, s) != hipSuccess || hipStreamWaitEvent(aux_, words, 0) != hipSuccess) return -1;
         LaunchCtx cx = ctx; cx.stream = aux_;
         {   TimedLaunch t(cx, "PCGDeltaUpdate");
-            if (thallo_hip_linear_update_n(nullptr, v_.delta, T, v_.n_alloc, aux_workgroups_ > 0 ? aux_workgroups_ : thallo_hip_device_cu_count(), aux_) < 0) return -1; }
+            if (update(nullptr, v_.delta, T, v_.n_alloc, aux_workgroups_ > 0 ? aux_workgroups_ : thallo_hip_device_cu_count(), aux_) < 0) return -1; }
         if (hipEventRecord(done, aux_) != hipSuccess) return -1;
         R.sent.push_back(PRing::Sent{ R.flushed - 1, done });
     }
diff --git a/thallo_amd/csrc/solver.hpp b/thallo_amd/csrc/solver.hpp
--- a/thallo_amd/csrc/solver.hpp
+++ b/thallo_amd/csrc/solver.hpp
@@ -169,6 +169,7 @@
         std::vector<Sent> sent;
         size_t n_ev = 0;
         SolverVectors v;
+        bool from_zero = false;
         PRing(Plan& plan, int planes, bool on_second_stream) : P(plan), n(planes), async(on_second_stream), v(plan.v_) {}
         PRing(const PRing&) = delete;
         ~PRing() { if (!sent.empty()) (void)hipStreamWaitEvent(P.ctx.stream, sent.back().done, 0); }
@@ -220,7 +221,7 @@
     bool gn_loop_deferred(GnStep& st, int k_end);
     bool gn_loop_finish_in_launch(GnStep& st);
     int  step_gn_resident(int ev_iter);
-    bool gn_begin(int& ev_lin);
+    bool gn_begin(int& ev_lin, bool lean = false);
     int  gn_finish(int L, int ev_lin);
     int  gn_end(int ev_fin, int ev_iter);
     bool resident_used_ = false;
@@ -342,7 +343,8 @@
         const Owned o = owned_range(u);
         thallo_update_terms_t Tu = T;
         for (int j = 0; j < Tu.count; ++j) Tu.p[j] += off + o.lo;
-        if (!launched(thallo_hip_linear_update_n(plugin->unknown_ptr((int)u) + o.lo, v_.delta + off + o.lo, Tu, o.len, 0, ctx.stream))) return false;
+        const auto update = R.from_zero ? thallo_hip_linear_update_n_first : thallo_hip_linear_update_n;
+        if (!launched(update(plugin->unknown_ptr((int)u) + o.lo, v_.delta + off + o.lo, Tu, o.len, 0, ctx.stream))) return false;
         off += plugin->unknown_images()[u].n_floats;
     }
     return true;
```

Measured after the change: 17890 (median of 6 runs). About the same (+0.6%).
